# MeryylleA/Lunaris-Orion

Measured on AMD Instinct MI355X. Metric: 128x128 sprites/sec, VAE training step (train_hybrid.py _process_batch), latent_dim=512, higher is better.
Workload: dtype f16; 1 GPU; VAE-only training step (fwd+MSE/KL+bwd+clip+AdamW), per-GPU batch 64, latent_dim 512, teacher scalar 0 (--reward_scale 0 --quality_weight 0; the full hybrid step of BASELINE config 3 is the config3_full_hybrid object of a --full run at N=1), gradient_accumulation_steps 1, fp16 MFMA operands / fp32 accumulate, fp32 master weights; global_batch=64, latent_dim=512, parallelism=single, linear_weight_gradients=factored (never materialised)

## Files before the change

include/lunaris_hip.h:

```cpp
#ifndef LUNARIS_HIP_H
#define LUNARIS_HIP_H
#include <stddef.h>
#include <stdint.h>
#ifdef __cplusplus
extern "C" {
#endif

const char* lo_last_error(void);
int lo_version(void);

void lo_prof_enable(int on);
int lo_prof_count(void);
int lo_prof_get(int i, char* name, int name_cap, double* ms, double* flops, double* bytes);

enum {
  LO_KIND_CONV3_S1 = 0,
  LO_KIND_CONV3_S2 = 1,
  LO_KIND_CONVT4_S2 = 2,
  LO_KIND_CONV3_S1_DGRAD = 3,
  LO_KIND_CONV3_S2_DGRAD = 4,
  LO_KIND_CONVT4_S2_DGRAD = 5,
  LO_KIND_LINEAR = 6
};


size_t lo_packed_weight_elems_for(int kind, int B, int H, int W, int Cin, int Cout);
int lo_pack_weight_for(int kind, int B, int H, int W, int Cin, int Cout, const float* w, void* wp, void* stream);
int lo_conv_forward(int kind, int B, int H, int W, int Cin, int Cout, const void* in, const void* wp, const float* bias,
                    const void* add_src, void* out, float* gn_partial, int* mt_out, void* stream);
int lo_quantize_act_f8(const void* x16, void* x8, size_t n, void* stream);
int lo_pack_weight_f8_for(int kind, int B, int H, int W, int Cin, int Cout, const void* wp16, void* wp8, float* wscale, void* stream);
int lo_conv_forward_f8(int kind, int B, int H, int W, int Cin, int Cout, const void* in8, const void* wp8, const float* wscale,
                       const float* bias, const void* add_src, void* out, float* gn_partial, int* mt_out, void* stream);
int lo_conv3x3_fused_tap_forward(int B, int H, int W, int Cin, int Cout, int fp8, const void* in, const void* wp, const float* wscale,
                                 const float* bias, int leaky_relu, void* out, float* bn_partial, void* stream);
int lo_teacher_conv3x3_forward_f8(int B, int H, int W, int Cin, int Cout, const void* in8, const void* wp8, const float* wscale,
                                  const float* bias, int leaky_relu, void* out, float* bn_partial, int* rows_out, void* stream);
int lo_linear_splitk(int M, int K, int N, const void* x, const void* wp, const float* bias, float* slab, int nsplit,
                     float* out32, void* out16, void* stream);
size_t lo_wgrad_slab_bytes_for(int kind, int B, int H, int W, int Cin, int Cout);
int lo_conv_wgrad(int kind, int B, int H, int W, int Cin, int Cout, const void* x, const void* dy, float* slab,
                  float* grad, float scale, void* stream);

int lo_gn_mish_forward(const void* v, const float* gn_partial, int MT, const float* gamma, const float* beta,
                       const void* other, void* y, float* stats, int B, int HW, int C, int mode, void* stream);
int lo_gn_nchunk_for(int HW, int C);
int lo_gn_mish_backward(const void* dy, const void* v, const void* other, const float* stats, const float* gamma,
                        const float* beta, void* ds, void* dv, float* P1, float* P2, float* dgamma, float* dbeta,
                        float* dbias, int B, int HW, int C, int mode, float scale, void* stream);

int lo_first_conv_forward(const float* x, const float* w, const float* bias, void* v, float* gn_partial, int B, void* stream);
int lo_first_conv_wgrad_op(const float* x, const void* dv, float* partial , float* dw, int B, float scale, void* stream);
int lo_image_dgrad_op(const void* dy, int cout, int stride, const float* w, int B, float scale, float* dx, void* stream);
int lo_final_conv_forward(const void* a4, const float* w, const float* bias, const float* target, float* recon,
                          float* mse_partial, int B, void* stream);
int lo_final_conv_backward(const void* a4, const float* w, const float* recon, const float* target, const float* drecon,
                           const float* coef_dev, float gscale, void* da4, float* partial , float* dw,
                           float* db, int B, float scale, void* stream);

int lo_decode_sprites_u8(const void* u8_hwc, float* out_chw, int B, void* stream);

int lo_selfattn2d_forward(const float* x, const float* wq, const float* bq, const float* wk, const float* bk, const float* wv,
                          const float* bv, const float* gamma, float* q, float* k, float* v, float* out, int B, int C,
                          int N, void* stream);
size_t lo_selfattn2d_backward_scratch_elems(int B, int C, int N);
int lo_selfattn2d_backward(const float* x, const float* wq, const float* wk, const float* wv, const float* gamma,
                           const float* q, const float* k, const float* v, const float* dy, float* scratch, float* dx,
                           float* dwq, float* dbq, float* dwk, float* dbk, float* dwv, float* dbv, float* dgamma, int B,
                           int C, int N, void* stream);

int lo_clip_adamw_step(float* p, const float* g, float* m, float* v, size_t n, float max_norm, float lr, float beta1,
                       float beta2, float eps, float weight_decay, int step, float* scratch, void* stream);

int lo_clip_adamw_step_presummed(float* p, const float* g, float* m, float* v, size_t n, size_t presummed_begin, float max_norm,
                                 float lr, float beta1, float beta2, float eps, float weight_decay, int step, float* scratch,
                                 void* stream);

typedef struct LoVae LoVae;
int lo_vae_create(int batch, int latent_dim, LoVae** out);
#define LO_VAE_FP8_FWD 1u
int lo_vae_create_ex(int batch, int latent_dim, unsigned flags, LoVae** out);
void lo_vae_destroy(LoVae* h);
int lo_vae_set_gradnorm_scratch(LoVae* h, float* scratch);
int lo_gradnorm_early_range(const float* flat_grads, size_t begin, size_t end, float* scratch, void* stream);
int lo_vae_set_async_handover(LoVae* h, int on);
int lo_vae_wait_handover(LoVae* h, void* stream);
int lo_vae_gradnorm_presummed(const LoVae* h);
int lo_vae_num_params(const LoVae* h);
size_t lo_vae_param_offset(const LoVae* h, int index);
size_t lo_vae_param_numel(const LoVae* h, int index);
size_t lo_vae_flat_elems(const LoVae* h);
size_t lo_vae_workspace_bytes(const LoVae* h);
int lo_vae_pack(LoVae* h, const float* flat_params, void* ws, void* stream);
#define LO_OPT_PRESUMMED 1
#define LO_OPT_SERIAL 2
int lo_vae_optimizer_step(LoVae* h, float* p, const float* g, float* m, float* v, void* ws, float max_norm, float lr, float beta1,
                          float beta2, float eps, float weight_decay, int step, float* scratch, int flags, void* stream);
int lo_vae_join(LoVae* h, void* stream);
int lo_vae_set_linear_factored(LoVae* h, int mode);
int lo_vae_factor_block(const LoVae* h, size_t* byte_offset, size_t* bytes);
int lo_vae_materialize_gathered_linear_grads(LoVae* h, const void* gathered, int world, float* flat_grads, void* stream);
int lo_vae_linear_factored(const LoVae* h);
int lo_vae_materialize_linear_grads(LoVae* h, void* ws, float* flat_grads, void* stream);
int lo_vae_forward(LoVae* h, const float* x, const float* eps, uint64_t seed, const float* flat_params, void* ws,
                   float* recon, float* mu, float* logvar, const float* target, void* stream);
int lo_vae_decode(LoVae* h, const float* z, const float* flat_params, void* ws, float* recon, void* stream);
int lo_vae_encode(LoVae* h, const float* x, const float* flat_params, void* ws, float* mu, float* logvar, float* skip0, float* skip1,
                  float* skip2, void* stream);
int lo_vae_decode_skips(LoVae* h, const float* z, int n_skips, const float* skip0, const float* skip1, const float* skip2,
                        const float* flat_params, void* ws, float* recon, void* stream);
int lo_vae_decoder_backward(LoVae* h, const float* flat_params, void* ws, const float* recon, const float* drecon, float loss_scale,
                            float* dz, float* dskip0, float* dskip1, float* dskip2, float* flat_grads, void* stream);
int lo_vae_encoder_backward(LoVae* h, const float* x, const float* flat_params, void* ws, const float* gmu, const float* glv,
                            const float* gskip0, const float* gskip1, const float* gskip2, float loss_scale, float* flat_grads,
                            void* stream);
int lo_vae_encoder_backward_dx(LoVae* h, const float* x, const float* flat_params, void* ws, const float* gmu, const float* glv,
                               const float* gskip0, const float* gskip1, const float* gskip2, float loss_scale, float* flat_grads,
                               float* dx, void* stream);
int lo_vae_loss(LoVae* h, void* ws, float recon_weight, float kl_weight, float mean_advantage, const float* adv_dev,
                float accum, float loss_scale, float* losses_dev, void* stream);
int lo_vae_backward(LoVae* h, const float* x, const float* flat_params, void* ws, const float* recon, const float* target,
                    int fused, const float* drecon, const float* gmu, const float* glv, float loss_scale,
                    float* flat_grads, void* stream);
int lo_vae_backward_dx(LoVae* h, const float* x, const float* flat_params, void* ws, const float* recon, const float* target,
                       int fused, const float* drecon, const float* gmu, const float* glv, float loss_scale,
                       float* flat_grads, float* dx, void* stream);

int lo_vae_sync_fail_word(const LoVae* h, size_t* byte_offset, int* fused_layers);

int lo_grad_scale_pick(const float* g0, size_t n0, const float* g1, size_t n1, const float* g2, size_t n2, const float* g3, size_t n3,
                       const float* g4, size_t n4, float* scratch, void* stream);
int lo_scale_copy_dev(const float* src, float* dst, size_t n, const float* scale_dev, void* stream);
int lo_grad_unscale_dev(float* x, size_t n, const float* scale_dev, const void* fail_word, void* stream);
int lo_vae_fp8_layers(const LoVae* h, int* layers);
int lo_vae_debug_tensor(const LoVae* h, int which, int s, int k, size_t* byte_offset, int* dims4);

typedef struct LoTeacher LoTeacher;
int lo_teacher_create(int batch, int num_experts, int feature_dim, int embedding_dim, LoTeacher** out);
#define LO_TEACHER_FP8_CONV 1u
int lo_teacher_create_ex(int batch, int num_experts, int feature_dim, int embedding_dim, unsigned flags, LoTeacher** out);
void lo_teacher_destroy(LoTeacher* h);
int lo_teacher_num_tensors(const LoTeacher* h);
const char* lo_teacher_tensor_name(const LoTeacher* h, int index);
size_t lo_teacher_tensor_numel(const LoTeacher* h, int index);
long long lo_teacher_tensor_offset(const LoTeacher* h, int index);
size_t lo_teacher_flat_elems(const LoTeacher* h);
size_t lo_teacher_workspace_bytes(const LoTeacher* h);
int lo_teacher_pack(LoTeacher* h, const float* flat_state, void* ws, void* stream);
int lo_teacher_forward(LoTeacher* h, const float* x, float* flat_state, void* ws, int training, float dropout_p,
                       uint64_t drop_seed, float* quality_scores, float* expert_weights, float* style_embedding,
                       float* prompt_embedding, float* semantic_score, void* stream);
int lo_teacher_last_path(const LoTeacher* h);
int lo_dropout_mask(uint64_t drop_seed, int site, float dropout_p, size_t n, uint8_t* keep, void* stream);

int lo_teacher_grad_range(const LoTeacher* h, size_t* begin_elem, size_t* end_elem);
int lo_teacher_heads_backward(LoTeacher* h, const float* flat_state, void* ws, const float* expert_weights, float coef,
                              float* rows, float* flat_grads, void* stream);
int lo_teacher_heads_saved(const LoTeacher* h, size_t* byte_offsets3, size_t* elems3);
int lo_teacher_heads_backward_ex(LoTeacher* h, const float* flat_state, const float* pooled_f, const float* pooled_e,
                                 const float* raw_q, const float* expert_weights, const float* d_quality, const float* d_weights,
                                 float dropout_p, uint64_t drop_seed, float* rows, float* flat_grads, void* stream);
size_t lo_teacher_full_backward_bytes(const LoTeacher* h);
int lo_teacher_forward_keep(LoTeacher* h, const float* images_nchw, float* flat_state, void* ws, void* bws, float dropout_p,
                            uint64_t drop_seed, float* quality_scores, float* expert_weights, float* style_embedding,
                            float* prompt_embedding, float* semantic_score, void* stream);
int lo_teacher_full_backward(LoTeacher* h, const float* images_nchw, float* flat_state, void* ws, void* bws, const float* expert_weights,
                             float coef, float gscale, float* rows, float* flat_grads, void* stream);
int lo_teacher_full_backward_ex(LoTeacher* h, const float* images_nchw, float* flat_state, void* ws, void* bws, const float* pooled_f,
                                const float* pooled_e, const float* raw_q, const float* expert_weights, const float* d_quality,
                                const float* d_weights, float dropout_p, uint64_t drop_seed, float gscale, float* rows, float* flat_grads,
                                void* stream);
int lo_teacher_full_backward_dx(LoTeacher* h, const float* images_nchw, float* flat_state, void* ws, void* bws, const float* pooled_f,
                                const float* pooled_e, const float* raw_q, const float* expert_weights, const float* d_quality,
                                const float* d_weights, float dropout_p, uint64_t drop_seed, float gscale, float* rows, float* flat_grads,
                                float* dx, void* stream);
int lo_teacher_clip_adamw_full(LoTeacher* h, float* flat_state, const float* flat_grads, float* m, float* v, float max_norm, float lr,
                               float beta1, float beta2, float eps, float weight_decay, int step, float* scratch, void* stream);
int lo_teacher_full_param_count(const LoTeacher* h, size_t* tensors, size_t* elems);
int lo_hybrid_reward(const float* quality_scores, const float* semantic_score, int B, float semantic_weight,
                     float reward_scale, float momentum, float quality_weight, float accum, float* state2, float* out7,
                     float* adv_dev, void* stream);

int lo_vae_backward_phase(LoVae* h, int phase, const float* x, const float* flat_params, void* ws, const float* recon,
                          const float* target, int fused, const float* drecon, const float* gmu, const float* glv,
                          float loss_scale, float* flat_grads, void* stream);
int lo_vae_linear_grad_range(const LoVae* h, size_t* begin_elem, size_t* end_elem);
int lo_vae_phase1_grad_range(const LoVae* h, size_t* begin_elem, size_t* end_elem);
int lo_vae_stage4_grad_range(const LoVae* h, size_t* begin_elem, size_t* end_elem);

int lo_dp_pack_f16(const float* g, void* wire, size_t n, float scale, void* stream);
int lo_dp_unpack_f16(const void* wire, float* g, size_t n, float inv_scale, void* stream);
int lo_dp_unpack_f16_sumsq(const void* wire, float* g, size_t n, float inv_scale, float* scratch, void* stream);
int lo_dp_sum_shares(const void* recv, void* share, int world, size_t chunk, int is_f16, void* stream);

#ifdef __cplusplus
}
#endif
#endif
```

lunaris_orion_amd/_lib.py:

```python
from __future__ import annotations

import ctypes as C
import os

import torch

HERE = os.path.dirname(os.path.abspath(__file__))
LIB_PATH = os.path.join(HERE, "liblunaris_hip.so")

if not os.path.exists(LIB_PATH):
    raise ImportError(
        f"{LIB_PATH} not found: build it with `python -m lunaris_orion_amd.build` (hipcc, gfx950). "
        "There is no CPU or PyTorch fallback for the lunaris_orion_amd hot path."
    )

lib = C.CDLL(LIB_PATH, mode=C.RTLD_GLOBAL)

vp, f32p, i32, sz, u64, flt = C.c_void_p, C.c_void_p, C.c_int, C.c_size_t, C.c_uint64, C.c_float

SIGNATURES = {
    "lo_last_error": (C.c_char_p, []),
    "lo_version": (i32, []),
    "lo_prof_enable": (None, [i32]),
    "lo_prof_count": (i32, []),
    "lo_prof_get": (i32, [i32, C.c_char_p, i32, C.POINTER(C.c_double), C.POINTER(C.c_double), C.POINTER(C.c_double)]),
    "lo_packed_weight_elems_for": (sz, [i32] * 6),
    "lo_pack_weight_for": (i32, [i32] * 6 + [f32p, vp, vp]),
    "lo_conv_forward": (i32, [i32] * 6 + [vp, vp, f32p, vp, vp, f32p, C.POINTER(C.c_int), vp]),
    "lo_quantize_act_f8": (i32, [vp, vp, sz, vp]),
    "lo_pack_weight_f8_for": (i32, [i32] * 6 + [vp, vp, f32p, vp]),
    "lo_conv_forward_f8": (i32, [i32] * 6 + [vp, vp, f32p, f32p, vp, vp, f32p, C.POINTER(C.c_int), vp]),
    "lo_conv3x3_fused_tap_forward": (i32, [i32] * 6 + [vp, vp, f32p, f32p, i32, vp, f32p, vp]),
    "lo_teacher_conv3x3_forward_f8": (i32, [i32] * 5 + [vp, vp, f32p, f32p, i32, vp, f32p, C.POINTER(C.c_int), vp]),
    "lo_linear_splitk": (i32, [i32, i32, i32, vp, vp, f32p, f32p, i32, f32p, vp, vp]),
    "lo_wgrad_slab_bytes_for": (sz, [i32] * 6),
    "lo_conv_wgrad": (i32, [i32] * 6 + [vp, vp, f32p, f32p, flt, vp]),
    "lo_gn_mish_forward": (i32, [vp, f32p, i32, f32p, f32p, vp, vp, f32p, i32, i32, i32, i32, vp]),
    "lo_gn_nchunk_for": (i32, [i32, i32]),
    "lo_gn_mish_backward": (i32, [vp, vp, vp, f32p, f32p, f32p, vp, vp, f32p, f32p, f32p, f32p, f32p, i32, i32, i32, i32, flt, vp]),
    "lo_first_conv_forward": (i32, [f32p, f32p, f32p, vp, f32p, i32, vp]),
    "lo_first_conv_wgrad_op": (i32, [f32p, vp, f32p, f32p, i32, flt, vp]),
    "lo_image_dgrad_op": (i32, [vp, i32, i32, f32p, i32, flt, f32p, vp]),
    "lo_final_conv_forward": (i32, [vp, f32p, f32p, f32p, f32p, f32p, i32, vp]),
    "lo_final_conv_backward": (i32, [vp, f32p, f32p, f32p, f32p, f32p, flt, vp, f32p, f32p, f32p, i32, flt, vp]),
    "lo_decode_sprites_u8": (i32, [vp, f32p, i32, vp]),
    "lo_selfattn2d_forward": (i32, [f32p] * 12 + [i32, i32, i32, vp]),
    "lo_selfattn2d_backward_scratch_elems": (C.c_size_t, [i32, i32, i32]),
    "lo_selfattn2d_backward": (i32, [f32p] * 18 + [i32, i32, i32, vp]),
    "lo_clip_adamw_step": (i32, [f32p, f32p, f32p, f32p, sz, flt, flt, flt, flt, flt, flt, i32, f32p, vp]),
    "lo_teacher_create": (i32, [i32, i32, i32, i32, C.POINTER(C.c_void_p)]),
    "lo_teacher_create_ex": (i32, [i32, i32, i32, i32, C.c_uint, C.POINTER(C.c_void_p)]),
    "lo_teacher_destroy": (None, [vp]),
    "lo_teacher_num_tensors": (i32, [vp]),
    "lo_teacher_tensor_name": (C.c_char_p, [vp, i32]),
    "lo_teacher_tensor_numel": (sz, [vp, i32]),
    "lo_teacher_tensor_offset": (C.c_longlong, [vp, i32]),
    "lo_teacher_flat_elems": (sz, [vp]),
    "lo_teacher_workspace_bytes": (sz, [vp]),
    "lo_teacher_pack": (i32, [vp, f32p, vp, vp]),
    "lo_teacher_forward": (i32, [vp, f32p, f32p, vp, i32, flt, u64, f32p, f32p, f32p, f32p, f32p, vp]),
    "lo_teacher_last_path": (i32, [vp]),
    "lo_dropout_mask": (i32, [u64, i32, flt, sz, vp, vp]),
    "lo_teacher_grad_range": (i32, [vp, C.POINTER(C.c_size_t), C.POINTER(C.c_size_t)]),
    "lo_teacher_heads_backward": (i32, [vp, f32p, vp, f32p, flt, f32p, f32p, vp]),
    "lo_teacher_heads_saved": (i32, [vp, C.POINTER(C.c_size_t), C.POINTER(C.c_size_t)]),
    "lo_teacher_full_backward_bytes": (C.c_size_t, [vp]),
    "lo_teacher_full_backward_ex": (i32, [vp, f32p, f32p, vp, vp, f32p, f32p, f32p, f32p, f32p, f32p, flt, u64, flt, f32p, f32p, vp]),
    "lo_teacher_full_backward_dx": (i32, [vp, f32p, f32p, vp, vp, f32p, f32p, f32p, f32p, f32p, f32p, flt, u64, flt, f32p, f32p, f32p, vp]),
    "lo_teacher_forward_keep": (i32, [vp, f32p, f32p, vp, vp, flt, u64, f32p, f32p, f32p, f32p, f32p, vp]),
    "lo_teacher_full_backward": (i32, [vp, f32p, f32p, vp, vp, f32p, flt, flt, f32p, f32p, vp]),
    "lo_teacher_clip_adamw_full": (i32, [vp, f32p, f32p, f32p, f32p, flt, flt, flt, flt, flt, flt, i32, f32p, vp]),
    "lo_teacher_full_param_count": (i32, [vp, C.POINTER(C.c_size_t), C.POINTER(C.c_size_t)]),
    "lo_teacher_heads_backward_ex": (i32, [vp, f32p, f32p, f32p, f32p, f32p, f32p, f32p, flt, u64, f32p, f32p, vp]),
    "lo_hybrid_reward": (i32, [f32p, f32p, i32, flt, flt, flt, flt, flt, f32p, f32p, f32p, vp]),
    "lo_vae_create": (i32, [i32, i32, C.POINTER(C.c_void_p)]),
    "lo_vae_create_ex": (i32, [i32, i32, C.c_uint, C.POINTER(C.c_void_p)]),
    "lo_vae_set_gradnorm_scratch": (i32, [vp, f32p]),
    "lo_gradnorm_early_range": (i32, [f32p, sz, sz, f32p, vp]),
    "lo_vae_set_async_handover": (i32, [vp, i32]),
    "lo_vae_wait_handover": (i32, [vp, vp]),
    "lo_vae_optimizer_step": (i32, [vp, f32p, f32p, f32p, f32p, vp, flt, flt, flt, flt, flt, flt, i32, f32p, i32, vp]),
    "lo_vae_join": (i32, [vp, vp]),
    "lo_vae_set_linear_factored": (i32, [vp, i32]),
    "lo_vae_linear_factored": (i32, [vp]),
    "lo_vae_factor_block": (i32, [vp, C.POINTER(C.c_size_t), C.POINTER(C.c_size_t)]),
    "lo_vae_materialize_gathered_linear_grads": (i32, [vp, vp, i32, f32p, vp]),
    "lo_vae_materialize_linear_grads": (i32, [vp, vp, f32p, vp]),
    "lo_vae_gradnorm_presummed": (i32, [vp]),
    "lo_clip_adamw_step_presummed": (i32, [f32p, f32p, f32p, f32p, sz, sz, flt, flt, flt, flt, flt, flt, i32, f32p, vp]),
    "lo_vae_destroy": (None, [vp]),
    "lo_vae_num_params": (i32, [vp]),
    "lo_vae_param_offset": (sz, [vp, i32]),
    "lo_vae_param_numel": (sz, [vp, i32]),
    "lo_vae_flat_elems": (sz, [vp]),
    "lo_vae_workspace_bytes": (sz, [vp]),
    "lo_vae_pack": (i32, [vp, f32p, vp, vp]),
    "lo_vae_forward": (i32, [vp, f32p, f32p, u64, f32p, vp, f32p, f32p, f32p, f32p, vp]),
    "lo_vae_decode": (i32, [vp, f32p, f32p, vp, f32p, vp]),
    "lo_vae_encode": (i32, [vp, f32p, f32p, vp, f32p, f32p, f32p, f32p, f32p, vp]),
    "lo_vae_decode_skips": (i32, [vp, f32p, i32, f32p, f32p, f32p, f32p, vp, f32p, vp]),
    "lo_vae_decoder_backward": (i32, [vp, f32p, vp, f32p, f32p, flt, f32p, f32p, f32p, f32p, f32p, vp]),
    "lo_vae_encoder_backward": (i32, [vp, f32p, f32p, vp, f32p, f32p, f32p, f32p, f32p, flt, f32p, vp]),
    "lo_vae_encoder_backward_dx": (i32, [vp, f32p, f32p, vp, f32p, f32p, f32p, f32p, f32p, flt, f32p, f32p, vp]),
    "lo_vae_loss": (i32, [vp, vp, flt, flt, flt, f32p, flt, flt, f32p, vp]),
    "lo_vae_backward": (i32, [vp, f32p, f32p, vp, f32p, f32p, i32, f32p, f32p, f32p, flt, f32p, vp]),
    "lo_vae_backward_dx": (i32, [vp, f32p, f32p, vp, f32p, f32p, i32, f32p, f32p, f32p, flt, f32p, f32p, vp]),
    "lo_vae_backward_phase": (i32, [vp, i32, f32p, f32p, vp, f32p, f32p, i32, f32p, f32p, f32p, flt, f32p, vp]),
    "lo_vae_linear_grad_range": (i32, [vp, C.POINTER(C.c_size_t), C.POINTER(C.c_size_t)]),
    "lo_vae_phase1_grad_range": (i32, [vp, C.POINTER(C.c_size_t), C.POINTER(C.c_size_t)]),
    "lo_vae_debug_tensor": (i32, [vp, i32, i32, i32, C.POINTER(C.c_size_t), C.POINTER(C.c_int)]),
    "lo_dp_pack_f16": (i32, [f32p, vp, sz, flt, vp]),
    "lo_dp_unpack_f16": (i32, [vp, f32p, sz, flt, vp]),
    "lo_dp_unpack_f16_sumsq": (i32, [vp, f32p, sz, flt, f32p, vp]),
    "lo_dp_sum_shares": (i32, [vp, vp, i32, sz, i32, vp]),
    "lo_vae_sync_fail_word": (i32, [vp, C.POINTER(C.c_size_t), C.POINTER(C.c_int)]),
    "lo_grad_scale_pick": (i32, [f32p, sz, f32p, sz, f32p, sz, f32p, sz, f32p, sz, f32p, vp]),
    "lo_scale_copy_dev": (i32, [f32p, f32p, sz, f32p, vp]),
    "lo_grad_unscale_dev": (i32, [f32p, sz, f32p, vp, vp]),
    "lo_vae_fp8_layers": (i32, [vp, C.POINTER(C.c_int)]),
    "lo_vae_stage4_grad_range": (i32, [vp, C.POINTER(C.c_size_t), C.POINTER(C.c_size_t)]),
}

for _name, (_res, _args) in SIGNATURES.items():
    _fn = getattr(lib, _name)
    _fn.restype = _res
    _fn.argtypes = _args


class LunarisHipError(RuntimeError):
    pass


def check(rc: int, what: str = "") -> None:
    if rc != 0:
        msg = lib.lo_last_error()
        raise LunarisHipError(f"{what or 'liblunaris_hip'} failed (rc={rc}): {msg.decode() if msg else ''}")


def ptr(t) -> int | None:
    if t is None:
        return None
    return t.data_ptr()


def stream_ptr() -> int:
    return torch.cuda.current_stream().cuda_stream


def require_gpu() -> None:
    if not torch.cuda.is_available():
        raise LunarisHipError(
            "lunaris_orion_amd needs an AMD GPU (gfx950) visible to PyTorch-ROCm; there is no CPU fallback. "
            "The CPU oracle lives in oracle/ and is test infrastructure only."
        )
```

lunaris_orion_amd/build.py:

```python
from __future__ import annotations

import os
import subprocess
import sys

HERE = os.path.dirname(os.path.abspath(__file__))
CSRC = os.path.join(HERE, "csrc")
LIB = os.path.join(HERE, "liblunaris_hip.so")
SOURCES = ["lo_util.cpp", "lo_conv_geom.hip", "lo_igemm.hip", "lo_conv_f8.hip", "lo_conv_select.hip", "lo_conv3.hip", "lo_wgrad.hip", "lo_wgrad3.hip", "lo_wgrad2.hip", "lo_norm.hip", "lo_edge.hip", "lo_imgdgrad.hip", "lo_train.hip", "lo_lowrank.hip", "lo_attn.hip", "lo_teacher_plan.hip", "lo_teacher_kernels.hip", "lo_teacher_f128.hip", "lo_teacher_heads.hip", "lo_teacher_forward.hip", "lo_teacher_bwd_block.hip", "lo_teacher_bwd.hip", "lo_api.hip", "lo_vae_plan.hip", "lo_vae_opt.hip", "lo_vae_step.hip"]
HEADERS = ["lo_common.h", "lo_internal.h", "lo_conv.h", "lo_conv_dev.h", "lo_norm.h", "lo_vae.h", "lo_teacher.h", os.path.join("..", "..", "include", "lunaris_hip.h")]


def _hipcc() -> str:
    for c in (os.environ.get("HIPCC"), "/opt/rocm/bin/hipcc", "hipcc"):
        if c and (os.path.isabs(c) and os.path.exists(c) or not os.path.isabs(c)):
            return c
    return "hipcc"


def needs_build() -> bool:
    if not os.path.exists(LIB):
        return True
    t = os.path.getmtime(LIB)
    for f in SOURCES + HEADERS:
        p = os.path.join(CSRC, f)
        if os.path.exists(p) and os.path.getmtime(p) > t:
            return True
    return False


def build(force: bool = False, verbose: bool = True) -> str:
    if not force and not needs_build():
        return LIB
    objs = []
    procs = []
    os.makedirs(os.path.join(HERE, "build"), exist_ok=True)
    for f in SOURCES:
        src = os.path.join(CSRC, f)
        obj = os.path.join(HERE, "build", f + ".o")
        cmd = [_hipcc(), "--offload-arch=gfx950", "-O3", "-fPIC", "-std=c++17", "-x", "hip", "-c", src, "-o", obj]
        if verbose:
            print(" ".join(cmd), flush=True)
        procs.append((f, subprocess.Popen(cmd, stdout=subprocess.PIPE, stderr=subprocess.STDOUT, text=True)))
        objs.append(obj)
    fail = False
    for f, p in procs:
        out, _ = p.communicate()
        if p.returncode != 0:
            fail = True
            sys.stderr.write(f"[build] {f} failed:\n{out}\n")
        elif verbose and out.strip():
            print(out)
    if fail:
        raise RuntimeError("hipcc failed")
    cmd = [_hipcc(), "--offload-arch=gfx950", "-shared", "-fPIC", "-o", LIB] + objs
    if verbose:
        print(" ".join(cmd), flush=True)
    subprocess.check_call(cmd)
    return LIB


if __name__ == "__main__":
    build(force="--force" in sys.argv)
    print("built", LIB)
```

lunaris_orion_amd/csrc/lo_api.hip:

```cpp
#include "lo_internal.h"
#include "lo_conv.h"
#include "lo_norm.h"
#include "../../include/lunaris_hip.h"
#include <stdio.h>
#include <string.h>
#include <stdlib.h>
#include <vector>


extern "C" const char* lo_last_error(void) { return lo_get_error(); }
extern "C" int lo_version(void) { return 1; }

extern "C" size_t lo_packed_weight_elems_for(int kind, int B, int H, int W, int Cin, int Cout) {
  LoGeom g;
  if (lo_make_geom(&g, kind, B, H, W, Cin, Cout) != LO_OK) return 0;
  return lo_packed_weight_elems(g);
}
extern "C" int lo_pack_weight_for(int kind, int B, int H, int W, int Cin, int Cout, const float* w, void* wp, void* stream) {
  LoGeom g;
  LO_TRY(lo_make_geom(&g, kind, B, H, W, Cin, Cout));
  return lo_pack_weight(w, (f16*)wp, g, S(stream));
}
extern "C" int lo_conv_forward(int kind, int B, int H, int W, int Cin, int Cout, const void* in, const void* wp,
                               const float* bias, const void* add_src, void* out, float* gn_partial, int* mt_out,
                               void* stream) {
  LoGeom g;
  LO_TRY(lo_make_geom(&g, kind, B, H, W, Cin, Cout));
  const LoConvOp op{.in = (const f16*)in, .w = (const f16*)wp, .bias = bias, .add_src = (const f16*)add_src, .out = (f16*)out, .gn_partial = gn_partial};
  if (mt_out) *mt_out = lo_conv_choose(g, lo_conv_use(op)).mts;
  return lo_conv_run(g, op, S(stream));
}
extern "C" int lo_quantize_act_f8(const void* x16, void* x8, size_t n, void* stream) {
  LO_REQUIRE(x16 && x8, "lo_quantize_act_f8: null argument");
  return lo_quantize_f8((const f16*)x16, (uint8_t*)x8, n, S(stream));
}
extern "C" int lo_pack_weight_f8_for(int kind, int B, int H, int W, int Cin, int Cout, const void* wp16, void* wp8, float* wscale,
                                     void* stream) {
  LO_REQUIRE(wp16 && wp8 && wscale, "lo_pack_weight_f8_for: null argument");
  LoGeom g;
  LO_TRY(lo_make_geom(&g, kind, B, H, W, Cin, Cout));
  return lo_pack_f8_one(g, (const f16*)wp16, (uint8_t*)wp8, wscale, S(stream));
}
extern "C" int lo_conv_forward_f8(int kind, int B, int H, int W, int Cin, int Cout, const void* in8, const void* wp8,
                                  const float* wscale, const float* bias, const void* add_src, void* out, float* gn_partial,
                                  int* mt_out, void* stream) {
  LO_REQUIRE(in8 && wp8 && wscale && out, "lo_conv_forward_f8: null argument");
  LoGeom g;
  LO_TRY(lo_make_geom(&g, kind, B, H, W, Cin, Cout));
  const LoConvOp op{.bias = bias, .add_src = (const f16*)add_src, .out = (f16*)out, .gn_partial = gn_partial};
  LoConvUse use = lo_conv_use(op);
  use.f8 = true;
  if (mt_out) *mt_out = lo_conv_choose(g, use).mts;
  return lo_conv_run_f8(g, (const uint8_t*)in8, (const uint8_t*)wp8, wscale, op, S(stream));
}
extern "C" int lo_conv3x3_fused_tap_forward(int B, int H, int W, int Cin, int Cout, int fp8, const void* in, const void* wp, const float* wscale,
                                            const float* bias, int leaky_relu, void* out, float* bn_partial, void* stream) {
  LO_REQUIRE(in && wp && out && (!fp8 || wscale), "lo_conv3x3_fused_tap_forward: null argument");
  LoGeom g;
  LO_TRY(lo_make_geom(&g, LO_CONV3_S1, B, H, W, Cin, Cout));
  LoConvExtra ex{leaky_relu ? 1 : 0, bn_partial};
  if (fp8) return lo_conv3_run_pp_f8(g, (const uint8_t*)in, (const uint8_t*)wp, wscale, bias, (f16*)out, S(stream), &ex);
  return lo_conv3_run_pp_xf(g, (const f16*)in, nullptr, nullptr, 0, (const f16*)wp, bias, (f16*)out, S(stream), &ex);
}
extern "C" int lo_teacher_conv3x3_forward_f8(int B, int H, int W, int Cin, int Cout, const void* in8, const void* wp8, const float* wscale,
                                             const float* bias, int leaky_relu, void* out, float* bn_partial, int* rows_out, void* stream) {
  LO_REQUIRE(in8 && wp8 && wscale && out, "lo_teacher_conv3x3_forward_f8: null argument");
  LoGeom g;
  LO_TRY(lo_make_geom(&g, LO_CONV3_S1, B, H, W, Cin, Cout));
  const LoConvExtra ex{leaky_relu ? 1 : 0, bn_partial};
  const LoConvOp op{.bias = bias, .out = (f16*)out, .ex = &ex};
  LoConvUse use = lo_conv_use(op);
  use.f8 = true;
  const LoConvChoice c = lo_conv_choose(g, use);
  LO_REQUIRE(c.kernel == LO_CK_IGEMM_F8 && (B * H * W) % c.bm == 0,
             "lo_teacher_conv3x3_forward_f8: %d -> %d channels on %d x %d x %d is not served on e4m3 operands (Cin %% 128, Cout %% 64, whole M tiles)",
             Cin, Cout, B, H, W);
  if (rows_out) *rows_out = c.rows;
  return lo_conv_run_f8(g, (const uint8_t*)in8, (const uint8_t*)wp8, wscale, op, S(stream));
}
extern "C" int lo_linear_splitk(int M, int K, int N, const void* x, const void* wp, const float* bias, float* slab,
                                int nsplit, float* out32, void* out16, void* stream) {
  LoGeom g;
  LO_TRY(lo_make_geom(&g, LO_LINEAR, M, 1, 1, K, N));
  LO_TRY(lo_conv_run(g, {.in = (const f16*)x, .w = (const f16*)wp, .slab = slab, .nsplit = nsplit}, S(stream)));
  return lo_splitk_reduce(slab, bias, out32, (f16*)out16, M, N, nsplit, S(stream));
}
extern "C" size_t lo_wgrad_slab_bytes_for(int kind, int B, int H, int W, int Cin, int Cout) {
  LoGeom g;
  if (lo_make_geom(&g, kind, B, H, W, Cin, Cout) != LO_OK) return 0;
  return lo_wgrad_slab_bytes(g);
}
extern "C" int lo_conv_wgrad(int kind, int B, int H, int W, int Cin, int Cout, const void* x, const void* dy, float* slab,
                             float* grad, float scale, void* stream) {
  LoGeom g;
  LO_REQUIRE(kind == LO_CONV3_S1 || kind == LO_CONV3_S2 || kind == LO_CONVT4_S2 || kind == LO_LINEAR,
             "lo_conv_wgrad: kind %d is not a forward op", kind);
  LO_TRY(lo_make_geom(&g, kind, B, H, W, Cin, Cout));
  return lo_wgrad_run(g, (const f16*)x, (const f16*)dy, slab, grad, scale, S(stream));
}
extern "C" int lo_gn_mish_forward(const void* v, const float* gn_partial, int MT, const float* gamma, const float* beta,
                                  const void* other, void* y, float* stats, int B, int HW, int C, int mode, void* stream) {
  return lo_gn_forward({(const f16*)v, stats, gamma, beta, B, HW, C},
                       {.partial = gn_partial, .MT = MT, .other = (const f16*)other, .mode = mode, .y = (f16*)y}, S(stream));
}
extern "C" int lo_gn_nchunk_for(int HW, int C) { return lo_gn_nchunk(HW, C); }
extern "C" int lo_gn_mish_backward(const void* dy, const void* v, const void* other, const float* stats, const float* gamma,
                                   const float* beta, void* ds, void* dv, float* P1, float* P2, float* dgamma, float* dbeta,
                                   float* dbias, int B, int HW, int C, int mode, float scale, void* stream) {
  return lo_gn_bwd({(const f16*)v, stats, gamma, beta, B, HW, C},
                   {.dy = (const f16*)dy, .other = (const f16*)other, .mode = mode, .ds = (f16*)ds, .dv = (f16*)dv, .P1 = P1, .P2 = P2},
                   dgamma, dbeta, dbias, scale, S(stream));
}
extern "C" int lo_first_conv_forward(const float* x, const float* w, const float* bias, void* v, float* gn_partial, int B,
                                     void* stream) {
  return lo_first_conv_fwd(x, w, bias, (f16*)v, gn_partial, B, S(stream));
}
extern "C" int lo_first_conv_wgrad_op(const float* x, const void* dv, float* partial, float* dw, int B, float scale, void* stream) {
  return lo_first_conv_wgrad(x, (const f16*)dv, partial, dw, B, scale, S(stream));
}
extern "C" int lo_image_dgrad_op(const void* dy, int cout, int stride, const float* w, int B, float scale, float* dx, void* stream) {
  return lo_image_dgrad((const f16*)dy, cout, stride, w, B, scale, dx, S(stream));
}
extern "C" int lo_final_conv_forward(const void* a4, const float* w, const float* bias, const float* target, float* recon,
                                     float* mse_partial, int B, void* stream) {
  return lo_final_conv_fwd((const f16*)a4, w, bias, target, recon, mse_partial, B, S(stream));
}
extern "C" int lo_final_conv_backward(const void* a4, const float* w, const float* recon, const float* target,
                                      const float* drecon, const float* coef_dev, float gscale, void* da4, float* partial,
                                      float* dw, float* db, int B, float scale, void* stream) {
  return lo_final_conv_bwd((const f16*)a4, w, recon, target, drecon, coef_dev, gscale, (f16*)da4, partial, dw, db, B, scale,
                           S(stream));
}
extern "C" int lo_clip_adamw_step(float* p, const float* g, float* m, float* v, size_t n, float max_norm, float lr,
                                  float beta1, float beta2, float eps, float weight_decay, int step, float* scratch,
                                  void* stream) {
  LO_TRY(lo_gradnorm(g, n, max_norm, scratch, scratch + 1024, S(stream)));
  return lo_adamw(p, g, m, v, n, scratch + 1024, lr, beta1, beta2, eps, weight_decay, step, S(stream));
}

extern "C" int lo_clip_adamw_step_presummed(float* p, const float* g, float* m, float* v, size_t n, size_t presummed_begin, float max_norm,
                                            float lr, float beta1, float beta2, float eps, float weight_decay, int step, float* scratch,
                                            void* stream) {
  LO_REQUIRE(p && g && m && v && scratch && presummed_begin <= n && presummed_begin % 4 == 0, "lo_clip_adamw_step_presummed: bad argument");
  LO_TRY(lo_gradnorm_split(g, presummed_begin, max_norm, scratch, scratch + 1024, S(stream)));
  return lo_adamw(p, g, m, v, n, scratch + 1024, lr, beta1, beta2, eps, weight_decay, step, S(stream));
}

extern "C" int lo_decode_sprites_u8(const void* u8_hwc, float* out_chw, int B, void* stream) {
  LO_REQUIRE(u8_hwc && out_chw && B > 0, "lo_decode_sprites_u8: bad argument");
  return lo_decode_sprites((const uint8_t*)u8_hwc, out_chw, B, S(stream));
}

extern "C" int lo_selfattn2d_forward(const float* x, const float* wq, const float* bq, const float* wk, const float* bk,
                                     const float* wv, const float* bv, const float* gamma, float* q, float* k, float* v,
                                     float* out, int B, int C, int N, void* stream) {
  LO_REQUIRE(x && wq && bq && wk && bk && wv && bv && gamma && q && k && v && out, "lo_selfattn2d_forward: null argument");
  return lo_selfattn2d_fwd(x, wq, bq, wk, bk, wv, bv, gamma, q, k, v, out, B, C, N, S(stream));
}

extern "C" size_t lo_selfattn2d_backward_scratch_elems(int B, int C, int N) { return lo_selfattn2d_bwd_scratch(B, C, N); }
extern "C" int lo_selfattn2d_backward(const float* x, const float* wq, const float* wk, const float* wv, const float* gamma,
                                      const float* q, const float* k, const float* v, const float* dy, float* scratch, float* dx,
                                      float* dwq, float* dbq, float* dwk, float* dbk, float* dwv, float* dbv, float* dgamma, int B,
                                      int C, int N, void* stream) {
  LO_REQUIRE(x && wq && wk && wv && gamma && q && k && v && dy && scratch && dx && dwq && dbq && dwk && dbk && dwv && dbv && dgamma,
             "lo_selfattn2d_backward: null argument");
  return lo_selfattn2d_bwd(x, wq, wk, wv, gamma, q, k, v, dy, scratch, dx, dwq, dbq, dwk, dbk, dwv, dbv, dgamma, B, C, N, S(stream));
}

extern "C" int lo_dp_pack_f16(const float* g, void* wire, size_t n, float scale, void* stream) {
  LO_REQUIRE(g && wire, "lo_dp_pack_f16: null argument");
  return lo_dp_pack_f16_run(g, (f16*)wire, n, scale, S(stream));
}
extern "C" int lo_dp_unpack_f16_sumsq(const void* wire, float* g, size_t n, float inv_scale, float* scratch, void* stream) {
  LO_REQUIRE(g && wire && scratch, "lo_dp_unpack_f16_sumsq: null argument");
  return lo_dp_unpack_f16_sumsq_run((const f16*)wire, g, n, inv_scale, scratch, S(stream));
}
extern "C" int lo_dp_unpack_f16(const void* wire, float* g, size_t n, float inv_scale, void* stream) {
  LO_REQUIRE(g && wire, "lo_dp_unpack_f16: null argument");
  return lo_dp_unpack_f16_run((const f16*)wire, g, n, inv_scale, S(stream));
}
extern "C" int lo_dp_sum_shares(const void* recv, void* share, int world, size_t chunk, int is_f16, void* stream) {
  LO_REQUIRE(recv && share && world >= 1, "lo_dp_sum_shares: bad argument");
  return lo_dp_sum_shares_run(recv, share, world, chunk, is_f16, 1.0f / (float)world, S(stream));
}

extern "C" int lo_grad_scale_pick(const float* g0, size_t n0, const float* g1, size_t n1, const float* g2, size_t n2, const float* g3,
                                  size_t n3, const float* g4, size_t n4, float* scratch, void* stream) {
  LO_REQUIRE(scratch, "lo_grad_scale_pick: null scratch");
  const float* g[5] = {g0, g1, g2, g3, g4};
  const size_t n[5] = {n0, n1, n2, n3, n4};
  return lo_grad_scale_pick_run(g, n, scratch, S(stream));
}
extern "C" int lo_scale_copy_dev(const float* src, float* dst, size_t n, const float* scale_dev, void* stream) {
  LO_REQUIRE(src && dst && scale_dev, "lo_scale_copy_dev: null argument");
  return lo_scale_copy_dev_run(src, dst, n, scale_dev, S(stream));
}
extern "C" int lo_grad_unscale_dev(float* x, size_t n, const float* scale_dev, const void* fail_word, void* stream) {
  LO_REQUIRE(x && scale_dev, "lo_grad_unscale_dev: null argument");
  return lo_scale_dev_run(x, n, scale_dev, (const unsigned int*)fail_word, S(stream));
}
```

lunaris_orion_amd/csrc/lo_conv.h:

```cpp
#pragma once
#include "lo_common.h"

int lo_pack_weight(const float* w, f16* wp, const LoGeom& g, hipStream_t st);
int lo_pack_all(const LoPackJob* jobs_dev, int njobs, int nblocks, hipStream_t st, int block_base = 0);
int lo_pack_blocks(const LoGeom& g);
size_t lo_packed_weight_elems(const LoGeom& g);
static inline int lo_geom_packed_elems(const LoGeom& g) {
  int off = 0;
  for (int p = 0; p < g.n_phase; ++p) off += g.Cout * g.T[p] * g.Cin;
  return off;
}
static inline double lo_geom_flops(const LoGeom& g) {
  double f = 0;
  for (int p = 0; p < g.n_phase; ++p) f += 2.0 * g.B * g.GH * g.GW * (double)g.Cout * g.T[p] * g.Cin;
  return f;
}
static inline double lo_geom_bytes(const LoGeom& g) {
  return 2.0 * ((double)g.B * g.Hin * g.Win * g.Cin + (double)g.B * g.Hout * g.Wout * g.Cout + lo_geom_packed_elems(g));
}

struct LoGnBwdFuse {
  const f16* v; const float* stats; const float* gamma; const float* beta; float* P1;
  f16* dv = nullptr; float* P2 = nullptr; unsigned int* counter = nullptr; unsigned int target = 0; unsigned int* fail = nullptr;
  bool keep_out = false;
};
struct LoConvExtra { int act; float* bn_partial; int out_pitch = 0; int out_choff = 0; };
struct LoConvOp {
  const f16* in = nullptr;
  const f16* w = nullptr;
  const float* bias = nullptr;
  const f16* add_src = nullptr;
  f16* out = nullptr;
  float* gn_partial = nullptr;
  float* slab = nullptr;
  int nsplit = 1;
  const LoGnBwdFuse* gb = nullptr;
  const LoConvExtra* ex = nullptr;
  const LoGnFuse* gf = nullptr;
};
struct LoConvUse {
  bool bias = false, gn_partial = false, add = false;
  bool gb = false, gb_apply = false;
  bool ex = false, concat = false;
  bool gf = false;
  int nsplit = 1;
  bool f8 = false;
};
static inline LoConvUse lo_conv_use(const LoConvOp& op) {
  LoConvUse u;
  u.bias = op.bias != nullptr; u.gn_partial = op.gn_partial != nullptr; u.add = op.add_src != nullptr;
  u.gb = op.gb != nullptr; u.gb_apply = op.gb && op.gb->dv;
  u.ex = op.ex != nullptr; u.concat = op.ex && op.ex->out_pitch > 0;
  u.gf = op.gf != nullptr;
  u.nsplit = op.nsplit < 1 ? 1 : op.nsplit;
  return u;
}

enum LoConvKernel { LO_CK_NONE = 0, LO_CK_IGEMM, LO_CK_IGEMM_SPLITK, LO_CK_IGEMM_F8, LO_CK_CONV3_PP, LO_CK_CONVT4_PATCH, LO_CK_CONVS2D_PATCH };
struct LoConvChoice {
  int kernel;
  int bm, bn, bk;
  int th, tw;
  int grid;
  int mts;
  int rows;
  int nt;
  bool gn_fuse;
  bool gnb_apply;
};
LoConvChoice lo_conv_choose(const LoGeom& g, const LoConvUse& use);
int lo_conv_splitk_plan(const LoGeom& g);
int lo_conv_run(const LoGeom& g, const LoConvOp& op, hipStream_t st, LoConvChoice* chosen = nullptr);
int lo_conv_run_f8(const LoGeom& g, const uint8_t* in8, const uint8_t* w8, const float* wscale, const LoConvOp& op, hipStream_t st,
                   LoConvChoice* chosen = nullptr);

int lo_igemm_run(const LoGeom& g, const LoConvOp& op, const LoConvChoice& c, hipStream_t st);
int lo_igemm_run_f8(const LoGeom& g, const uint8_t* in8, const uint8_t* w8, const float* wscale, const LoConvOp& op, const LoConvChoice& c,
                    hipStream_t st);
int lo_splitk_reduce(const float* slab, const float* bias, float* out32, f16* out16, int M, int N, int nsplit, hipStream_t st);

int lo_conv3_run(const LoGeom& g, const LoConvOp& op, const LoConvChoice& c, hipStream_t st);
int lo_convt4_patch_run(const LoGeom& g, const LoConvOp& op, const LoConvChoice& c, hipStream_t st);
int lo_convs2d_patch_run(const LoGeom& g, const LoConvOp& op, const LoConvChoice& c, hipStream_t st);
bool lo_conv3_pp_applies(const LoGeom& g);
bool lo_conv3_pp_f8_applies(const LoGeom& g);
int lo_conv3_pp_rows(const LoGeom& g);
int lo_conv3_run_pp_xf(const LoGeom& g, const f16* in, const f16* xc, const f16* kx, int nlev, const f16* wp, const float* bias,
                       f16* out, hipStream_t st, const LoConvExtra* ex);
int lo_conv3_run_pp_f8(const LoGeom& g, const uint8_t* in8, const uint8_t* w8, const float* wscale, const float* bias, f16* out,
                       hipStream_t st, const LoConvExtra* ex);

struct LoPackF8Job { const f16* src; uint8_t* dst; float* scale; int K[LO_MAX_PHASE]; int wofs[LO_MAX_PHASE]; int Cout, n_phase, block0; };
void lo_pack_f8_job(LoPackF8Job* j, const LoGeom& g, const f16* src, uint8_t* dst, float* scale, int block0);
int lo_pack_f8_all(const LoPackF8Job* jobs_dev, int njobs, int nblocks, hipStream_t st, int block_base = 0);
int lo_pack_f8_one(const LoGeom& g, const f16* wp, uint8_t* w8, float* wscale, hipStream_t st);
int lo_quantize_f8(const f16* x, uint8_t* x8, size_t n, hipStream_t st);

enum LoWgradKernel { LO_WK_WGRAD3 = 0, LO_WK_WGRAD2, LO_WK_TN };
struct LoWgradChoice { int kernel; int nsplit; };
LoWgradChoice lo_wgrad_choose(const LoGeom& g);
int lo_wgrad_run(const LoGeom& g, const f16* x, const f16* dy, float* slab, float* grad, float scale, hipStream_t st);
size_t lo_wgrad_slab_bytes(const LoGeom& g);
int lo_wgrad3_nsplit(const LoGeom& g);
int lo_wgrad3_run(const LoGeom& g, const f16* x, const f16* dy, float* slab, hipStream_t st, int* nsplit_out);
int lo_wgrad2_nsplit(const LoGeom& g);
int lo_wgrad2_run(const LoGeom& g, const f16* x, const f16* dy, float* slab, hipStream_t st, int* nsplit_out);
```

lunaris_orion_amd/csrc/lo_conv_select.hip:

```cpp
#include "lo_conv.h"
#include "lo_norm.h"
#include <stdarg.h>
#include <stdio.h>
#include <string.h>
#include <stdlib.h>

int lo_conv_splitk_plan(const LoGeom& g) {
  if (g.n_phase != 1 || g.T[0] < 9 || g.Cin % 64 != 0 || g.Cout % 128 != 0) return 0;
  const long M = (long)g.B * g.GH * g.GW;
  if (M % 128 != 0 || !lo_gn_bwd_local_applies(g.GH * g.GW, g.Cout)) return 0;
  const long tiles = (M / 128) * (g.Cout / 128);
  if (tiles >= 256) return 0;
  const int ksteps = g.T[0] * (g.Cin / 64);
  int ns = (int)((512 + tiles - 1) / tiles);
  while (ns > 1 && ksteps / ns < 8) --ns;
  return ns >= 2 ? ns : 0;
}

static void pick_tile(const LoGeom& g, int* bm_out, int* bn_out) {
  const int per_sample = g.GH * g.GW;
  const size_t M = (size_t)g.B * per_sample;
  const int BK = (g.Cin % 64 == 0) ? 64 : 32;
  constexpr int min_wgs = 512;
  const int cand[4][2] = {{128, 128}, {128, 64}, {64, 128}, {64, 64}};
  int bm = 64, bn = (g.Cout % 64 == 0) ? 64 : 32;
  if (BK == 32) {
    bn = 64;
    bm = (per_sample % 128 == 0 && (M / 128) * (g.Cout / 64) * g.n_phase >= (size_t)min_wgs) ? 128 : 64;
  } else if (g.Cout % 64 != 0) {
    bm = (per_sample % 128 == 0 && (M / 128) * (g.Cout / 32) * g.n_phase >= (size_t)min_wgs) ? 128 : 64;
  } else {
    for (int i = 0; i < 4; ++i) {
      int cm = cand[i][0], cn = cand[i][1];
      if (per_sample % cm || g.Cout % cn || (g.Cout >> 3) > cn) continue;
      bm = cm; bn = cn;
      if (((M + cm - 1) / cm) * (g.Cout / cn) * g.n_phase >= (size_t)min_wgs) break;
    }
  }
  *bm_out = bm; *bn_out = bn;
}

static inline int conv3_mode() {
  static const int m = getenv("LO_HALO") ? atoi(getenv("LO_HALO")) : 2;
  return m;
}
static inline bool conv3_tile(const LoGeom& g, int* th, int* tw, int* bn) {
  if (g.n_phase != 1 || g.T[0] != 9 || g.in_stride != 1 || g.out_stride != 1) return false;
  if (g.Cin % 64 || g.Cout % 64 || g.Win % 16 || g.Hin % 16) return false;
  const long t16 = (long)g.B * (g.Hin / 16) * (g.Win / 16);
  if (g.Cout % 128 == 0 && t16 * (g.Cout / 128) >= 256) { *th = 16; *tw = 16; *bn = 128; }
  else if (g.Cout % 128 == 0) { *th = 8; *tw = 16; *bn = 128; }
  else if (g.Cout == 64) { *th = 16; *tw = 16; *bn = 64; }
  else return false;
  return (g.Cout >> 3) <= *bn;
}
static bool conv3_selected(const LoGeom& g, bool need_bn, int* th, int* tw, int* bn) {
  const int mode = conv3_mode();
  if (mode == 0 || !conv3_tile(g, th, tw, bn)) return false;
  if (mode == 2) {
    const long tiles = (long)g.B * (g.Hin / *th) * (g.Win / *tw) * (g.Cout / *bn);
    const bool long_grid = *th == 16 && *bn == 128 && tiles >= 1024;
    if (!(long_grid || (!need_bn && tiles >= 256))) return false;
  }
  return true;
}

static bool convt4_patch_geom(const LoGeom& g) {
  if (g.n_phase != 4 || g.in_stride != 1 || g.out_stride != 2) return false;
  if (!((g.Cin == 64 && g.Cout == 32) || (g.Cin == 128 && g.Cout == 64))) return false;
  for (int p = 0; p < 4; ++p) if (g.T[p] != 4) return false;
  return g.Hin % 16 == 0 && g.Win % 16 == 0 && g.Hout == 2 * g.Hin && g.Wout == 2 * g.Win;
}
static bool convs2d_patch_geom(const LoGeom& g) {
  if (g.n_phase != 4 || g.in_stride != 1 || g.out_stride != 2 || g.Cin != 128 || g.Cout != 64) return false;
  if (g.T[0] != 1 || g.T[1] != 2 || g.T[2] != 2 || g.T[3] != 4) return false;
  for (int p = 0; p < 4; ++p)
    for (int t = 0; t < g.T[p]; ++t) if (g.dy[p][t] < 0 || g.dy[p][t] > 1 || g.dx[p][t] < 0 || g.dx[p][t] > 1) return false;
  return g.Hin % 16 == 0 && g.Win % 16 == 0 && g.Hout == 2 * g.Hin && g.Wout == 2 * g.Win;
}

static void set_rows(LoConvChoice& c, const LoGeom& g, int mts, int nt) {
  c.mts = mts; c.nt = nt;
  c.rows = g.B * mts;
}
static void choose_igemm_tile(LoConvChoice& c, const LoGeom& g, int n_z) {
  const long M = (long)g.B * g.GH * g.GW;
  c.mts = (g.GH * g.GW / c.bm) * g.n_phase; c.nt = g.Cout / c.bn;
  c.rows = (int)((M / c.bm) * g.n_phase);
  c.grid = (int)((M + c.bm - 1) / c.bm) * c.nt * n_z;
}

static LoConvChoice choose_f8(const LoGeom& g) {
  static const bool force = !(getenv("LO_F8_FORCE") && atoi(getenv("LO_F8_FORCE")) == 0);
  LoConvChoice c{};
  int th, tw, bn;
  if (!(g.Cin % 128 == 0 && g.Cout % 64 == 0 && (force || !conv3_selected(g, false, &th, &tw, &bn)))) return c;
  c.kernel = LO_CK_IGEMM_F8;
  pick_tile(g, &c.bm, &c.bn);
  c.bk = 128;
  choose_igemm_tile(c, g, g.n_phase);
  return c;
}

LoConvChoice lo_conv_choose(const LoGeom& g, const LoConvUse& u) {
  if (u.f8) return choose_f8(g);
  LoConvChoice c{};
  const int nsplit = u.nsplit < 1 ? 1 : u.nsplit;
  const int per_sample = g.GH * g.GW;
  const bool bare = nsplit == 1 && !u.gb && !u.ex && !u.gf;
  const int tiles16 = (g.Hin / 16) * (g.Win / 16);
  if (bare && !u.add && convt4_patch_geom(g)) {
    c.kernel = LO_CK_CONVT4_PATCH;
    set_rows(c, g, tiles16, 1);
    c.grid = g.B * tiles16;
  } else if (bare && !u.bias && !u.gn_partial && convs2d_patch_geom(g) && g.B * tiles16 >= 128) {
    c.kernel = LO_CK_CONVS2D_PATCH;
    set_rows(c, g, 0, 1);
    c.grid = g.B * tiles16;
  } else if (int th, tw, bn; nsplit == 1 && conv3_selected(g, u.ex, &th, &tw, &bn)) {
    c.kernel = LO_CK_CONV3_PP;
    c.th = th; c.tw = tw; c.bn = bn;
    set_rows(c, g, (g.Hin / c.th) * (g.Win / c.tw), g.Cout / c.bn);
    c.grid = c.rows * c.nt;
    c.gn_fuse = u.gf && c.mts * c.nt <= LO_GNF_MAX_TILES;
    c.gnb_apply = u.gb_apply && (g.Cout >> 3) >= 8 && c.mts * c.nt <= LO_GNF_MAX_TILES;
  } else if (nsplit > 1) {
    c.kernel = LO_CK_IGEMM_SPLITK;
    c.bm = c.bn = (g.T[0] > 1 && ((long)g.B * per_sample) % 128 == 0 && g.Cout % 128 == 0) ? 128 : 64;
    c.bk = (g.Cin % 64 == 0) ? 64 : 32;
    choose_igemm_tile(c, g, nsplit);
    c.mts = c.rows = 0;
  } else {
    c.kernel = LO_CK_IGEMM;
    pick_tile(g, &c.bm, &c.bn);
    c.bk = (g.Cin % 64 == 0) ? 64 : 32;
    choose_igemm_tile(c, g, g.n_phase);
    const bool whole = g.Cin % 64 == 0 && g.Cout % 64 == 0 && per_sample % c.bm == 0 && (g.Cout >> 3) <= c.bn;
    c.gn_fuse = u.gf && whole && !convt4_patch_geom(g) && c.mts * c.nt <= LO_GNF_MAX_TILES;
    c.gnb_apply = u.gb_apply && whole && g.n_phase == 1 && (g.Cout >> 3) >= 8 && c.nt <= 8 && c.mts <= LO_GNF_MAX_TILES;
  }
  return c;
}

int lo_conv_run(const LoGeom& g, const LoConvOp& op, hipStream_t st, LoConvChoice* chosen) {
  const LoGnFuse* gf = op.gf;
  const LoGnBwdFuse* gb = op.gb;
  LO_REQUIRE(g.Cin % 32 == 0, "lo_conv_run: Cin=%d must be a multiple of 32", g.Cin);
  LO_REQUIRE(g.Cout % 32 == 0, "lo_conv_run: Cout=%d must be a multiple of 32", g.Cout);
  const LoConvUse u = lo_conv_use(op);
  const LoConvChoice c = lo_conv_choose(g, u);
  if (chosen) *chosen = c;
  if (gf) {
    LO_REQUIRE(u.nsplit <= 1 && !u.add && !gb && !u.ex && gf->y && gf->xbuf && gf->counter && gf->fail && gf->gamma && gf->beta &&
               (gf->mode == 0 || gf->other), "lo_conv_run: bad fused-GroupNorm arguments");
    LO_REQUIRE(c.gn_fuse && c.mts == gf->MTs && c.nt == gf->NT,
               "lo_conv_run: fused GroupNorm asked for a geometry / tile grid the kernel does not have (check LoConvChoice::gn_fuse)");
  }
  if (u.gb_apply)
    LO_REQUIRE(gb->P2 && gb->counter && gb->fail && c.gnb_apply,
               "lo_conv_run: fused GroupNorm-backward apply asked for a geometry the kernel does not support (check LoConvChoice::gnb_apply)");
  LO_REQUIRE(!u.concat || (!u.add && !gb && op.ex->out_pitch % 8 == 0 && op.ex->out_choff % 8 == 0), "lo_conv_run: bad concatenated-output arguments");
  switch (c.kernel) {
    case LO_CK_CONVT4_PATCH: return lo_convt4_patch_run(g, op, c, st);
    case LO_CK_CONVS2D_PATCH: return lo_convs2d_patch_run(g, op, c, st);
    case LO_CK_CONV3_PP: return lo_conv3_run(g, op, c, st);
    case LO_CK_IGEMM_SPLITK:
    case LO_CK_IGEMM: return lo_igemm_run(g, op, c, st);
    default: break;
  }
  lo_set_error("lo_conv_run: no kernel for this op");
  return LO_ERR_ARG;
}

int lo_conv_run_f8(const LoGeom& g, const uint8_t* in8, const uint8_t* w8, const float* wscale, const LoConvOp& op, hipStream_t st,
                   LoConvChoice* chosen) {
  LO_REQUIRE(!op.gb && !op.gf && !op.slab && op.nsplit <= 1 && !(op.ex && op.ex->out_pitch > 0),
             "lo_conv_run_f8: the e4m3 path has bias, residual add, GroupNorm partials and the teacher epilogue (activation, BatchNorm partials) only");
  LoConvUse u = lo_conv_use(op);
  u.f8 = true;
  const LoConvChoice c = lo_conv_choose(g, u);
  if (chosen) *chosen = c;
  LO_REQUIRE(c.kernel == LO_CK_IGEMM_F8, "lo_conv_run_f8: geometry not supported (Cin %% 128, Cout %% 64)");
  return lo_igemm_run_f8(g, in8, w8, wscale, op, c, st);
}
```

lunaris_orion_amd/csrc/lo_internal.h:

```cpp
#pragma once
#include "lo_common.h"

static inline hipStream_t S(void* s) { return reinterpret_cast<hipStream_t>(s); }
#define LO_TRY(call)            \
  do {                          \
    int _r = (call);            \
    if (_r != LO_OK) return _r; \
  } while (0)

const char* lo_get_error();

int lo_first_conv_fwd(const float* x, const float* w, const float* bias, f16* v, float* gn_partial, int B, hipStream_t st);
int lo_first_conv_wgrad(const float* x, const f16* dv, float* partial, float* dw, int B, float scale, hipStream_t st);
int lo_colsum(const float* partial, float* out, int nrow, int ncol, int stride, float scale, hipStream_t st);

int lo_image_dgrad(const f16* dy, int cout, int stride, const float* w, int B, float scale, float* dx, hipStream_t st);
int lo_final_conv_fwd(const f16* a4, const float* w, const float* bias, const float* target, float* recon,
                      float* mse_partial, int B, hipStream_t st);
int lo_final_conv_bwd(const f16* a4, const float* w, const float* recon, const float* target, const float* drecon,
                      const float* coef, float gscale, f16* da4, float* partial, float* dw, float* db, int B, float scale,
                      hipStream_t st, hipStream_t sum_st = nullptr, hipEvent_t sum_after = nullptr);

int lo_head_reduce(const float* slab, const float* bias, const float* eps_in, uint64_t seed, float* mu, float* logvar,
                   f16* z, float* eps_out, float* kl_partial, int B, int L, int nsplit, hipStream_t st, float* mu_user = nullptr,
                   float* logvar_user = nullptr);
int lo_loss_finalize(const float* mse_partial, int n_mse, const float* kl_partial, int n_kl, float rw, float kw, float adv,
                     const float* adv_dev, float accum, float ls, float* losses, float* coefs, float n_rec, float n_lat,
                     hipStream_t st);
int lo_latent_bwd(const f16* dz, const float* mu, const float* logvar, const float* eps, const float* coefs,
                  const float* gmu, const float* glv, float gscale, f16* dml, int B, int L, hipStream_t st);
int lo_colsum_f16(const f16* x, float* out, int M, int N, float scale, hipStream_t st);
int lo_cast_f32_f16(const float* src, f16* dst, size_t n, hipStream_t st);
int lo_scale_f32(float* x, size_t n, float scale, hipStream_t st);
int lo_dp_pack_f16_run(const float* g, f16* wire, size_t n, float scale, hipStream_t st);
int lo_dp_unpack_f16_run(const f16* wire, float* g, size_t n, float inv_scale, hipStream_t st);
int lo_dp_unpack_f16_sumsq_run(const f16* wire, float* g, size_t n, float inv_scale, float* scratch, hipStream_t st);
int lo_dp_sum_shares_run(const void* recv, void* share, int world, size_t chunk, int is_f16, float inv_world, hipStream_t st);
int lo_transpose_cast(const float* src, f16* dst, int R, int C, hipStream_t st);
int lo_gradnorm(const float* g, size_t n, float max_norm, float* partial, float* norm_out, hipStream_t st,
                const unsigned int* fail = nullptr);
int lo_sumsq_range(const float* g, size_t begin, size_t end, float* partial, hipStream_t st);
int lo_gradnorm_split(const float* g, size_t presummed_begin, float max_norm, float* partial, float* norm_out, hipStream_t st,
                      const unsigned int* fail = nullptr);
int lo_grad_scale_pick_run(const float* const g[5], const size_t n[5], float* scratch, hipStream_t st);
int lo_scale_copy_dev_run(const float* src, float* dst, size_t n, const float* scale_dev, hipStream_t st);
int lo_scale_dev_run(float* x, size_t n, const float* scale_dev, const unsigned int* fail, hipStream_t st);
int lo_adamw(float* p, const float* g, float* m, float* v, size_t n, const float* norm, float lr, float beta1, float beta2,
             float eps, float wd, int step, hipStream_t st, f16* cast = nullptr);

int lo_selfattn2d_fwd(const float* x, const float* wq, const float* bq, const float* wk, const float* bk, const float* wv,
                      const float* bv, const float* gamma, float* q, float* k, float* v, float* out, int B, int C, int N,
                      hipStream_t st);
size_t lo_selfattn2d_bwd_scratch(int B, int C, int N);
int lo_selfattn2d_bwd(const float* x, const float* wq, const float* wk, const float* wv, const float* gamma, const float* q,
                      const float* k, const float* v, const float* dy, float* scratch, float* dx, float* dwq, float* dbq,
                      float* dwk, float* dbk, float* dwv, float* dbv, float* dgamma, int B, int C, int N, hipStream_t st);
int lo_decode_sprites(const uint8_t* u8, float* out, int B, hipStream_t st);

int lo_lowrank_bp(int B);
bool lo_lowrank_applies(int B, int N, int K);
int lo_transpose_pad_f16_multi(const f16* const* src, f16* const* dst, const int* C, int njobs, int R, int Rp, hipStream_t st);
struct LoLowrankNorm { const f16* fshort; int n_short; const f16* flong; int n_long; float* gram; float* partial; int nslots; };
int lo_lowrank_sumsq(const LoLowrankNorm* layers, int nlayers, int B, float scale, hipStream_t st);
struct LoLowrankMat { float* p; float* m; float* v; f16* cast; f16* cast_t; const f16* xt; const f16* yt; int N, K; };
int lo_adamw_lowrank(const LoLowrankMat* mats, int nmat, int B, float gscale, const float* norm, float lr, float beta1, float beta2,
                     float eps, float wd, int step, hipStream_t st);
int lo_lowrank_materialize(float* gout, const f16* xt, const f16* yt, int N, int K, int B, float gscale, hipStream_t st);
int lo_lowrank_materialize_gathered(float* gout, const f16* xt, const f16* yt, size_t rank_stride_elems, int world, int N, int K, int B,
                                    float gscale, hipStream_t st);
int lo_sumsq_blocks(const float* g, size_t n, float* partial, int nblocks, hipStream_t st);
```

lunaris_orion_amd/csrc/lo_train.hip:

```cpp
#include "lo_common.h"
#include <stdlib.h>

__device__ __forceinline__ uint64_t lo_mix64(uint64_t x) {
  x += 0x9E3779B97F4A7C15ull;
  x = (x ^ (x >> 30)) * 0xBF58476D1CE4E5B9ull;
  x = (x ^ (x >> 27)) * 0x94D049BB133111EBull;
  return x ^ (x >> 31);
}
__device__ __forceinline__ float lo_randn(uint64_t seed, uint64_t idx) {
  uint64_t h = lo_mix64(seed ^ lo_mix64(idx));
  float u1 = ((float)(uint32_t)(h >> 40) + 0.5f) * (1.0f / 16777216.0f);
  float u2 = ((float)(uint32_t)((h >> 8) & 0xFFFFFF)) * (1.0f / 16777216.0f);
  return sqrtf(-2.0f * __logf(u1)) * __cosf(6.28318530718f * u2);
}

__global__ __launch_bounds__(256) void lo_head_reduce_kernel(const float* __restrict__ slab, const float* __restrict__ bias,
                                                             const float* __restrict__ eps_in, uint64_t seed,
                                                             float* __restrict__ mu, float* __restrict__ logvar,
                                                             f16* __restrict__ z, float* __restrict__ eps_out,
                                                             float* __restrict__ kl_partial, int B, int L, int nsplit,
                                                             float* __restrict__ mu_user, float* __restrict__ logvar_user) {
  __shared__ float red[4];
  int i = blockIdx.x * 256 + threadIdx.x;
  float term = 0.f;
  if (i < B * L) {
    int b = i / L, l = i - b * L;
    float m = bias[l], lv = bias[L + l];
    int s = 0;
    for (; s + 8 <= nsplit; s += 8) {
      float pm[8], pl[8];
#pragma unroll
      for (int u = 0; u < 8; ++u) {
        const float* p = slab + ((size_t)(s + u) * B + b) * (2 * L);
        pm[u] = p[l];
        pl[u] = p[L + l];
      }
#pragma unroll
      for (int u = 0; u < 8; ++u) { m += pm[u]; lv += pl[u]; }
    }
    for (; s < nsplit; ++s) {
      const float* p = slab + ((size_t)s * B + b) * (2 * L);
      m += p[l];
      lv += p[L + l];
    }
    float e = eps_in ? eps_in[i] : lo_randn(seed, (uint64_t)i);
    float sd = expf(0.5f * lv);
    mu[i] = m;
    logvar[i] = lv;
    if (mu_user) { mu_user[i] = m; logvar_user[i] = lv; }
    eps_out[i] = e;
    z[i] = (f16)(m + e * sd);
    term = 1.f + lv - m * m - expf(lv);
  }
  float w = lo_wave_sum(term);
  if ((threadIdx.x & 63) == 0) red[threadIdx.x >> 6] = w;
  __syncthreads();
  if (threadIdx.x == 0) kl_partial[blockIdx.x] = red[0] + red[1] + red[2] + red[3];
}

__global__ __launch_bounds__(256) void lo_loss_finalize_kernel(const float* __restrict__ mse_partial, int n_mse,
                                                               const float* __restrict__ kl_partial, int n_kl,
                                                               float rw, float kw, float adv_host, float accum, float ls,
                                                               const float* __restrict__ adv_dev, float* __restrict__ losses,
                                                               float* __restrict__ coefs, float n_rec, float n_lat) {
  __shared__ double red[2][4];
  double a = 0.0, b = 0.0;
  for (int i0 = threadIdx.x; i0 < n_mse; i0 += 8 * 256) {
    float v[8];
#pragma unroll
    for (int u = 0; u < 8; ++u) v[u] = i0 + u * 256 < n_mse ? mse_partial[i0 + u * 256] : 0.f;
#pragma unroll
    for (int u = 0; u < 8; ++u) a += (double)v[u];
  }
  for (int i = threadIdx.x; i < n_kl; i += 256) b += (double)kl_partial[i];
#pragma unroll
  for (int o = 32; o > 0; o >>= 1) { a += __shfl_xor(a, o, 64); b += __shfl_xor(b, o, 64); }
  if ((threadIdx.x & 63) == 0) { red[0][threadIdx.x >> 6] = a; red[1][threadIdx.x >> 6] = b; }
  __syncthreads();
  if (threadIdx.x == 0) {
    const double sa = (red[0][0] + red[0][1]) + (red[0][2] + red[0][3]), sb = (red[1][0] + red[1][1]) + (red[1][2] + red[1][3]);
    float recon_loss = (float)(sa / (double)n_rec);
    float kl_loss = (float)(-0.5 * sb / (double)n_lat);
    float adv = adv_dev ? adv_dev[0] : adv_host;
    float pg = -adv * recon_loss;
    losses[0] = recon_loss;
    losses[1] = kl_loss;
    losses[2] = (rw * recon_loss + kw * kl_loss + pg) / accum;
    losses[3] = pg;
    coefs[0] = ls * (rw - adv) / accum * 2.0f / n_rec;
    coefs[1] = ls * kw / accum / n_lat;
  }
}

__global__ void lo_latent_bwd_kernel(const f16* __restrict__ dz, const float* __restrict__ mu, const float* __restrict__ logvar,
                                     const float* __restrict__ eps, const float* __restrict__ coefs,
                                     const float* __restrict__ gmu, const float* __restrict__ glv, float gscale,
                                     f16* __restrict__ dml, int B, int L) {
  int i = blockIdx.x * blockDim.x + threadIdx.x;
  if (i >= B * L) return;
  int b = i / L, l = i - b * L;
  float ckl = coefs ? coefs[1] : 0.f;
  float d = (float)dz[i];
  float lv = logvar[i];
  float dm = ckl * mu[i] + d;
  float dl = ckl * 0.5f * (expf(lv) - 1.f) + d * eps[i] * 0.5f * expf(0.5f * lv);
  if (gmu) dm += gscale * gmu[i];
  if (glv) dl += gscale * glv[i];
  dml[(size_t)b * 2 * L + l] = (f16)dm;
  dml[(size_t)b * 2 * L + L + l] = (f16)dl;
}

__global__ __launch_bounds__(256) void lo_colsum_f16_kernel(const f16* __restrict__ x, float* __restrict__ out, int M, int N, float scale) {
  __shared__ float red[8][32][8];
  const int cc = threadIdx.x & 31, rg = threadIdx.x >> 5;
  const int j0 = (blockIdx.x * 32 + cc) * 8;
  float t[8];
#pragma unroll
  for (int q = 0; q < 8; ++q) t[q] = 0.f;
  if (j0 < N) {
    for (int m = rg; m < M; m += 32) {
      f16x8 v[4];
#pragma unroll
      for (int u = 0; u < 4; ++u)
        if (m + 8 * u < M) v[u] = *reinterpret_cast<const f16x8*>(x + (size_t)(m + 8 * u) * N + j0);
#pragma unroll
      for (int u = 0; u < 4; ++u)
        if (m + 8 * u < M) {
#pragma unroll
          for (int q = 0; q < 8; ++q) t[q] += (float)v[u][q];
        }
    }
  }
#pragma unroll
  for (int q = 0; q < 8; ++q) red[rg][cc][q] = t[q];
  __syncthreads();
  const int c = threadIdx.x;
  const int j = blockIdx.x * 256 + c;
  if (j < N) {
    float tot = 0.f;
#pragma unroll
    for (int r = 0; r < 8; ++r) tot += red[r][c >> 3][c & 7];
    out[j] = tot * scale;
  }
}

__global__ void lo_decode_sprites_kernel(const uint8_t* __restrict__ u8, float* __restrict__ out, int npix_total) {
  int i = blockIdx.x * blockDim.x + threadIdx.x;
  if (i >= npix_total) return;
  int n = i >> 14, p = i & 16383;
  const uint8_t* s = u8 + (size_t)i * 3;
  float* d = out + (size_t)n * 3 * 16384 + p;
  d[0] = (float)s[0] / 127.5f - 1.0f;
  d[16384] = (float)s[1] / 127.5f - 1.0f;
  d[32768] = (float)s[2] / 127.5f - 1.0f;
}

__global__ void lo_cast_f32_f16_kernel(const float* __restrict__ src, f16* __restrict__ dst, size_t n4) {
  size_t i = (size_t)blockIdx.x * blockDim.x + threadIdx.x;
  size_t stride = (size_t)gridDim.x * blockDim.x;
  for (; i < n4; i += stride) {
    f32x4 v = reinterpret_cast<const f32x4*>(src)[i];
    f16x4 h = {(f16)v[0], (f16)v[1], (f16)v[2], (f16)v[3]};
    reinterpret_cast<f16x4*>(dst)[i] = h;
  }
}
__global__ __launch_bounds__(256) void lo_transpose_cast_kernel(const float* __restrict__ src, f16* __restrict__ dst, int R, int C) {
  __shared__ float t[64][65];
  const int r0 = blockIdx.y * 64, c0 = blockIdx.x * 64;
  const int tx = threadIdx.x & 63, ty = threadIdx.x >> 6;
  for (int i = ty; i < 64; i += 4) {
    int r = r0 + i, c = c0 + tx;
    t[i][tx] = (r < R && c < C) ? src[(size_t)r * C + c] : 0.f;
  }
  __syncthreads();
  for (int i = ty; i < 64; i += 4) {
    int c = c0 + i, r = r0 + tx;
    if (r < R && c < C) dst[(size_t)c * R + r] = (f16)t[tx][i];
  }
}

__global__ __launch_bounds__(256) void lo_sumsq_partial_kernel(const float* __restrict__ g, size_t n, float* __restrict__ partial) {
  __shared__ float red[4];
  size_t i = (size_t)blockIdx.x * 256 + threadIdx.x;
  size_t stride = (size_t)gridDim.x * 256;
  float acc = 0.f;
  size_t n4 = n / 4;
  for (size_t k = i; k < n4; k += stride) {
    f32x4 v = reinterpret_cast<const f32x4*>(g)[k];
    acc += v[0] * v[0] + v[1] * v[1] + v[2] * v[2] + v[3] * v[3];
  }
  if (blockIdx.x == 0 && threadIdx.x == 0)
    for (size_t k = n4 * 4; k < n; ++k) acc += g[k] * g[k];
  float w = lo_wave_sum(acc);
  if ((threadIdx.x & 63) == 0) red[threadIdx.x >> 6] = w;
  __syncthreads();
  if (threadIdx.x == 0) partial[blockIdx.x] = red[0] + red[1] + red[2] + red[3];
}
__global__ __launch_bounds__(256) void lo_gradnorm_finalize_kernel(const float* __restrict__ partial, int n, float max_norm,
                                                                   float* __restrict__ norm_out, const unsigned int* __restrict__ fail) {
  __shared__ double red[256];
  double a = 0.0;
  for (int i = threadIdx.x; i < n; i += 256) a += (double)partial[i];
  red[threadIdx.x] = a;
  __syncthreads();
  if (threadIdx.x == 0) {
    double s = 0.0;
    for (int i = 0; i < 256; ++i) s += red[i];
    float norm = (float)sqrt(s);
    float coef = max_norm / (norm + 1e-6f);
    if (coef > 1.0f) coef = 1.0f;
    bool finite = isfinite(norm);
    const bool lost = fail && *fail != 0u;
    norm_out[0] = norm;
    norm_out[1] = (finite && !lost) ? coef : 0.f;
    norm_out[2] = (finite && !lost) ? 1.f : 0.f;
    if (!finite) norm_out[3] += 1.f;
  }
}
__device__ __forceinline__ void lo_adamw_elem(float& p, float g, float& m, float& v, float coef, float decay, float omb1, float beta2,
                                              float omb2, float bc2_sqrt, float eps, float step_size) {
#pragma clang fp contract(off)
  const float gg = g * coef;
  const float pp = p * decay;
  const float mm = __builtin_fmaf(gg - m, omb1, m);
  const float v2 = __builtin_fmaf(omb2 * gg, gg, v * beta2);
  const float denom = sqrtf(v2) / bc2_sqrt + eps;
  p = __builtin_fmaf(-step_size, mm / denom, pp);
  m = mm;
  v = v2;
}
__global__ __launch_bounds__(256) void lo_adamw_kernel(float* __restrict__ p, const float* __restrict__ g, float* __restrict__ m,
                                                       float* __restrict__ v, size_t n, const float* __restrict__ norm,
                                                       float lr, float beta1, float beta2, float eps, float wd, float bc1,
                                                       float bc2_sqrt, f16* __restrict__ cast) {
  const float coef = norm ? norm[1] : 1.0f;
  const bool ok = norm ? (norm[2] != 0.f) : true;
  if (!ok) return;
  size_t i = (size_t)blockIdx.x * 256 + threadIdx.x;
  size_t stride = (size_t)gridDim.x * 256;
  const float step_size = lr / bc1, decay = 1.0f - lr * wd, omb1 = 1.0f - beta1, omb2 = 1.0f - beta2;
  size_t n4 = n / 4;
  constexpr int U = 4;
  for (size_t k0 = i; k0 < n4; k0 += U * stride) {
    f32x4 pv[U], gv[U], mv[U], vv[U];
#pragma unroll
    for (int u = 0; u < U; ++u) {
      const size_t k = k0 + u * stride;
      if (k < n4) {
        pv[u] = reinterpret_cast<f32x4*>(p)[k];
        gv[u] = reinterpret_cast<const f32x4*>(g)[k];
        mv[u] = reinterpret_cast<f32x4*>(m)[k];
        vv[u] = reinterpret_cast<f32x4*>(v)[k];
      }
    }
#pragma unroll
    for (int u = 0; u < U; ++u) {
      const size_t k = k0 + u * stride;
      if (k < n4) {
#pragma unroll
        for (int j = 0; j < 4; ++j) {
          float pe = pv[u][j], me = mv[u][j], ve = vv[u][j];
          lo_adamw_elem(pe, gv[u][j], me, ve, coef, decay, omb1, beta2, omb2, bc2_sqrt, eps, step_size);
          pv[u][j] = pe; mv[u][j] = me; vv[u][j] = ve;
        }
        reinterpret_cast<f32x4*>(p)[k] = pv[u];
        reinterpret_cast<f32x4*>(m)[k] = mv[u];
        reinterpret_cast<f32x4*>(v)[k] = vv[u];
        if (cast) reinterpret_cast<f16x4*>(cast)[k] = (f16x4){(f16)pv[u][0], (f16)pv[u][1], (f16)pv[u][2], (f16)pv[u][3]};
      }
    }
  }
  if (blockIdx.x == 0 && threadIdx.x == 0)
    for (size_t k = n4 * 4; k < n; ++k) {
      float pe = p[k], me = m[k], ve = v[k];
      lo_adamw_elem(pe, g[k], me, ve, coef, decay, omb1, beta2, omb2, bc2_sqrt, eps, step_size);
      p[k] = pe; m[k] = me; v[k] = ve;
      if (cast) cast[k] = (f16)pe;
    }
}

int lo_head_reduce(const float* slab, const float* bias, const float* eps_in, uint64_t seed, float* mu, float* logvar,
                   f16* z, float* eps_out, float* kl_partial, int B, int L, int nsplit, hipStream_t st, float* mu_user,
                   float* logvar_user) {
  int nb = (B * L + 255) / 256;
  LoProfScope _p("lo_head_reduce", 0, 4.0 * B * 2 * L * (nsplit + 2), st);
  hipLaunchKernelGGL(lo_head_reduce_kernel, dim3(nb), dim3(256), 0, st, slab, bias, eps_in, seed, mu, logvar, z, eps_out,
                     kl_partial, B, L, nsplit, mu_user, logvar_user);
  LO_LAUNCH_CHECK("head_reduce");
  return LO_OK;
}
int lo_loss_finalize(const float* mse_partial, int n_mse, const float* kl_partial, int n_kl, float rw, float kw, float adv,
                     const float* adv_dev, float accum, float ls, float* losses, float* coefs, float n_rec, float n_lat,
                     hipStream_t st) {
  LoProfScope _p("lo_loss_finalize", 0, 0, st);
  hipLaunchKernelGGL(lo_loss_finalize_kernel, dim3(1), dim3(256), 0, st, mse_partial, n_mse, kl_partial, n_kl, rw, kw, adv,
                     accum, ls, adv_dev, losses, coefs, n_rec, n_lat);
  LO_LAUNCH_CHECK("loss_finalize");
  return LO_OK;
}
int lo_latent_bwd(const f16* dz, const float* mu, const float* logvar, const float* eps, const float* coefs,
                  const float* gmu, const float* glv, float gscale, f16* dml, int B, int L, hipStream_t st) {
  int n = B * L;
  LoProfScope _p("lo_latent_bwd", 0, 0, st);
  LO_LAUNCH_STOP(lo_latent_bwd_kernel, dim3((n + 255) / 256), dim3(256), 0, st, dz, mu, logvar, eps, coefs, gmu, glv,
                     gscale, dml, B, L);
  LO_LAUNCH_CHECK("latent_bwd");
  return LO_OK;
}
int lo_colsum_f16(const f16* x, float* out, int M, int N, float scale, hipStream_t st) {
  LO_REQUIRE(N % 8 == 0, "lo_colsum_f16: N=%d must be a multiple of 8", N);
  LoProfScope _p("lo_colsum_f16", 0, 2.0 * M * N, st);
  hipLaunchKernelGGL(lo_colsum_f16_kernel, dim3((N + 255) / 256), dim3(256), 0, st, x, out, M, N, scale);
  LO_LAUNCH_CHECK("colsum_f16");
  return LO_OK;
}
__global__ void lo_scale_f32_kernel(float* __restrict__ x, size_t n, float scale) {
  const size_t i = (size_t)blockIdx.x * blockDim.x + threadIdx.x;
  if (i < n) x[i] *= scale;
}
int lo_scale_f32(float* x, size_t n, float scale, hipStream_t st) {
  hipLaunchKernelGGL(lo_scale_f32_kernel, dim3((unsigned)((n + 255) / 256)), dim3(256), 0, st, x, n, scale);
  LO_LAUNCH_CHECK("scale_f32");
  return LO_OK;
}
int lo_cast_f32_f16(const float* src, f16* dst, size_t n, hipStream_t st) {
  LO_REQUIRE(n % 4 == 0, "lo_cast_f32_f16: n must be a multiple of 4");
  size_t n4 = n / 4;
  int nb = (int)((n4 + 255) / 256 < 4096 ? (n4 + 255) / 256 : 4096);
  LoProfScope _p("lo_cast_f32_f16", 0, 6.0 * n, st);
  hipLaunchKernelGGL(lo_cast_f32_f16_kernel, dim3(nb), dim3(256), 0, st, src, dst, n4);
  LO_LAUNCH_CHECK("cast");
  return LO_OK;
}
int lo_transpose_cast(const float* src, f16* dst, int R, int C, hipStream_t st) {
  LoProfScope _p("lo_transpose_cast", 0, 6.0 * R * C, st);
  hipLaunchKernelGGL(lo_transpose_cast_kernel, dim3((C + 63) / 64, (R + 63) / 64), dim3(256), 0, st, src, dst, R, C);
  LO_LAUNCH_CHECK("transpose_cast");
  return LO_OK;
}
#define LO_NORM_BLOCKS 1024
int lo_sumsq_range(const float* g, size_t begin, size_t end, float* partial, hipStream_t st) {
  LoProfScope _p("lo_gradnorm (early range)", 0, 4.0 * (end - begin), st);
  hipLaunchKernelGGL(lo_sumsq_partial_kernel, dim3(LO_NORM_BLOCKS / 2), dim3(256), 0, st, g + begin, end - begin, partial + LO_NORM_BLOCKS / 2);
  LO_LAUNCH_CHECK("sumsq_range");
  return LO_OK;
}
int lo_sumsq_blocks(const float* g, size_t n, float* partial, int nblocks, hipStream_t st) {
  LoProfScope _p("lo_gradnorm (early range)", 0, 4.0 * n, st);
  hipLaunchKernelGGL(lo_sumsq_partial_kernel, dim3(nblocks), dim3(256), 0, st, g, n, partial);
  LO_LAUNCH_CHECK("sumsq_blocks");
  return LO_OK;
}
int lo_gradnorm_split(const float* g, size_t presummed_begin, float max_norm, float* partial, float* norm_out, hipStream_t st,
                      const unsigned int* fail) {
  LoProfScope _p("lo_gradnorm", 0, 4.0 * presummed_begin, st);
  hipLaunchKernelGGL(lo_sumsq_partial_kernel, dim3(LO_NORM_BLOCKS / 2), dim3(256), 0, st, g, presummed_begin, partial);
  LO_LAUNCH_CHECK("sumsq_head");
  hipLaunchKernelGGL(lo_gradnorm_finalize_kernel, dim3(1), dim3(256), 0, st, partial, LO_NORM_BLOCKS, max_norm, norm_out, fail);
  LO_LAUNCH_CHECK("gradnorm_finalize");
  return LO_OK;
}
int lo_gradnorm(const float* g, size_t n, float max_norm, float* partial , float* norm_out, hipStream_t st,
                const unsigned int* fail) {
  LoProfScope _p("lo_gradnorm", 0, 4.0 * n, st);
  hipLaunchKernelGGL(lo_sumsq_partial_kernel, dim3(LO_NORM_BLOCKS), dim3(256), 0, st, g, n, partial);
  LO_LAUNCH_CHECK("sumsq");
  hipLaunchKernelGGL(lo_gradnorm_finalize_kernel, dim3(1), dim3(256), 0, st, partial, LO_NORM_BLOCKS, max_norm, norm_out, fail);
  LO_LAUNCH_CHECK("gradnorm_finalize");
  return LO_OK;
}
int lo_adamw(float* p, const float* g, float* m, float* v, size_t n, const float* norm, float lr, float beta1, float beta2,
             float eps, float wd, int step, hipStream_t st, f16* cast) {
  float bc1 = 1.0f - powf(beta1, (float)step);
  float bc2 = 1.0f - powf(beta2, (float)step);
  double bc1d = 1.0 - pow((double)beta1, (double)step), bc2d = 1.0 - pow((double)beta2, (double)step);
  (void)bc1; (void)bc2;
  LoProfScope _p(cast ? "lo_adamw(+fp16 copy)" : "lo_adamw", 0, (cast ? 30.0 : 28.0) * n, st);
  constexpr int max_blocks = 256;
  const size_t want = (n / 4 + 255) / 256;
  const int nblk = want >= (size_t)max_blocks ? max_blocks : (want < 1 ? 1 : (int)want);
  LO_LAUNCH_STOP(lo_adamw_kernel, dim3(nblk), dim3(256), 0, st, p, g, m, v, n, norm, lr, beta1, beta2, eps, wd,
                     (float)bc1d, (float)sqrt(bc2d), cast);
  LO_LAUNCH_CHECK("adamw");
  return LO_OK;
}

int lo_decode_sprites(const uint8_t* u8, float* out, int B, hipStream_t st) {
  int n = B * 16384;
  LoProfScope _p("lo_decode_sprites", 0, 15.0 * n, st);
  hipLaunchKernelGGL(lo_decode_sprites_kernel, dim3((n + 255) / 256), dim3(256), 0, st, u8, out, n);
  LO_LAUNCH_CHECK("decode_sprites");
  return LO_OK;
}

__device__ __forceinline__ float lo_sat16(float x) { return x != x ? x : fminf(fmaxf(x, -65504.0f), 65504.0f); }
__global__ __launch_bounds__(256) void lo_dp_pack_f16_kernel(const float* __restrict__ g, f16* __restrict__ wire, size_t n, float scale) {
  const size_t stride = (size_t)gridDim.x * blockDim.x * 4;
  for (size_t i = ((size_t)blockIdx.x * blockDim.x + threadIdx.x) * 4; i < n; i += stride) {
    if (i + 4 <= n) {
      const float4 v = *reinterpret_cast<const float4*>(g + i);
      f16x4 o = {(f16)lo_sat16(v.x * scale), (f16)lo_sat16(v.y * scale), (f16)lo_sat16(v.z * scale), (f16)lo_sat16(v.w * scale)};
      *reinterpret_cast<f16x4*>(wire + i) = o;
    } else {
      for (size_t j = i; j < n; ++j) wire[j] = (f16)lo_sat16(g[j] * scale);
    }
  }
}
__global__ __launch_bounds__(256) void lo_dp_unpack_f16_kernel(const f16* __restrict__ wire, float* __restrict__ g, size_t n, float inv_scale) {
  const size_t stride = (size_t)gridDim.x * blockDim.x * 4;
  for (size_t i = ((size_t)blockIdx.x * blockDim.x + threadIdx.x) * 4; i < n; i += stride) {
    if (i + 4 <= n) {
      const f16x4 v = *reinterpret_cast<const f16x4*>(wire + i);
      *reinterpret_cast<float4*>(g + i) = make_float4((float)v[0] * inv_scale, (float)v[1] * inv_scale, (float)v[2] * inv_scale, (float)v[3] * inv_scale);
    } else {
      for (size_t j = i; j < n; ++j) g[j] = (float)wire[j] * inv_scale;
    }
  }
}
__global__ __launch_bounds__(256) void lo_dp_unpack_f16_sumsq_kernel(const f16* __restrict__ wire, float* __restrict__ g, size_t n, float inv_scale,
                                                                     float* __restrict__ partial) {
  __shared__ float red[4];
  const size_t stride = (size_t)gridDim.x * blockDim.x * 4;
  float acc = 0.f;
  for (size_t i = ((size_t)blockIdx.x * blockDim.x + threadIdx.x) * 4; i < n; i += stride) {
    if (i + 4 <= n) {
      const f16x4 v = *reinterpret_cast<const f16x4*>(wire + i);
      const float a = (float)v[0] * inv_scale, b = (float)v[1] * inv_scale, c = (float)v[2] * inv_scale, d = (float)v[3] * inv_scale;
      *reinterpret_cast<float4*>(g + i) = make_float4(a, b, c, d);
      acc += a * a + b * b + c * c + d * d;
    } else {
      for (size_t j = i; j < n; ++j) { const float a = (float)wire[j] * inv_scale; g[j] = a; acc += a * a; }
    }
  }
  const float w = lo_wave_sum(acc);
  if ((threadIdx.x & 63) == 0) red[threadIdx.x >> 6] = w;
  __syncthreads();
  if (threadIdx.x == 0) partial[blockIdx.x] = red[0] + red[1] + red[2] + red[3];
}
template <typename T>
__global__ __launch_bounds__(256) void lo_dp_sum_shares_kernel(const T* __restrict__ recv, T* __restrict__ share, int world, size_t chunk, float inv_world) {
  const size_t stride = (size_t)gridDim.x * blockDim.x;
  for (size_t i = (size_t)blockIdx.x * blockDim.x + threadIdx.x; i < chunk; i += stride) {
    float t = 0.f;
    for (int r = 0; r < world; ++r) t += (float)recv[(size_t)r * chunk + i];
    share[i] = (T)(t * inv_world);
  }
}
static inline int lo_dp_blocks(size_t work_items) {
  size_t b = (work_items + 255) / 256;
  return (int)(b < 1 ? 1 : (b > 2048 ? 2048 : b));
}
int lo_dp_pack_f16_run(const float* g, f16* wire, size_t n, float scale, hipStream_t st) {
  LoProfScope _p("lo_dp_pack_f16", 0, 6.0 * n, st);
  hipLaunchKernelGGL(lo_dp_pack_f16_kernel, dim3(lo_dp_blocks((n + 3) / 4)), dim3(256), 0, st, g, wire, n, scale);
  LO_LAUNCH_CHECK("dp_pack_f16");
  return LO_OK;
}
int lo_dp_unpack_f16_run(const f16* wire, float* g, size_t n, float inv_scale, hipStream_t st) {
  LoProfScope _p("lo_dp_unpack_f16", 0, 6.0 * n, st);
  hipLaunchKernelGGL(lo_dp_unpack_f16_kernel, dim3(lo_dp_blocks((n + 3) / 4)), dim3(256), 0, st, wire, g, n, inv_scale);
  LO_LAUNCH_CHECK("dp_unpack_f16");
  return LO_OK;
}
int lo_dp_unpack_f16_sumsq_run(const f16* wire, float* g, size_t n, float inv_scale, float* scratch, hipStream_t st) {
  LoProfScope _p("lo_dp_unpack_f16(+sumsq)", 0, 6.0 * n, st);
  hipLaunchKernelGGL(lo_dp_unpack_f16_sumsq_kernel, dim3(LO_NORM_BLOCKS / 2), dim3(256), 0, st, wire, g, n, inv_scale, scratch + LO_NORM_BLOCKS / 2);
  LO_LAUNCH_CHECK("dp_unpack_f16_sumsq");
  return LO_OK;
}
int lo_dp_sum_shares_run(const void* recv, void* share, int world, size_t chunk, int is_f16, float inv_world, hipStream_t st) {
  LoProfScope _p("lo_dp_sum_shares", 0, (is_f16 ? 2.0 : 4.0) * (world + 1) * chunk, st);
  if (is_f16) hipLaunchKernelGGL((lo_dp_sum_shares_kernel<f16>), dim3(lo_dp_blocks(chunk)), dim3(256), 0, st, (const f16*)recv, (f16*)share, world, chunk, inv_world);
  else hipLaunchKernelGGL((lo_dp_sum_shares_kernel<float>), dim3(lo_dp_blocks(chunk)), dim3(256), 0, st, (const float*)recv, (float*)share, world, chunk, inv_world);
  LO_LAUNCH_CHECK("dp_sum_shares");
  return LO_OK;
}

struct LoAmaxJobs { const float* p[5]; size_t n[5]; };
__global__ __launch_bounds__(256) void lo_amax_partial_kernel(LoAmaxJobs J, float* __restrict__ partial) {
  __shared__ float red[4];
  float a = 0.f;
#pragma unroll
  for (int j = 0; j < 5; ++j) {
    const float* g = J.p[j];
    if (!g) continue;
    const size_t n = J.n[j], n4 = n / 4;
    for (size_t k = (size_t)blockIdx.x * 256 + threadIdx.x; k < n4; k += (size_t)gridDim.x * 256) {
      const f32x4 v = reinterpret_cast<const f32x4*>(g)[k];
      a = fmaxf(a, fmaxf(fmaxf(fabsf(v[0]), fabsf(v[1])), fmaxf(fabsf(v[2]), fabsf(v[3]))));
    }
    if (blockIdx.x == 0 && threadIdx.x == 0)
      for (size_t k = n4 * 4; k < n; ++k) a = fmaxf(a, fabsf(g[k]));
  }
#pragma unroll
  for (int o = 32; o > 0; o >>= 1) a = fmaxf(a, __shfl_xor(a, o, 64));
  if ((threadIdx.x & 63) == 0) red[threadIdx.x >> 6] = a;
  __syncthreads();
  if (threadIdx.x == 0) partial[blockIdx.x] = fmaxf(fmaxf(red[0], red[1]), fmaxf(red[2], red[3]));
}
__global__ __launch_bounds__(256) void lo_amax_finalize_kernel(const float* __restrict__ partial, int n, float* __restrict__ out2) {
  __shared__ float red[4];
  float a = 0.f;
  for (int i = threadIdx.x; i < n; i += 256) a = fmaxf(a, partial[i]);
#pragma unroll
  for (int o = 32; o > 0; o >>= 1) a = fmaxf(a, __shfl_xor(a, o, 64));
  if ((threadIdx.x & 63) == 0) red[threadIdx.x >> 6] = a;
  __syncthreads();
  if (threadIdx.x == 0) {
    a = fmaxf(fmaxf(red[0], red[1]), fmaxf(red[2], red[3]));
    float r = 1.0f;
    if (a > 0.f && isfinite(a)) {
      int e;
      (void)frexpf(a, &e);
      e = e > 100 ? 100 : (e < -100 ? -100 : e);
      r = ldexpf(1.0f, 2 - e);
    }
    out2[0] = r;
    out2[1] = 1.0f / r;
    out2[2] = a;
  }
}
__global__ __launch_bounds__(256) void lo_scale_copy_dev_kernel(const float* __restrict__ src, float* __restrict__ dst, size_t n,
                                                                const float* __restrict__ scale) {
  const float s = scale[0];
  const size_t n4 = n / 4;
  for (size_t k = (size_t)blockIdx.x * 256 + threadIdx.x; k < n4; k += (size_t)gridDim.x * 256) {
    f32x4 v = reinterpret_cast<const f32x4*>(src)[k];
    v *= s;
    reinterpret_cast<f32x4*>(dst)[k] = v;
  }
  if (blockIdx.x == 0 && threadIdx.x == 0)
    for (size_t k = n4 * 4; k < n; ++k) dst[k] = src[k] * s;
}
__global__ __launch_bounds__(256) void lo_scale_dev_kernel(float* __restrict__ x, size_t n, const float* __restrict__ scale,
                                                           const unsigned int* __restrict__ fail) {
  const float s = (fail && *fail != 0u) ? __builtin_nanf("") : scale[0];
  const size_t n4 = n / 4;
  for (size_t k = (size_t)blockIdx.x * 256 + threadIdx.x; k < n4; k += (size_t)gridDim.x * 256) {
    f32x4 v = reinterpret_cast<f32x4*>(x)[k];
    v *= s;
    reinterpret_cast<f32x4*>(x)[k] = v;
  }
  if (blockIdx.x == 0 && threadIdx.x == 0)
    for (size_t k = n4 * 4; k < n; ++k) x[k] *= s;
}
static inline int lo_stream_blocks(size_t n) {
  size_t b = (n / 4 + 255) / 256;
  return (int)(b < 1 ? 1 : (b > 1024 ? 1024 : b));
}
int lo_grad_scale_pick_run(const float* const g[5], const size_t n[5], float* scratch , hipStream_t st) {
  LoAmaxJobs J;
  size_t total = 0;
  for (int j = 0; j < 5; ++j) { J.p[j] = g[j]; J.n[j] = g[j] ? n[j] : 0; total += J.n[j]; }
  size_t want = (total / 4 + 255) / 256;
  const int nb = (int)(want < 1 ? 1 : (want > 256 ? 256 : want));
  hipLaunchKernelGGL(lo_amax_partial_kernel, dim3(nb), dim3(256), 0, st, J, scratch + 4);
  LO_LAUNCH_CHECK("amax_partial");
  hipLaunchKernelGGL(lo_amax_finalize_kernel, dim3(1), dim3(256), 0, st, scratch + 4, nb, scratch);
  LO_LAUNCH_CHECK("amax_finalize");
  return LO_OK;
}
int lo_scale_copy_dev_run(const float* src, float* dst, size_t n, const float* scale_dev, hipStream_t st) {
  hipLaunchKernelGGL(lo_scale_copy_dev_kernel, dim3(lo_stream_blocks(n)), dim3(256), 0, st, src, dst, n, scale_dev);
  LO_LAUNCH_CHECK("scale_copy_dev");
  return LO_OK;
}
int lo_scale_dev_run(float* x, size_t n, const float* scale_dev, const unsigned int* fail, hipStream_t st) {
  hipLaunchKernelGGL(lo_scale_dev_kernel, dim3(lo_stream_blocks(n)), dim3(256), 0, st, x, n, scale_dev, fail);
  LO_LAUNCH_CHECK("scale_dev");
  return LO_OK;
}
```

lunaris_orion_amd/csrc/lo_vae.h:

```cpp
#pragma once
#include "lo_internal.h"
#include "lo_conv.h"
#include "lo_norm.h"
#include "../../include/lunaris_hip.h"
#include <stdio.h>
#include <string.h>
#include <stdlib.h>
#include <vector>

#define WSP(T, off) reinterpret_cast<T*>(reinterpret_cast<unsigned char*>(ws) + (off))
#define PRM(i) (P + h->p_off[(i)])
#define GRD(i) (G + h->p_off[(i)])

struct ConvLayer {
  int kind = 0;
  int H = 0, W = 0, Cin = 0, Cout = 0;
  int Ho = 0, Wo = 0;
  LoGeom gf{}, gd{};
  int p_w = 0, p_b = 0, p_gw = 0, p_gb = 0;
  size_t o_wp_f = 0, o_wp_d = 0;
  size_t o_v = 0, o_a = 0;
  size_t o_part = 0, o_stats = 0;
  size_t o_P1 = 0, o_P2 = 0;
  int prow_cap = 0, np1 = 0, np2 = 0;
  int MT = 0;
  size_t o_dv = 0;
  bool f8 = false;
  size_t o_wp8 = 0, o_wscale = 0, o_a8 = 0;
  bool gnf = false; int gnf_mts = 0, gnf_nt = 0;
  size_t o_xbuf = 0, o_xcnt = 0;
  unsigned gnf_epoch = 0;
  size_t o_bcnt = 0;
  unsigned gba_epoch = 0;
  bool dv_done = false;
  hipEvent_t ev_ready = nullptr;
  int sk_fwd = 0, sk_dgrad = 0;
};

struct LoVae {
  int B = 0, L = 0;
  int nparam = 0;
  std::vector<size_t> p_off, p_numel;
  size_t flat_elems = 0;
  ConvLayer enc[4][3];
  ConvLayer dec[4];
  size_t o_eout[4] = {};
  size_t o_skipin[3] = {};
  LoGeom g_head{}, g_head_d{}, g_dfc{}, g_dfc_d{};
  int head_split = 32, dfcd_split = 32;
  size_t o_wp_head = 0, o_wp_head_t = 0, o_wp_dfc = 0, o_wp_dfc_t = 0;
  size_t o_xflat = 0, o_slab_head = 0, o_eps = 0, o_z = 0, o_klp = 0, o_mu = 0, o_lv = 0, o_yfc = 0, o_h0 = 0;
  size_t o_msep = 0, o_losses = 0, o_coefs = 0;
  size_t o_G[6] = {}, o_skipg[3] = {}, o_P1 = 0, o_P2 = 0, o_wslab = 0, o_wslab_lin = 0, o_fcw_part = 0, o_lc_part = 0, o_dz = 0, o_dml = 0,
         o_slab_dz = 0, o_gfc = 0;
  size_t o_packjobs = 0;
  std::vector<LoPackJob> packjobs_host;
  int n_packjobs = 0, pack_blocks = 0;
  int n_packjobs_enc = 0, pack_blocks_enc = 0;
  const void* packjobs_for_ws = nullptr;
  const void* packjobs_for_params = nullptr;
  size_t ws_bytes = 0;
  int idx_fc_mu_w = 0, idx_fc_mu_b = 0, idx_fc_lv_w = 0, idx_fc_lv_b = 0, idx_dfc_w = 0, idx_dfc_b = 0, idx_final_w = 0, idx_final_b = 0;
  bool forward_done = false, loss_done = false;
  bool enc_done = false, dec_done = false;
  int dec_skips = 0;
  hipStream_t side = nullptr;
  hipEvent_t ev_dv[4] = {}, ev_join = nullptr, ev_pre = nullptr, ev_range = nullptr;
  bool async_handover = false, range_pending = false;
  hipEvent_t ev_lvl[6] = {};
  bool lvl_pending[6] = {};
  struct { bool pending = false; float* P; const float* G; float* M; float* V; void* ws; const float* norm; float lr, beta1, beta2, eps, wd; int step; } defer;
  int n_packjobs_s4 = 0, pack_blocks_s4 = 0, n_packjobs8_s4 = 0, pack_blocks8_s4 = 0;
  int bwd_layer = 0;
  size_t o_skslab = 0;
  bool gn_local = true;
  int nevent = 0;
  bool overlap = false;
  float* norm_scratch = nullptr;
  bool fuse_gnb = true;
  bool fuse_gnf = false;
  bool fuse_gna = true;
  size_t o_sync_fail = 0;
  bool lin_factored = false, fac_ready = false;
  bool lin_factored_dp = false;
  int Bp = 0;
  size_t o_fac_dmlT = 0, o_fac_xT = 0, o_fac_gfcT = 0, o_fac_zT = 0, o_gram = 0;
  float fac_scale = 1.f;
  int n_cu = 0;
  const void* sync_for_ws = nullptr;
  bool fp8_fwd = false;
  size_t o_eout8[4] = {}, o_h08 = 0, o_packjobs8 = 0;
  std::vector<LoPackF8Job> packjobs8_host;
  int n_packjobs8 = 0, pack_blocks8 = 0;
  int n_packjobs8_enc = 0, pack_blocks8_enc = 0;
};

template <typename H, typename F>
static inline void for_each_layer(H* h, F&& fn) {
  for (int s = 0; s < 4; ++s)
    for (int k = 0; k < 3; ++k) fn(h->enc[s][k]);
  for (int s = 0; s < 4; ++s) fn(h->dec[s]);
}

static inline LoGnLayer vae_gn_layer(const LoVae* h, const ConvLayer& c, const float* P, void* ws) {
  return {WSP(f16, c.o_v), WSP(float, c.o_stats), PRM(c.p_gw), PRM(c.p_gb), h->B, c.Ho * c.Wo, c.Cout};
}
static inline int vae_record_rows(ConvLayer& c, LoGnRows r) {
  LO_REQUIRE(r.p1 <= c.prow_cap && r.p2 <= c.prow_cap, "GroupNorm backward %dx%dx%d: %d / %d rows of P1 / P2 per sample, room for %d",
             c.Ho, c.Wo, c.Cout, r.p1, r.p2, c.prow_cap);
  if (r.p1 > 0) c.np1 = r.p1;
  if (r.p2 > 0) c.np2 = r.p2;
  return LO_OK;
}

static inline bool vae_side_on(const LoVae* h) { return h->overlap && !g_lo_prof_on; }
static inline int vae_order(hipStream_t behind, hipStream_t ahead, hipEvent_t e) {
  LO_HIP(hipEventRecord(e, ahead));
  LO_HIP(hipStreamWaitEvent(behind, e, 0));
  return LO_OK;
}
static inline bool lo_event_marker() {
  static const bool on = getenv("LO_EVENT_MARKER") != nullptr;
  return on;
}
struct LoHandover {
  hipEvent_t ev = nullptr;
  LoHandover(hipEvent_t e, bool on) { if (on) { ev = e; if (!lo_event_marker()) g_lo_stop_event = e; } }
  LoHandover(LoVae* h, bool on) : LoHandover(on ? h->ev_dv[h->nevent & 3] : nullptr, on) { if (on) ++h->nevent; }
  ~LoHandover() { g_lo_stop_event = nullptr; }
  int finish(hipStream_t st) {
    if (ev && (g_lo_stop_event || lo_event_marker())) {
      g_lo_stop_event = nullptr;
      LO_HIP(hipEventRecord(ev, st));
    }
    return LO_OK;
  }
};

struct LoProfTag {
  template <typename... A>
  explicit LoProfTag(const char* fmt, A... a) {
    if (!(g_lo_prof_on && g_lo_prof_layers)) return;
    char text[64];
    snprintf(text, sizeof(text), fmt, a...);
    g_lo_prof_tag = lo_prof_intern(text);
  }
  void end() { g_lo_prof_tag = nullptr; }
  ~LoProfTag() { end(); }
};

int vae_flush_deferred(LoVae* h, hipStream_t after_main);
int vae_wait_level(LoVae* h, hipStream_t st, int lvl);
```

lunaris_orion_amd/csrc/lo_vae_plan.hip:

```cpp
#include "lo_vae.h"
#include <memory>

namespace {
struct Arena {
  size_t off = 0;
  size_t take(size_t bytes) {
    size_t o = off;
    off += (bytes + 255) & ~(size_t)255;
    return o;
  }
};
bool env_is_zero(const char* v) { return v && atoi(v) == 0; }
const int kEncCh[5] = {3, 64, 128, 256, 512};
const int kDecCh[5] = {512, 256, 128, 64, 32};
}

static int setup_conv_layer(ConvLayer& c, int kind, int B, int H, int W, int Cin, int Cout, int p_w, Arena& ar, bool first) {
  c.kind = kind; c.H = H; c.W = W; c.Cin = Cin; c.Cout = Cout;
  c.p_w = p_w; c.p_b = p_w + 1; c.p_gw = p_w + 2; c.p_gb = p_w + 3;
  if (!first) {
    LO_TRY(lo_make_geom(&c.gf, kind, B, H, W, Cin, Cout));
    int dk = kind == LO_CONV3_S1 ? LO_CONV3_S1_DGRAD : (kind == LO_CONV3_S2 ? LO_CONV3_S2_DGRAD : LO_CONVT4_S2_DGRAD);
    c.Ho = c.gf.Hout; c.Wo = c.gf.Wout;
    LO_TRY(lo_make_geom(&c.gd, dk, B, c.Ho, c.Wo, Cout, Cin));
    c.o_wp_f = ar.take(lo_packed_weight_elems(c.gf) * 2);
    c.o_wp_d = ar.take(lo_packed_weight_elems(c.gd) * 2);
    c.MT = lo_conv_choose(c.gf, {.bias = true, .gn_partial = true}).mts;
  } else {
    c.Ho = H / 2; c.Wo = W / 2;
    c.MT = 64;
  }
  size_t act = (size_t)B * c.Ho * c.Wo * Cout * 2;
  c.o_v = ar.take(act);
  c.o_a = ar.take(act);
  c.o_part = ar.take((size_t)B * c.MT * 16 * 4);
  c.o_stats = ar.take((size_t)B * 16 * 4);
  int nchunk = lo_gn_nchunk(c.Ho * c.Wo, Cout);
  c.prow_cap = nchunk > (c.Ho * c.Wo) / 64 ? nchunk : (c.Ho * c.Wo) / 64;
  c.o_P1 = ar.take((size_t)B * c.prow_cap * Cout * 2 * 4);
  c.o_P2 = ar.take((size_t)B * c.prow_cap * Cout * 4);
  c.o_dv = ar.take(act);
  c.o_xbuf = ar.take((size_t)B * LO_GNF_MAX_TILES * 128);
  c.o_xcnt = ar.take((size_t)B * 4);
  c.o_bcnt = ar.take((size_t)B * 8 * 4);
  return LO_OK;
}

static int plan_parameters(LoVae* h) {
  const int L = h->L;
  std::vector<size_t>& numel = h->p_numel;
  for (int s = 0; s < 4; ++s) {
    size_t ci = kEncCh[s], co = kEncCh[s + 1];
    numel.push_back(co * ci * 9); numel.push_back(co); numel.push_back(co); numel.push_back(co);
    for (int k = 0; k < 2; ++k) { numel.push_back(co * co * 9); numel.push_back(co); numel.push_back(co); numel.push_back(co); }
  }
  h->idx_fc_mu_w = (int)numel.size(); numel.push_back((size_t)L * 32768);
  h->idx_fc_mu_b = (int)numel.size(); numel.push_back(L);
  h->idx_fc_lv_w = (int)numel.size(); numel.push_back((size_t)L * 32768);
  h->idx_fc_lv_b = (int)numel.size(); numel.push_back(L);
  h->idx_dfc_w = (int)numel.size(); numel.push_back((size_t)32768 * L);
  h->idx_dfc_b = (int)numel.size(); numel.push_back(32768);
  const int dec_first = (int)numel.size();
  for (int s = 0; s < 4; ++s) {
    size_t ci = kDecCh[s], co = kDecCh[s + 1];
    numel.push_back(ci * co * 16); numel.push_back(co); numel.push_back(co); numel.push_back(co);
  }
  h->idx_final_w = (int)numel.size(); numel.push_back(3 * 32 * 9);
  h->idx_final_b = (int)numel.size(); numel.push_back(3);
  h->nparam = (int)numel.size();
  h->p_off.assign(h->nparam, 0);
  size_t off = 0;
  auto place = [&](int i) { h->p_off[i] = off; off += (numel[i] + 63) & ~(size_t)63; };
  for (int i = 0; i < h->nparam; ++i) {
    if (i == h->idx_fc_mu_b || i == h->idx_fc_lv_w || i == h->idx_fc_lv_b) continue;
    place(i);
    if (i == h->idx_fc_mu_w) { place(h->idx_fc_lv_w); place(h->idx_fc_mu_b); place(h->idx_fc_lv_b); }
  }
  h->flat_elems = off;
  return dec_first;
}

static int plan_forward_buffers(LoVae* h, Arena& ar, int dec_first) {
  const int B = h->B, L = h->L;
  int Hs = 128;
  int pidx = 0;
  for (int s = 0; s < 4; ++s) {
    int ci = kEncCh[s], co = kEncCh[s + 1];
    LO_TRY(setup_conv_layer(h->enc[s][0], LO_CONV3_S2, B, Hs, Hs, ci, co, pidx, ar, s == 0));
    pidx += 4;
    Hs /= 2;
    LO_TRY(setup_conv_layer(h->enc[s][1], LO_CONV3_S1, B, Hs, Hs, co, co, pidx, ar, false));
    pidx += 4;
    LO_TRY(setup_conv_layer(h->enc[s][2], LO_CONV3_S1, B, Hs, Hs, co, co, pidx, ar, false));
    pidx += 4;
    h->o_eout[s] = ar.take((size_t)B * Hs * Hs * co * 2);
  }
  Hs = 8;
  for (int s = 0; s < 4; ++s) {
    LO_TRY(setup_conv_layer(h->dec[s], LO_CONVT4_S2, B, Hs, Hs, kDecCh[s], kDecCh[s + 1], dec_first + 4 * s, ar, false));
    Hs *= 2;
  }
  for (int k = 0; k < 3; ++k) h->o_skipin[k] = ar.take((size_t)B * (64 >> k) * (64 >> k) * (64 << k) * 2);
  LO_TRY(lo_make_geom(&h->g_head, LO_LINEAR, B, 1, 1, 32768, 2 * L));
  LO_TRY(lo_make_geom(&h->g_head_d, LO_LINEAR, B, 1, 1, 2 * L, 32768));
  LO_TRY(lo_make_geom(&h->g_dfc, LO_LINEAR, B, 1, 1, L, 32768));
  LO_TRY(lo_make_geom(&h->g_dfc_d, LO_LINEAR, B, 1, 1, 32768, L));
  h->o_wp_head = ar.take((size_t)2 * L * 32768 * 2);
  h->o_wp_head_t = ar.take((size_t)2 * L * 32768 * 2);
  h->o_wp_dfc = ar.take((size_t)L * 32768 * 2);
  h->o_wp_dfc_t = ar.take((size_t)L * 32768 * 2);
  h->o_xflat = ar.take((size_t)B * 32768 * 2);
  h->o_slab_head = ar.take((size_t)h->head_split * B * 2 * L * 4);
  h->o_eps = ar.take((size_t)B * L * 4);
  h->o_mu = ar.take((size_t)B * L * 4);
  h->o_lv = ar.take((size_t)B * L * 4);
  h->o_z = ar.take((size_t)B * L * 2);
  h->o_klp = ar.take((size_t)((B * L + 255) / 256) * 4);
  h->o_yfc = ar.take((size_t)B * 32768 * 2);
  h->o_h0 = ar.take((size_t)B * 32768 * 2);
  h->o_msep = ar.take((size_t)B * 64 * 4);
  h->o_losses = ar.take(16 * 4);
  h->o_coefs = ar.take(16 * 4);
  return LO_OK;
}

static void plan_backward_buffers(LoVae* h, Arena& ar) {
  const int B = h->B, L = h->L;
  size_t max_act = (size_t)B * 128 * 128 * 32 * 2;
  for (int i = 0; i < 4; ++i) h->o_G[i] = ar.take(max_act);
  h->o_skipg[0] = ar.take((size_t)B * 64 * 64 * 64 * 2);
  h->o_skipg[1] = ar.take((size_t)B * 32 * 32 * 128 * 2);
  h->o_skipg[2] = ar.take((size_t)B * 16 * 16 * 256 * 2);
  h->o_P1 = ar.take((size_t)B * 64 * 512 * 2 * 4);
  h->o_P2 = ar.take((size_t)B * 64 * 512 * 4);
  size_t wslab = 0;
  for_each_layer(h, [&](ConvLayer& c) {
    if (&c == &h->enc[0][0]) return;
    size_t b = lo_wgrad_slab_bytes(c.gf);
    wslab = b > wslab ? b : wslab;
  });
  h->o_wslab = ar.take(wslab);
  size_t b = lo_wgrad_slab_bytes(h->g_head), b2 = lo_wgrad_slab_bytes(h->g_dfc);
  h->o_wslab_lin = ar.take(b > b2 ? b : b2);
  h->o_fcw_part = ar.take((size_t)B * 16 * 1728 * 4);
  h->o_lc_part = ar.take((size_t)B * 64 * 867 * 4);
  h->o_dz = ar.take((size_t)B * L * 2);
  h->o_dml = ar.take((size_t)B * 2 * L * 2);
  h->o_gfc = ar.take((size_t)B * 32768 * 2);
  h->o_slab_dz = ar.take((size_t)h->dfcd_split * B * L * 4);
  h->o_packjobs = ar.take(sizeof(LoPackJob) * 64);
  h->o_sync_fail = ar.take(256);
  h->Bp = lo_lowrank_bp(B);
  h->o_fac_dmlT = ar.take((size_t)2 * L * h->Bp * 2);
  h->o_fac_xT = ar.take((size_t)32768 * h->Bp * 2);
  h->o_fac_gfcT = ar.take((size_t)32768 * h->Bp * 2);
  h->o_fac_zT = ar.take((size_t)L * h->Bp * 2);
  h->o_gram = ar.take((size_t)2 * 128 * 128 * 4);
}

static void plan_splitk_and_fp8(LoVae* h, Arena& ar) {
  const int B = h->B;
  size_t slab = 0;
  if (!env_is_zero(getenv("LO_SPLITK_CONV")) && !h->fp8_fwd)
    for_each_layer(h, [&](ConvLayer& c) {
      if (&c == &h->enc[0][0]) return;
      c.sk_fwd = lo_conv_splitk_plan(c.gf);
      c.sk_dgrad = lo_conv_splitk_plan(c.gd);
      const size_t bf = (size_t)c.sk_fwd * B * c.gf.GH * c.gf.GW * c.gf.Cout * 4, bd = (size_t)c.sk_dgrad * B * c.gd.GH * c.gd.GW * c.gd.Cout * 4;
      slab = bf > slab ? bf : slab;
      slab = bd > slab ? bd : slab;
    });
  h->o_skslab = ar.take(slab > 0 ? slab : 256);
  if (!h->fp8_fwd) return;
  auto enable = [&](ConvLayer& c, size_t* producer_copy) {
    if (lo_conv_choose(c.gf, {.bias = true, .gn_partial = true, .f8 = true}).kernel == LO_CK_NONE) return;
    if (lo_conv_choose(c.gf, {.bias = true, .gn_partial = true}).kernel == LO_CK_CONVT4_PATCH) return;
    c.f8 = true;
    c.o_wp8 = ar.take(lo_packed_weight_elems(c.gf));
    c.o_wscale = ar.take((size_t)c.gf.n_phase * c.Cout * 4);
    if (!*producer_copy) *producer_copy = ar.take((size_t)B * c.H * c.W * c.Cin);
  };
  for (int s = 0; s < 4; ++s) {
    if (s > 0) enable(h->enc[s][0], &h->o_eout8[s - 1]);
    enable(h->enc[s][1], &h->enc[s][0].o_a8);
    enable(h->enc[s][2], &h->enc[s][1].o_a8);
  }
  enable(h->dec[0], &h->o_h08);
  for (int s = 1; s < 4; ++s) enable(h->dec[s], &h->dec[s - 1].o_a8);
  h->o_packjobs8 = ar.take(sizeof(LoPackF8Job) * 32);
}

static void plan_gn_fusions(LoVae* h) {
  h->fuse_gnb = !env_is_zero(getenv("LO_GNB_FUSE"));
  h->gn_local = !env_is_zero(getenv("LO_GN_LOCAL"));
  h->fuse_gnf = getenv("LO_GN_FUSE") && atoi(getenv("LO_GN_FUSE")) != 0 && !h->fp8_fwd;
  h->fuse_gna = h->fuse_gnb && !env_is_zero(getenv("LO_GNB_APPLY_FUSE"));
  int dev = 0, ncu = 0;
  if (hipGetDevice(&dev) == hipSuccess && hipDeviceGetAttribute(&ncu, hipDeviceAttributeMultiprocessorCount, dev) == hipSuccess) h->n_cu = ncu;
  else (void)hipGetLastError();
  if (h->n_cu < 256) h->fuse_gnf = false;
  for_each_layer(h, [&](ConvLayer& c) {
    if (!h->fuse_gnf || &c == &h->enc[0][0] || c.sk_fwd) return;
    const LoConvChoice ch = lo_conv_choose(c.gf, {.bias = true, .gf = true});
    c.gnf = ch.gn_fuse; c.gnf_mts = ch.mts; c.gnf_nt = ch.nt;
  });
}

static void create_side_stream(LoVae* h) {
  h->overlap = getenv("LO_NO_OVERLAP") == nullptr;
  if (!h->overlap) return;
  int prio_least = 0, prio_greatest = 0;
  bool ok;
  if (hipDeviceGetStreamPriorityRange(&prio_least, &prio_greatest) == hipSuccess && prio_least != prio_greatest)
    ok = hipStreamCreateWithPriority(&h->side, hipStreamNonBlocking, prio_least) == hipSuccess;
  else
    ok = hipStreamCreateWithFlags(&h->side, hipStreamNonBlocking) == hipSuccess;
  constexpr unsigned evf = hipEventDisableTiming | hipEventDisableSystemFence;
  for (int i = 0; i < 4 && ok; ++i)
    ok = hipEventCreateWithFlags(&h->ev_dv[i], evf) == hipSuccess;
  ok = ok && hipEventCreateWithFlags(&h->ev_range, hipEventDisableTiming) == hipSuccess;
  ok = ok && hipEventCreateWithFlags(&h->ev_join, evf) == hipSuccess &&
       hipEventCreateWithFlags(&h->ev_pre, evf) == hipSuccess;
  for (int l = 1; l < 6 && ok; ++l) ok = hipEventCreateWithFlags(&h->ev_lvl[l], evf) == hipSuccess;
  if (!ok) { (void)hipGetLastError(); h->overlap = false; }
}

extern "C" int lo_vae_create(int B, int L, LoVae** out) { return lo_vae_create_ex(B, L, 0u, out); }

extern "C" int lo_vae_create_ex(int B, int L, unsigned flags, LoVae** out) {
  LO_REQUIRE(out, "lo_vae_create: null out");
  LO_REQUIRE((flags & ~(unsigned)LO_VAE_FP8_FWD) == 0, "lo_vae_create_ex: unknown flag bits 0x%x", flags);
  LO_REQUIRE(B >= 1 && B <= 4096, "lo_vae_create: batch %d out of range", B);
  LO_REQUIRE(L >= 64 && L % 64 == 0 && L <= 4096, "lo_vae_create: latent_dim %d must be a multiple of 64", L);
  std::unique_ptr<LoVae> h(new LoVae());
  h->B = B; h->L = L;
  h->fp8_fwd = (flags & LO_VAE_FP8_FWD) != 0;
  Arena ar;
  LO_TRY(plan_forward_buffers(h.get(), ar, plan_parameters(h.get())));
  plan_backward_buffers(h.get(), ar);
  plan_splitk_and_fp8(h.get(), ar);
  h->ws_bytes = ar.off;
  plan_gn_fusions(h.get());
  create_side_stream(h.get());
  *out = h.release();
  return LO_OK;
}

extern "C" void lo_vae_destroy(LoVae* h) {
  if (!h) return;
  if (h->overlap) {
    (void)vae_flush_deferred(h, nullptr);
    (void)hipStreamDestroy(h->side);
    for (int i = 0; i < 4; ++i) (void)hipEventDestroy(h->ev_dv[i]);
    (void)hipEventDestroy(h->ev_join); (void)hipEventDestroy(h->ev_pre); (void)hipEventDestroy(h->ev_range);
    for (int l = 1; l < 6; ++l) (void)hipEventDestroy(h->ev_lvl[l]);
  }
  delete h;
}
extern "C" int lo_vae_set_gradnorm_scratch(LoVae* h, float* scratch) {
  LO_REQUIRE(h, "lo_vae_set_gradnorm_scratch: null handle");
  h->norm_scratch = scratch;
  return LO_OK;
}
extern "C" int lo_vae_gradnorm_presummed(const LoVae* h) { return h && h->norm_scratch && (vae_side_on(h) || h->lin_factored); }
extern "C" int lo_vae_set_linear_factored(LoVae* h, int on) {
  LO_REQUIRE(h, "lo_vae_set_linear_factored: null handle");
  LO_REQUIRE(on >= 0 && on <= 2, "lo_vae_set_linear_factored: mode must be 0 (off), 1 (single process) or 2 (data parallel: factors only)");
  if (on) LO_REQUIRE(lo_lowrank_applies(h->B, 2 * h->L, 32768) && lo_lowrank_applies(h->B, 32768, h->L),
                     "lo_vae_set_linear_factored: batch %d is above the rank the factored update is built for (128)", h->B);
  h->lin_factored = on == 1;
  h->lin_factored_dp = on == 2;
  h->fac_ready = false;
  return LO_OK;
}
extern "C" int lo_vae_factor_block(const LoVae* h, size_t* byte_offset, size_t* bytes) {
  LO_REQUIRE(h && byte_offset && bytes, "lo_vae_factor_block: null argument");
  *byte_offset = h->o_fac_dmlT;
  *bytes = h->o_gram - h->o_fac_dmlT;
  return LO_OK;
}
extern "C" int lo_vae_materialize_gathered_linear_grads(LoVae* h, const void* gathered, int world, float* G, void* stream) {
  LO_REQUIRE(h && gathered && G && world >= 1, "lo_vae_materialize_gathered_linear_grads: bad argument");
  hipStream_t st = S(stream);
  const int L = h->L;
  const size_t blk = (h->o_gram - h->o_fac_dmlT) / 2;
  const f16* base = reinterpret_cast<const f16*>(gathered);
  const float sc = h->fac_scale / (float)world;
  LO_TRY(lo_lowrank_materialize_gathered(G + h->p_off[h->idx_fc_mu_w], base + (h->o_fac_xT - h->o_fac_dmlT) / 2, base, blk, world, 2 * L, 32768, h->B, sc, st));
  return lo_lowrank_materialize_gathered(G + h->p_off[h->idx_dfc_w], base + (h->o_fac_zT - h->o_fac_dmlT) / 2, base + (h->o_fac_gfcT - h->o_fac_dmlT) / 2,
                                         blk, world, 32768, L, h->B, sc, st);
}
extern "C" int lo_vae_linear_factored(const LoVae* h) { return h && h->lin_factored ? 1 : 0; }
extern "C" int lo_vae_num_params(const LoVae* h) { return h->nparam; }
extern "C" size_t lo_vae_param_offset(const LoVae* h, int i) { return (i >= 0 && i < h->nparam) ? h->p_off[i] : (size_t)-1; }
extern "C" size_t lo_vae_param_numel(const LoVae* h, int i) { return (i >= 0 && i < h->nparam) ? h->p_numel[i] : 0; }
extern "C" size_t lo_vae_flat_elems(const LoVae* h) { return h->flat_elems; }
extern "C" size_t lo_vae_workspace_bytes(const LoVae* h) { return h->ws_bytes; }

extern "C" int lo_vae_debug_tensor(const LoVae* h, int which, int s, int k, size_t* byte_offset, int* dims4) {
  LO_REQUIRE(h && byte_offset && dims4 && s >= 0 && s < 4 && k >= 0 && k < 3, "lo_vae_debug_tensor: bad argument");
  const ConvLayer* c = which == 0 ? &h->enc[s][k] : ((which == 1 || which == 3) ? &h->dec[s] : (which == 2 ? &h->enc[s][2] : nullptr));
  LO_REQUIRE(c, "lo_vae_debug_tensor: unknown tensor kind %d", which);
  *byte_offset = which == 2 ? h->o_eout[s] : (which == 3 ? c->o_a : c->o_v);
  dims4[0] = h->B; dims4[1] = c->Ho; dims4[2] = c->Wo; dims4[3] = c->Cout;
  return LO_OK;
}

extern "C" int lo_vae_sync_fail_word(const LoVae* h, size_t* byte_offset, int* fused_layers) {
  LO_REQUIRE(h && byte_offset, "lo_vae_sync_fail_word: null argument");
  *byte_offset = h->o_sync_fail;
  if (fused_layers) {
    int n = 0;
    for_each_layer(h, [&](const ConvLayer& c) { n += c.gnf ? 1 : 0; });
    *fused_layers = n;
  }
  return LO_OK;
}

extern "C" int lo_vae_set_async_handover(LoVae* h, int on) {
  LO_REQUIRE(h, "lo_vae_set_async_handover: null handle");
  h->async_handover = on != 0;
  return LO_OK;
}
extern "C" int lo_vae_wait_handover(LoVae* h, void* stream) {
  LO_REQUIRE(h, "lo_vae_wait_handover: null handle");
  if (h->range_pending) {
    LO_HIP(hipStreamWaitEvent(S(stream), h->ev_range, 0));
    h->range_pending = false;
  }
  return LO_OK;
}
extern "C" int lo_gradnorm_early_range(const float* flat_grads, size_t begin, size_t end, float* scratch, void* stream) {
  LO_REQUIRE(flat_grads && scratch && end > begin, "lo_gradnorm_early_range: bad argument");
  return lo_sumsq_range(flat_grads, begin, end, scratch, S(stream));
}

extern "C" int lo_vae_fp8_layers(const LoVae* h, int* layers) {
  LO_REQUIRE(h && layers, "lo_vae_fp8_layers: null argument");
  int n = 0;
  for_each_layer(h, [&](const ConvLayer& c) { n += c.f8 ? 1 : 0; });
  *layers = n;
  return LO_OK;
}
extern "C" int lo_vae_linear_grad_range(const LoVae* h, size_t* begin, size_t* end) {
  LO_REQUIRE(h && begin && end, "lo_vae_linear_grad_range: null argument");
  *begin = h->p_off[h->idx_fc_mu_w];
  *end = h->p_off[h->idx_dfc_b] + ((h->p_numel[h->idx_dfc_b] + 63) & ~(size_t)63);
  return LO_OK;
}

extern "C" int lo_vae_phase1_grad_range(const LoVae* h, size_t* begin, size_t* end) {
  LO_REQUIRE(h && begin && end, "lo_vae_phase1_grad_range: null argument");
  *begin = h->p_off[h->idx_fc_mu_w];
  *end = h->flat_elems;
  return LO_OK;
}

extern "C" int lo_vae_stage4_grad_range(const LoVae* h, size_t* begin, size_t* end) {
  LO_REQUIRE(h && begin && end, "lo_vae_stage4_grad_range: null argument");
  *begin = h->p_off[h->enc[3][0].p_w];
  *end = h->p_off[h->idx_fc_mu_w];
  return LO_OK;
}
```

lunaris_orion_amd/csrc/lo_vae_step.hip:

```cpp
#include "lo_vae.h"

static int vae_ensure_sync_init(LoVae* h, void* ws, hipStream_t st) {
  if (h->sync_for_ws == ws) return LO_OK;
  hipError_t e = hipSuccess;
  for_each_layer(h, [&](ConvLayer& c) {
    if (e == hipSuccess) e = hipMemsetAsync(WSP(void, c.o_xcnt), 0, (size_t)h->B * 4, st);
    if (e == hipSuccess) e = hipMemsetAsync(WSP(void, c.o_bcnt), 0, (size_t)h->B * 8 * 4, st);
    c.gnf_epoch = 0; c.gba_epoch = 0;
  });
  LO_HIP(e);
  LO_HIP(hipMemsetAsync(WSP(void, h->o_sync_fail), 0, 256, st));
  h->sync_for_ws = ws;
  return LO_OK;
}

static int conv_gn(LoVae* h, ConvLayer& c, const f16* in, const f16* other, f16* y, int mode, const float* P, void* ws,
                   hipStream_t st, size_t o_in8 = 0, size_t o_y8 = 0) {
  LoProfTag tag("fwd kind%d %dx%d %d->%d", c.kind, c.Ho, c.Wo, c.gf.Cin, c.gf.Cout);
  if (c.sk_fwd && !c.f8 && !o_y8) {
    LO_TRY(lo_conv_run(c.gf, {.in = in, .w = WSP(f16, c.o_wp_f), .slab = WSP(float, h->o_skslab), .nsplit = c.sk_fwd}, st));
    tag.end();
    return lo_gn_forward(vae_gn_layer(h, c, P, ws),
                         {.slab = WSP(float, h->o_skslab), .nsplit = c.sk_fwd, .bias = PRM(c.p_b), .other = other, .mode = mode, .y = y}, st);
  }
  const bool fuse = c.gnf && !c.f8 && !o_y8;
  LoGnFuse gf;
  if (fuse) {
    memset(&gf, 0, sizeof(gf));
    gf.xbuf = WSP(float, c.o_xbuf); gf.counter = WSP(unsigned int, c.o_xcnt);
    gf.MTs = c.gnf_mts; gf.NT = c.gnf_nt;
    gf.target = (++c.gnf_epoch) * (unsigned)(c.gnf_mts * c.gnf_nt);
    gf.gamma = PRM(c.p_gw); gf.beta = PRM(c.p_gb); gf.other = other; gf.y = y; gf.stats = WSP(float, c.o_stats); gf.mode = mode;
    gf.fail = WSP(unsigned int, h->o_sync_fail);
  }
  int r_;
  if (c.f8) {
    LO_REQUIRE(o_in8, "fp8 mode: no e4m3 copy of the input of a conv %d->%d", c.Cin, c.Cout);
    r_ = lo_conv_run_f8(c.gf, WSP(uint8_t, o_in8), WSP(uint8_t, c.o_wp8), WSP(float, c.o_wscale),
                        {.bias = PRM(c.p_b), .out = WSP(f16, c.o_v), .gn_partial = WSP(float, c.o_part)}, st);
  } else {
    r_ = lo_conv_run(c.gf, {.in = in, .w = WSP(f16, c.o_wp_f), .bias = PRM(c.p_b), .out = WSP(f16, c.o_v),
                            .gn_partial = fuse ? nullptr : WSP(float, c.o_part), .gf = fuse ? &gf : nullptr}, st);
  }
  tag.end();
  if (r_ != LO_OK) { if (fuse) --c.gnf_epoch; return r_; }
  if (fuse) return LO_OK;
  return lo_gn_forward(vae_gn_layer(h, c, P, ws), {.partial = WSP(float, c.o_part), .MT = c.MT, .other = other, .mode = mode, .y = y,
                                                   .y8 = o_y8 ? WSP(uint8_t, o_y8) : nullptr}, st);
}

static int vae_decoder_forward(LoVae* h, const f16* const skips[3], const float* P, void* ws, float* recon, const float* target,
                               hipStream_t st) {
  const int B = h->B;
  LO_TRY(vae_ensure_sync_init(h, ws, st));
  LO_TRY(vae_wait_level(h, st, 4));
  LO_TRY(lo_conv_run(h->g_dfc, {.in = WSP(f16, h->o_z), .w = WSP(f16, h->o_wp_dfc), .bias = PRM(h->idx_dfc_b), .out = WSP(f16, h->o_yfc)}, st));
  LO_TRY(lo_nchw_to_nhwc_f16(WSP(f16, h->o_yfc), WSP(f16, h->o_h0), B, 64, 512, st, h->o_h08 ? WSP(uint8_t, h->o_h08) : nullptr));
  const f16* cur = WSP(f16, h->o_h0);
  size_t cur8 = h->o_h08;
  for (int s = 0; s < 4; ++s) {
    ConvLayer& c = h->dec[s];
    const f16* skip = s < 3 ? skips[2 - s] : nullptr;
    LO_TRY(conv_gn(h, c, cur, skip, WSP(f16, c.o_a), skip ? 1 : 0, P, ws, st, cur8, c.o_a8));
    cur = WSP(f16, c.o_a);
    cur8 = c.o_a8;
  }
  h->dec_done = true;
  h->dec_skips = (skips[0] ? 1 : 0) + (skips[1] ? 1 : 0) + (skips[2] ? 1 : 0);
  return lo_final_conv_fwd(cur, PRM(h->idx_final_w), PRM(h->idx_final_b), target, recon, target ? WSP(float, h->o_msep) : nullptr,
                           B, st);
}

static int vae_encoder_forward(LoVae* h, const float* x, const float* eps, uint64_t seed, const float* P, void* ws, float* mu,
                               float* logvar, hipStream_t st);

extern "C" int lo_vae_forward(LoVae* h, const float* x, const float* eps, uint64_t seed, const float* P, void* ws,
                              float* recon, float* mu, float* logvar, const float* target, void* stream) {
  LO_REQUIRE(h && x && P && ws && recon && mu && logvar, "lo_vae_forward: null argument");
  hipStream_t st = S(stream);
  LO_TRY(vae_encoder_forward(h, x, eps, seed, P, ws, mu, logvar, st));
  const f16* skips[3] = {WSP(f16, h->o_eout[0]), WSP(f16, h->o_eout[1]), WSP(f16, h->o_eout[2])};
  LO_TRY(vae_decoder_forward(h, skips, P, ws, recon, target, st));
  h->forward_done = true;
  h->loss_done = false;
  return LO_OK;
}

static int vae_encoder_forward(LoVae* h, const float* x, const float* eps, uint64_t seed, const float* P, void* ws, float* mu,
                               float* logvar, hipStream_t st) {
  const int B = h->B, L = h->L;
  LO_TRY(vae_ensure_sync_init(h, ws, st));
  const f16* cur = nullptr;
  size_t cur8 = 0;
  for (int s = 0; s < 4; ++s) {
    ConvLayer& c0 = h->enc[s][0];
    ConvLayer& c1 = h->enc[s][1];
    ConvLayer& c2 = h->enc[s][2];
    if (s == 0) {
      LO_TRY(lo_first_conv_fwd(x, PRM(c0.p_w), PRM(c0.p_b), WSP(f16, c0.o_v), WSP(float, c0.o_part), B, st));
      LO_TRY(lo_gn_forward(vae_gn_layer(h, c0, P, ws), {.partial = WSP(float, c0.o_part), .MT = c0.MT, .y = WSP(f16, c0.o_a),
                                                        .y8 = c0.o_a8 ? WSP(uint8_t, c0.o_a8) : nullptr}, st));
      LO_TRY(vae_wait_level(h, st, 1));
    } else {
      if (s == 3) LO_TRY(vae_wait_level(h, st, 2));
      LO_TRY(conv_gn(h, c0, cur, nullptr, WSP(f16, c0.o_a), 0, P, ws, st, cur8, c0.o_a8));
    }
    LO_TRY(conv_gn(h, c1, WSP(f16, c0.o_a), nullptr, WSP(f16, c1.o_a), 0, P, ws, st, c0.o_a8, c1.o_a8));
    LO_TRY(conv_gn(h, c2, WSP(f16, c1.o_a), WSP(f16, c0.o_a), WSP(f16, h->o_eout[s]), 2, P, ws, st, c1.o_a8, h->o_eout8[s]));
    cur = WSP(f16, h->o_eout[s]);
    cur8 = h->o_eout8[s];
  }
  LO_TRY(lo_nhwc_to_nchw_f16(cur, WSP(f16, h->o_xflat), B, 64, 512, st));
  LO_TRY(vae_wait_level(h, st, 3));
  LO_TRY(lo_conv_run(h->g_head, {.in = WSP(f16, h->o_xflat), .w = WSP(f16, h->o_wp_head), .slab = WSP(float, h->o_slab_head), .nsplit = h->head_split}, st));
  LO_REQUIRE(h->p_off[h->idx_fc_lv_b] == h->p_off[h->idx_fc_mu_b] + (size_t)L, "flat layout: head biases not adjacent");
  LO_TRY(lo_head_reduce(WSP(float, h->o_slab_head), PRM(h->idx_fc_mu_b), eps, seed, WSP(float, h->o_mu), WSP(float, h->o_lv),
                        WSP(f16, h->o_z), WSP(float, h->o_eps), WSP(float, h->o_klp), B, L, h->head_split, st, mu, logvar));
  h->enc_done = true;
  return LO_OK;
}

extern "C" int lo_vae_encode(LoVae* h, const float* x, const float* P, void* ws, float* mu, float* logvar, float* skip0, float* skip1,
                             float* skip2, void* stream) {
  LO_REQUIRE(h && x && P && ws && mu && logvar, "lo_vae_encode: null argument");
  hipStream_t st = S(stream);
  LO_TRY(vae_encoder_forward(h, x, nullptr, 0, P, ws, mu, logvar, st));
  float* sk[3] = {skip0, skip1, skip2};
  for (int k = 0; k < 3; ++k)
    if (sk[k]) LO_TRY(lo_nhwc_f16_to_nchw_f32(WSP(f16, h->o_eout[k]), sk[k], h->B, (64 >> k) * (64 >> k), 64 << k, 1.0f, st));
  h->forward_done = false;
  return LO_OK;
}

extern "C" int lo_vae_decode_skips(LoVae* h, const float* z, int n_skips, const float* skip0, const float* skip1, const float* skip2,
                                   const float* P, void* ws, float* recon, void* stream) {
  LO_REQUIRE(h && z && P && ws && recon && n_skips >= 0 && n_skips <= 3, "lo_vae_decode_skips: bad argument");
  const float* sk[3] = {skip0, skip1, skip2};
  for (int k = 0; k < n_skips; ++k) LO_REQUIRE(sk[k], "lo_vae_decode_skips: skip %d is NULL but n_skips = %d", k, n_skips);
  hipStream_t st = S(stream);
  LO_TRY(lo_cast_f32_f16(z, WSP(f16, h->o_z), (size_t)h->B * h->L, st));
  const f16* skips[3] = {nullptr, nullptr, nullptr};
  for (int k = 0; k < n_skips; ++k) {
    LO_TRY(lo_nchw_f32_to_nhwc_f16(sk[k], WSP(f16, h->o_skipin[k]), h->B, (64 >> k) * (64 >> k), 64 << k, 1.0f, st));
    skips[k] = WSP(f16, h->o_skipin[k]);
  }
  LO_TRY(vae_decoder_forward(h, skips, P, ws, recon, nullptr, st));
  h->forward_done = false;
  return LO_OK;
}

extern "C" int lo_vae_decode(LoVae* h, const float* z, const float* P, void* ws, float* recon, void* stream) {
  LO_REQUIRE(h && z && P && ws && recon, "lo_vae_decode: null argument");
  hipStream_t st = S(stream);
  LO_TRY(lo_cast_f32_f16(z, WSP(f16, h->o_z), (size_t)h->B * h->L, st));
  const f16* skips[3] = {nullptr, nullptr, nullptr};
  LO_TRY(vae_decoder_forward(h, skips, P, ws, recon, nullptr, st));
  h->forward_done = false;
  return LO_OK;
}

extern "C" int lo_vae_loss(LoVae* h, void* ws, float recon_weight, float kl_weight, float mean_advantage, const float* adv_dev,
                           float accum, float loss_scale, float* losses_dev, void* stream) {
  LO_REQUIRE(h && ws && losses_dev, "lo_vae_loss: null argument");
  if (!h->forward_done) { lo_set_error("lo_vae_loss: no forward with a target has run"); return LO_ERR_STATE; }
  hipStream_t st = S(stream);
  const int B = h->B, L = h->L;
  LO_TRY(lo_loss_finalize(WSP(float, h->o_msep), B * 64, WSP(float, h->o_klp), (B * L + 255) / 256, recon_weight, kl_weight,
                          mean_advantage, adv_dev, accum, loss_scale, losses_dev, WSP(float, h->o_coefs),
                          (float)B * 3.f * 128.f * 128.f, (float)B * (float)L, st));
  h->loss_done = true;
  return LO_OK;
}

static int vae_gn_finalize(LoVae* h, unsigned enc_mask, bool dec, float* G, void* ws, float inv, hipStream_t st) {
  const int B = h->B;
  LoGnFinJobs jobs;
  jobs.n = 0;
  int blocks = 0;
  bool rows_ok = true;
  auto add = [&](ConvLayer& c) {
    LoGnFinJob& j = jobs.j[jobs.n++];
    j.P1 = WSP(float, c.o_P1); j.P2 = WSP(float, c.o_P2);
    j.dgamma = GRD(c.p_gw); j.dbeta = GRD(c.p_gb); j.dbias = GRD(c.p_b);
    rows_ok = rows_ok && c.np1 > 0 && c.np2 > 0;
    j.nblk1 = B * c.np1; j.nblk2 = B * c.np2;
    j.C = c.Cout; j.block0 = blocks;
    blocks += (c.Cout + 3) / 4;
  };
  for (int s = 0; s < 4; ++s)
    if (enc_mask & (1u << s)) for (int k = 0; k < 3; ++k) add(h->enc[s][k]);
  if (dec) for (int s = 0; s < 4; ++s) add(h->dec[s]);
  LO_REQUIRE(rows_ok, "GroupNorm finalize: a layer's backward has not run (no P1 / P2 rows recorded)");
  return lo_gn_finalize_all(jobs, inv, st);
}

struct LoGapTable { unsigned long long off[80]; int len[80]; int n; };
__global__ void lo_zero_gaps_kernel(float* G, LoGapTable t) {
  const int i = blockIdx.x;
  if (i < t.n && (int)threadIdx.x < t.len[i]) G[t.off[i] + threadIdx.x] = 0.f;
}
static int vae_zero_gaps(LoVae* h, float* G, hipStream_t st) {
  LoGapTable t;
  t.n = 0;
  LO_REQUIRE(h->nparam <= 80, "gap table too small");
  for (int i = 0; i < h->nparam; ++i) {
    const size_t n = h->p_numel[i], padded = (n + 63) & ~(size_t)63;
    if (padded > n) { t.off[t.n] = h->p_off[i] + n; t.len[t.n] = (int)(padded - n); ++t.n; }
  }
  if (t.n == 0) return LO_OK;
  hipLaunchKernelGGL(lo_zero_gaps_kernel, dim3(t.n), dim3(64), 0, st, G, t);
  LO_LAUNCH_CHECK("zero_gaps");
  return LO_OK;
}

namespace {
struct VaeBackward {
  LoVae* h; const float* P; float* G; void* ws; float loss_scale; hipStream_t st;
  float inv;
  bool side;
  f16 *Ga, *Gb, *Gc, *Gd;
  VaeBackward(LoVae* h_, const float* P_, float* G_, void* ws_, float loss_scale_, void* stream)
      : h(h_), P(P_), G(G_), ws(ws_), loss_scale(loss_scale_), st(S(stream)), inv(1.0f / loss_scale_), side(vae_side_on(h_)),
        Ga(WSP(f16, h_->o_G[0])), Gb(WSP(f16, h_->o_G[1])), Gc(WSP(f16, h_->o_G[2])), Gd(WSP(f16, h_->o_G[3])) {}

  int begin(bool first_call);
  int gn_backward(ConvLayer& c, const LoGnBwd& op);
  int layer(ConvLayer& c, const f16* dy, const f16* other, int mode, const f16* layer_in, f16* ds, f16* din, const f16* add_src,
            ConvLayer* prod = nullptr, bool din_has_other_readers = false);
  int dgrad_splitk(ConvLayer& c, int k, const f16* dv, f16* din, const f16* add_src, ConvLayer& prod, bool din_has_other_readers);
  int dgrad(ConvLayer& c, int k, const f16* dv, f16* din, const f16* add_src, ConvLayer* prod, bool din_has_other_readers);
  int decoder_chain(int fused, const float* recon, const float* target, const float* drecon, bool fac, float* dz32);
  int latent_and_heads(int fused, const float* gmu, const float* glv, bool fac, bool beside, bool hand_to_side);
  int early_norm(bool fac1);
  int encoder_stages(int s_hi, int s_lo, const float* x, float* dx);
  int finalize(unsigned enc_mask, bool dec, hipStream_t on) { return vae_gn_finalize(h, enc_mask, dec, G, ws, inv, on); }
  int publish_range(unsigned enc_mask, bool dec);
  int join() { return side ? vae_order(st, h->side, h->ev_join) : LO_OK; }
};

int VaeBackward::begin(bool first_call) {
  LO_TRY(vae_wait_level(h, st, 5));
  if (!first_call) return LO_OK;
  h->bwd_layer = 0;
  for_each_layer(h, [](ConvLayer& c) { c.np1 = 0; c.dv_done = false; c.np2 = 0; c.ev_ready = nullptr; });
  return LO_OK;
}

int VaeBackward::gn_backward(ConvLayer& c, const LoGnBwd& op_in) {
  LoGnBwd op = op_in;
  op.P1 = WSP(float, c.o_P1); op.P2 = WSP(float, c.o_P2);
  op.rows_in_P1 = c.np1; op.allow_local = h->gn_local;
  LO_TRY(vae_record_rows(c, lo_gn_bwd_choose(c.Ho * c.Wo, c.Cout, lo_gn_use(op)).rows));
  return lo_gn_backward(vae_gn_layer(h, c, P, ws), op, st);
}

int VaeBackward::layer(ConvLayer& c, const f16* dy, const f16* other, int mode, const f16* layer_in, f16* ds, f16* din,
                       const f16* add_src, ConvLayer* prod, bool din_has_other_readers) {
  const int k = h->bwd_layer++;
  f16* dv = WSP(f16, c.o_dv);
  hipEvent_t ready = nullptr;
  if (c.dv_done) { ready = c.ev_ready; c.ev_ready = nullptr; }
  else {
    LoHandover ho(h, side);
    LO_TRY(gn_backward(c, {.dy = dy, .other = other, .mode = mode, .ds = ds, .dv = dv}));
    LO_TRY(ho.finish(st));
    ready = ho.ev;
  }
  {
    if (side && ready) LO_HIP(hipStreamWaitEvent(h->side, ready, 0));
    else if (side) LO_TRY(vae_order(h->side, st, h->ev_dv[(h->nevent++) & 3]));
    LoProfTag tag("wgrad L%02d kind%d %dx%d %d->%d", k, c.kind, c.Ho, c.Wo, c.gf.Cin, c.gf.Cout);
    LO_TRY(lo_wgrad_run(c.gf, layer_in, dv, WSP(float, h->o_wslab), GRD(c.p_w), inv, side ? h->side : st));
  }
  if (!din) return LO_OK;
  if (prod && c.sk_dgrad && lo_gn_bwd_choose(prod->Ho * prod->Wo, prod->Cout, {.slab = true}).form == LO_GNB_SLAB_LOCAL)
    return dgrad_splitk(c, k, dv, din, add_src, *prod, din_has_other_readers);
  return dgrad(c, k, dv, din, add_src, prod, din_has_other_readers);
}

int VaeBackward::dgrad_splitk(ConvLayer& c, int k, const f16* dv, f16* din, const f16* add_src, ConvLayer& prod, bool din_has_other_readers) {
  {
    LoProfTag tag("dgrad L%02d kind%d %dx%d %d->%d", k, c.kind, c.Ho, c.Wo, c.gd.Cin, c.gd.Cout);
    LO_TRY(lo_conv_run(c.gd, {.in = dv, .w = WSP(f16, c.o_wp_d), .slab = WSP(float, h->o_skslab), .nsplit = c.sk_dgrad}, st));
  }
  LoHandover ho(h, side);
  LO_TRY(gn_backward(prod, {.slab = WSP(float, h->o_skslab), .nsplit = c.sk_dgrad, .add_src = add_src,
                            .dy_out = din_has_other_readers ? din : nullptr, .dv = WSP(f16, prod.o_dv)}));
  LO_TRY(ho.finish(st));
  prod.ev_ready = ho.ev;
  prod.dv_done = true;
  return LO_OK;
}

int VaeBackward::dgrad(ConvLayer& c, int k, const f16* dv, f16* din, const f16* add_src, ConvLayer* prod, bool din_has_other_readers) {
  LoGnBwdFuse gb, *gbp = nullptr;
  if (prod && h->fuse_gnb) {
    gb.v = WSP(f16, prod->o_v); gb.stats = WSP(float, prod->o_stats); gb.gamma = PRM(prod->p_gw); gb.beta = PRM(prod->p_gb);
    gb.P1 = WSP(float, prod->o_P1);
    const LoConvChoice ch = lo_conv_choose(c.gd, {.add = add_src != nullptr, .gb = true, .gb_apply = true});
    const int mts = ch.mts, nt = ch.nt;
    const bool apply = h->fuse_gna && ch.gnb_apply && h->B * mts * nt <= h->n_cu;
    LO_TRY(vae_record_rows(*prod, {mts, apply ? mts : 0}));
    if (apply) {
      gb.dv = WSP(f16, prod->o_dv); gb.P2 = WSP(float, prod->o_P2);
      gb.counter = WSP(unsigned int, prod->o_bcnt);
      gb.target = (++prod->gba_epoch) * (unsigned)mts;
      gb.fail = WSP(unsigned int, h->o_sync_fail);
      gb.keep_out = din_has_other_readers;
      prod->dv_done = true;
    }
    gbp = &gb;
  }
  const bool writes_dv = gbp && gbp->dv;
  LoProfTag tag("dgrad L%02d kind%d %dx%d %d->%d", k, c.kind, c.Ho, c.Wo, c.gd.Cin, c.gd.Cout);
  LoHandover ho(h, side && writes_dv);
  int r_ = lo_conv_run(c.gd, {.in = dv, .w = WSP(f16, c.o_wp_d), .add_src = add_src, .out = din, .gb = gbp}, st);
  if (r_ != LO_OK) { if (writes_dv) { --prod->gba_epoch; prod->dv_done = false; } return r_; }
  if (writes_dv) { LO_TRY(ho.finish(st)); prod->ev_ready = ho.ev; }
  return LO_OK;
}

int VaeBackward::decoder_chain(int fused, const float* recon, const float* target, const float* drecon, bool fac, float* dz32) {
  const int B = h->B, L = h->L;
  if (fused || drecon) {
    LoHandover ho(h, side && !lo_event_marker());
    LO_TRY(lo_final_conv_bwd(WSP(f16, h->dec[3].o_a), PRM(h->idx_final_w), recon, fused ? target : nullptr, fused ? nullptr : drecon,
                             fused ? WSP(float, h->o_coefs) : nullptr, loss_scale, Ga, WSP(float, h->o_lc_part),
                             GRD(h->idx_final_w), GRD(h->idx_final_b), B, inv, st, ho.ev ? h->side : nullptr, ho.ev));
  } else {
    LO_HIP(hipMemsetAsync(Ga, 0, (size_t)B * 128 * 128 * 32 * 2, st));
  }
  const f16* gout = Ga;
  for (int s = 3; s >= 0; --s) {
    const f16* layer_in = s > 0 ? WSP(f16, h->dec[s - 1].o_a) : WSP(f16, h->o_h0);
    f16* din = s > 0 ? WSP(f16, h->o_skipg[3 - s]) : Ga;
    LO_TRY(layer(h->dec[s], gout, nullptr, 0, layer_in, nullptr, din, nullptr, s > 0 ? &h->dec[s - 1] : nullptr, true));
    gout = din;
  }
  hipStream_t gs = side ? h->side : st;
  f16* Gfc = WSP(f16, h->o_gfc);
  {
    LoHandover ho(h, side);
    LO_TRY(lo_nhwc_to_nchw_f16(Ga, Gfc, B, 64, 512, st));
    LO_TRY(ho.finish(st));
    if (side) LO_HIP(hipStreamWaitEvent(h->side, ho.ev, 0));
  }
  LO_TRY(lo_colsum_f16(Gfc, GRD(h->idx_dfc_b), B, 32768, inv, gs));
  if (!fac)
    LO_TRY(lo_wgrad_run(h->g_dfc, WSP(f16, h->o_z), Gfc, WSP(float, h->o_wslab_lin), GRD(h->idx_dfc_w), inv, gs));
  LO_TRY(lo_conv_run(h->g_dfc_d, {.in = Gfc, .w = WSP(f16, h->o_wp_dfc_t), .slab = WSP(float, h->o_slab_dz), .nsplit = h->dfcd_split}, st));
  return lo_splitk_reduce(WSP(float, h->o_slab_dz), nullptr, dz32, WSP(f16, h->o_dz), B, L, h->dfcd_split, st);
}

int VaeBackward::latent_and_heads(int fused, const float* gmu, const float* glv, bool fac, bool beside, bool hand_to_side) {
  const int B = h->B, L = h->L;
  beside = beside && side;
  hipStream_t gs = beside ? h->side : st;
  {
    LoHandover ho(h, beside);
    LO_TRY(lo_latent_bwd(WSP(f16, h->o_dz), WSP(float, h->o_mu), WSP(float, h->o_lv), WSP(float, h->o_eps),
                         fused ? WSP(float, h->o_coefs) : nullptr, fused ? nullptr : gmu, fused ? nullptr : glv, loss_scale,
                         WSP(f16, h->o_dml), B, L, st));
    LO_TRY(ho.finish(st));
    if (beside) LO_HIP(hipStreamWaitEvent(h->side, ho.ev, 0));
  }
  LO_TRY(lo_colsum_f16(WSP(f16, h->o_dml), GRD(h->idx_fc_mu_b), B, 2 * L, inv, gs));
  if (fac) {
    const f16* src[4] = {WSP(f16, h->o_dml), WSP(f16, h->o_xflat), WSP(f16, h->o_gfc), WSP(f16, h->o_z)};
    f16* dst[4] = {WSP(f16, h->o_fac_dmlT), WSP(f16, h->o_fac_xT), WSP(f16, h->o_fac_gfcT), WSP(f16, h->o_fac_zT)};
    const int Cs[4] = {2 * L, 32768, 32768, L};
    LO_TRY(lo_transpose_pad_f16_multi(src, dst, Cs, 4, B, h->Bp, gs));
  } else {
    LO_TRY(lo_wgrad_run(h->g_head, WSP(f16, h->o_xflat), WSP(f16, h->o_dml), WSP(float, h->o_wslab_lin), GRD(h->idx_fc_mu_w), inv, gs));
  }
  LO_TRY(lo_conv_run(h->g_head_d, {.in = WSP(f16, h->o_dml), .w = WSP(f16, h->o_wp_head_t), .out = Gb}, st));
  LoHandover ho(h->ev_pre, beside && hand_to_side);
  LO_TRY(lo_nchw_to_nhwc_f16(Gb, Ga, B, 64, 512, st));
  LO_TRY(ho.finish(st));
  if (ho.ev) LO_HIP(hipStreamWaitEvent(h->side, ho.ev, 0));
  return LO_OK;
}

int VaeBackward::early_norm(bool fac1) {
  const int L = h->L;
  hipStream_t ns = side ? h->side : st;
  LO_TRY(finalize(0u, true, ns));
  if (!fac1) return lo_sumsq_range(G, h->p_off[h->idx_fc_mu_w], h->flat_elems, h->norm_scratch, ns);
  const size_t bh = h->p_off[h->idx_fc_mu_w], nh = (size_t)2 * L * 32768, bd = h->p_off[h->idx_dfc_w], nd = (size_t)32768 * L;
  float* sc = h->norm_scratch;
  LO_TRY(lo_sumsq_blocks(G + bd + nd, h->flat_elems - (bd + nd), sc + 512, 255, ns));
  LO_TRY(lo_sumsq_blocks(G + bh + nh, bd - (bh + nh), sc + 767, 1, ns));
  const LoLowrankNorm nl[2] = {{WSP(f16, h->o_dml), 2 * L, WSP(f16, h->o_xflat), 32768, WSP(float, h->o_gram), sc + 768, 128},
                               {WSP(f16, h->o_z), L, WSP(f16, h->o_gfc), 32768, WSP(float, h->o_gram) + 128 * 128, sc + 896, 128}};
  LO_TRY(lo_lowrank_sumsq(nl, 2, h->B, inv, ns));
  h->fac_scale = inv;
  h->fac_ready = true;
  return LO_OK;
}

int VaeBackward::encoder_stages(int s_hi, int s_lo, const float* x, float* dx) {
  const int B = h->B;
  for (int s = s_hi; s >= s_lo; --s) {
    ConvLayer& c0 = h->enc[s][0];
    ConvLayer& c1 = h->enc[s][1];
    ConvLayer& c2 = h->enc[s][2];
    LO_TRY(layer(c2, Ga, WSP(f16, c0.o_a), 2, WSP(f16, c1.o_a), Gb, Gd, nullptr, &c1));
    LO_TRY(layer(c1, Gd, nullptr, 0, WSP(f16, c0.o_a), nullptr, Gc, Gb, &c0));
    if (s > 0) {
      LO_TRY(layer(c0, Gc, nullptr, 0, WSP(f16, h->o_eout[s - 1]), nullptr, Ga, WSP(f16, h->o_skipg[s - 1])));
      continue;
    }
    const f16* dv0 = Gd;
    if (c0.dv_done) dv0 = WSP(f16, c0.o_dv);
    else
      LO_TRY(gn_backward(c0, {.dy = Gc, .dv = Gd}));
    LO_TRY(lo_first_conv_wgrad(x, dv0, WSP(float, h->o_fcw_part), GRD(c0.p_w), B, inv, st));
    if (dx) LO_TRY(lo_image_dgrad(dv0, 64, 2, PRM(c0.p_w), B, inv, dx, st));
  }
  return LO_OK;
}

int VaeBackward::publish_range(unsigned enc_mask, bool dec) {
  LO_TRY(finalize(enc_mask, dec, h->side));
  LO_HIP(hipEventRecord(h->ev_range, h->side));
  h->range_pending = true;
  return LO_OK;
}

int vae_backward_checks(const LoVae* h, bool args_ok, bool fwd_ran, int fused, const float* target, float loss_scale) {
  LO_REQUIRE(args_ok, "lo_vae_backward: null argument");
  if (!fwd_ran) { lo_set_error("lo_vae_backward: the forward this backward belongs to has not run"); return LO_ERR_STATE; }
  if (fused && (!h->loss_done || !target)) { lo_set_error("lo_vae_backward: fused mode needs lo_vae_loss and a target"); return LO_ERR_STATE; }
  LO_REQUIRE(loss_scale > 0.f, "lo_vae_backward: loss_scale must be positive");
  return LO_OK;
}
}

extern "C" int lo_vae_backward_dx(LoVae* h, const float* x, const float* P, void* ws, const float* recon, const float* target,
                                  int fused, const float* drecon, const float* gmu, const float* glv, float loss_scale,
                                  float* G, float* dx, void* stream) {
  const bool args_ok = h && P && ws && G && x && recon;
  LO_TRY(vae_backward_checks(h, args_ok, args_ok && h->forward_done, fused, target, loss_scale));
  VaeBackward b(h, P, G, ws, loss_scale, stream);
  LO_TRY(b.begin(true));
  const bool fac1 = h->lin_factored && fused;
  if (fac1 && !h->norm_scratch) { lo_set_error("lo_vae_backward: the factored Linear-gradient mode needs lo_vae_set_gradnorm_scratch"); return LO_ERR_STATE; }
  h->fac_ready = false;
  const bool early = h->norm_scratch && (b.side || fac1);
  LO_TRY(vae_zero_gaps(h, G, (b.side && fused) ? h->side : b.st));
  LO_TRY(b.decoder_chain(fused, recon, target, drecon, fac1, nullptr));
  LO_TRY(b.latent_and_heads(fused, gmu, glv, fac1, true, h->norm_scratch != nullptr));
  if (early) LO_TRY(b.early_norm(fac1));
  LO_TRY(b.encoder_stages(3, 0, x, dx));
  LO_TRY(b.finalize(0xFu, !early, b.st));
  return b.join();
}
extern "C" int lo_vae_backward(LoVae* h, const float* x, const float* P, void* ws, const float* recon, const float* target,
                               int fused, const float* drecon, const float* gmu, const float* glv, float loss_scale,
                               float* G, void* stream) {
  return lo_vae_backward_dx(h, x, P, ws, recon, target, fused, drecon, gmu, glv, loss_scale, G, nullptr, stream);
}

extern "C" int lo_vae_backward_phase(LoVae* h, int phase, const float* x, const float* P, void* ws, const float* recon,
                                     const float* target, int fused, const float* drecon, const float* gmu, const float* glv,
                                     float loss_scale, float* G, void* stream) {
  LO_REQUIRE(phase >= 1 && phase <= 4, "lo_vae_backward_phase: phase must be 1 (final conv, decoder, Linear layers), 2 (whole encoder), "
             "3 (encoder stage 4) or 4 (encoder stages 3..1, after 3)");
  const bool args_ok = h && P && ws && G && x && recon;
  LO_TRY(vae_backward_checks(h, args_ok, args_ok && h->forward_done, fused, target, loss_scale));
  VaeBackward b(h, P, G, ws, loss_scale, stream);
  LO_TRY(b.begin(phase == 1));
  const bool async = b.side && h->async_handover;
  if (phase == 1) {
    const bool facdp = h->lin_factored_dp && fused;
    h->fac_ready = false;
    LO_TRY(vae_zero_gaps(h, G, (b.side && fused) ? h->side : b.st));
    LO_TRY(b.decoder_chain(fused, recon, target, drecon, facdp, nullptr));
    LO_TRY(b.latent_and_heads(fused, gmu, glv, facdp, true, async));
    if (facdp) h->fac_scale = b.inv;
    if (async) return b.publish_range(0u, true);
    LO_TRY(b.join());
    return b.finalize(0u, true, b.st);
  }
  LO_TRY(b.encoder_stages(phase == 4 ? 2 : 3, phase == 3 ? 3 : 0, x, nullptr));
  if (phase == 3 && async) {
    LO_TRY(vae_order(h->side, b.st, h->ev_pre));
    return b.publish_range(0x8u, false);
  }
  LO_TRY(b.finalize(phase == 3 ? 0x8u : (phase == 4 ? 0x7u : 0xFu), false, b.st));
  return b.join();
}

extern "C" int lo_vae_decoder_backward(LoVae* h, const float* P, void* ws, const float* recon, const float* drecon, float loss_scale,
                                       float* dz, float* dskip0, float* dskip1, float* dskip2, float* G, void* stream) {
  LO_REQUIRE(h && drecon && dz, "lo_vae_decoder_backward: null argument");
  LO_TRY(vae_backward_checks(h, P && ws && G && recon, h->dec_done, 0, nullptr, loss_scale));
  VaeBackward b(h, P, G, ws, loss_scale, stream);
  const int B = h->B;
  float* dskip[3] = {dskip0, dskip1, dskip2};
  LO_TRY(b.begin(true));
  LO_TRY(vae_zero_gaps(h, G, b.st));
  LO_TRY(b.decoder_chain(0, recon, nullptr, drecon, false, dz));
  LO_TRY(lo_scale_f32(dz, (size_t)B * h->L, b.inv, b.st));
  for (int k = 0; k < 3; ++k)
    if (dskip[k]) LO_TRY(lo_nhwc_f16_to_nchw_f32(WSP(f16, h->o_skipg[k]), dskip[k], B, (64 >> k) * (64 >> k), 64 << k, b.inv, b.st));
  LO_TRY(b.join());
  return b.finalize(0u, true, b.st);
}
extern "C" int lo_vae_encoder_backward_dx(LoVae* h, const float* x, const float* P, void* ws, const float* gmu, const float* glv,
                                          const float* gskip0, const float* gskip1, const float* gskip2, float loss_scale, float* G,
                                          float* dx, void* stream) {
  const bool args_ok = h && P && ws && G && x;
  LO_TRY(vae_backward_checks(h, args_ok, args_ok && h->enc_done, 0, nullptr, loss_scale));
  VaeBackward b(h, P, G, ws, loss_scale, stream);
  const int B = h->B;
  const float* gskip[3] = {gskip0, gskip1, gskip2};
  LO_TRY(b.begin(true));
  LO_TRY(vae_zero_gaps(h, G, b.st));
  for (int k = 0; k < 3; ++k) {
    const size_t n = (size_t)B * (64 >> k) * (64 >> k) * (64 << k);
    if (gskip[k]) LO_TRY(lo_nchw_f32_to_nhwc_f16(gskip[k], WSP(f16, h->o_skipg[k]), B, (64 >> k) * (64 >> k), 64 << k, loss_scale, b.st));
    else LO_HIP(hipMemsetAsync(WSP(f16, h->o_skipg[k]), 0, n * 2, b.st));
  }
  LO_HIP(hipMemsetAsync(WSP(f16, h->o_dz), 0, (size_t)B * h->L * 2, b.st));
  LO_TRY(b.latent_and_heads(0, gmu, glv, false, false, false));
  LO_TRY(b.encoder_stages(3, 0, x, dx));
  LO_TRY(b.finalize(0xFu, false, b.st));
  return b.join();
}
extern "C" int lo_vae_encoder_backward(LoVae* h, const float* x, const float* P, void* ws, const float* gmu, const float* glv,
                                       const float* gskip0, const float* gskip1, const float* gskip2, float loss_scale, float* G,
                                       void* stream) {
  return lo_vae_encoder_backward_dx(h, x, P, ws, gmu, glv, gskip0, gskip1, gskip2, loss_scale, G, nullptr, stream);
}
```

Before: 24790 sprites/s.

## Add streaming linear kernel with NHWC epilogue and fold dz split-K reduce into latent backward

Adds a new weight-streaming linear GEMV-style kernel for small-batch fully connected layers. It can write its output directly in NHWC layout, which would remove the separate NCHW-to-NHWC transpose after the decoder FC and the head dgrad. It also lets the latent backward kernel sum the dz split-K slab itself, so the separate split-K reduce launch is dropped. The streaming kernel is only selected when LO_LINEAR_STREAM>=2, so by default only the slab-reduce fusion runs. That fusion adds a strided multi-split read inside the elementwise kernel.

```diff
diff --git a/include/lunaris_hip.h b/include/lunaris_hip.h
--- a/include/lunaris_hip.h
+++ b/include/lunaris_hip.h
@@ -38,6 +38,12 @@
                                   const float* bias, int leaky_relu, void* out, float* bn_partial, int* rows_out, void* stream);
 int lo_linear_splitk(int M, int K, int N, const void* x, const void* wp, const float* bias, float* slab, int nsplit,
                      float* out32, void* out16, void* stream);
+int lo_linear_forward(int M, int K, int N, const void* x, const void* wp, const float* bias, void* out, int nhwc_hw, void* stream);
+int lo_linear_uses_stream(int M, int K, int N, int nsplit, int nhwc);
+int lo_linear_stream_enable(int mode);
+int lo_nchw_to_nhwc_half(const void* src, void* dst, int B, int HW, int C, void* stream);
+int lo_latent_backward_slab(const float* slab, int nsplit, int fused, void* dz16, const float* mu, const float* logvar, const float* eps,
+                            const float* coefs, const float* gmu, const float* glv, float gscale, void* dml, int B, int L, void* stream);
 size_t lo_wgrad_slab_bytes_for(int kind, int B, int H, int W, int Cin, int Cout);
 int lo_conv_wgrad(int kind, int B, int H, int W, int Cin, int Cout, const void* x, const void* dy, float* slab,
                   float* grad, float scale, void* stream);
diff --git a/lunaris_orion_amd/_lib.py b/lunaris_orion_amd/_lib.py
--- a/lunaris_orion_amd/_lib.py
+++ b/lunaris_orion_amd/_lib.py
@@ -33,6 +33,11 @@
     "lo_conv3x3_fused_tap_forward": (i32, [i32] * 6 + [vp, vp, f32p, f32p, i32, vp, f32p, vp]),
     "lo_teacher_conv3x3_forward_f8": (i32, [i32] * 5 + [vp, vp, f32p, f32p, i32, vp, f32p, C.POINTER(C.c_int), vp]),
     "lo_linear_splitk": (i32, [i32, i32, i32, vp, vp, f32p, f32p, i32, f32p, vp, vp]),
+    "lo_linear_forward": (i32, [i32, i32, i32, vp, vp, f32p, vp, i32, vp]),
+    "lo_linear_uses_stream": (i32, [i32] * 5),
+    "lo_linear_stream_enable": (i32, [i32]),
+    "lo_nchw_to_nhwc_half": (i32, [vp, vp, i32, i32, i32, vp]),
+    "lo_latent_backward_slab": (i32, [f32p, i32, i32, vp, f32p, f32p, f32p, f32p, f32p, f32p, flt, vp, i32, i32, vp]),
     "lo_wgrad_slab_bytes_for": (sz, [i32] * 6),
     "lo_conv_wgrad": (i32, [i32] * 6 + [vp, vp, f32p, f32p, flt, vp]),
     "lo_gn_mish_forward": (i32, [vp, f32p, i32, f32p, f32p, vp, vp, f32p, i32, i32, i32, i32, vp]),
diff --git a/lunaris_orion_amd/build.py b/lunaris_orion_amd/build.py
--- a/lunaris_orion_amd/build.py
+++ b/lunaris_orion_amd/build.py
@@ -7,7 +7,7 @@
 HERE = os.path.dirname(os.path.abspath(__file__))
 CSRC = os.path.join(HERE, "csrc")
 LIB = os.path.join(HERE, "liblunaris_hip.so")
-SOURCES = ["lo_util.cpp", "lo_conv_geom.hip", "lo_igemm.hip", "lo_conv_f8.hip", "lo_conv_select.hip", "lo_conv3.hip", "lo_wgrad.hip", "lo_wgrad3.hip", "lo_wgrad2.hip", "lo_norm.hip", "lo_edge.hip", "lo_imgdgrad.hip", "lo_train.hip", "lo_lowrank.hip", "lo_attn.hip", "lo_teacher_plan.hip", "lo_teacher_kernels.hip", "lo_teacher_f128.hip", "lo_teacher_heads.hip", "lo_teacher_forward.hip", "lo_teacher_bwd_block.hip", "lo_teacher_bwd.hip", "lo_api.hip", "lo_vae_plan.hip", "lo_vae_opt.hip", "lo_vae_step.hip"]
+SOURCES = ["lo_util.cpp", "lo_conv_geom.hip", "lo_igemm.hip", "lo_linear_stream.hip", "lo_conv_f8.hip", "lo_conv_select.hip", "lo_conv3.hip", "lo_wgrad.hip", "lo_wgrad3.hip", "lo_wgrad2.hip", "lo_norm.hip", "lo_edge.hip", "lo_imgdgrad.hip", "lo_train.hip", "lo_lowrank.hip", "lo_attn.hip", "lo_teacher_plan.hip", "lo_teacher_kernels.hip", "lo_teacher_f128.hip", "lo_teacher_heads.hip", "lo_teacher_forward.hip", "lo_teacher_bwd_block.hip", "lo_teacher_bwd.hip", "lo_api.hip", "lo_vae_plan.hip", "lo_vae_opt.hip", "lo_vae_step.hip"]
 HEADERS = ["lo_common.h", "lo_internal.h", "lo_conv.h", "lo_conv_dev.h", "lo_norm.h", "lo_vae.h", "lo_teacher.h", os.path.join("..", "..", "include", "lunaris_hip.h")]
 
 
diff --git a/lunaris_orion_amd/csrc/lo_api.hip b/lunaris_orion_amd/csrc/lo_api.hip
--- a/lunaris_orion_amd/csrc/lo_api.hip
+++ b/lunaris_orion_amd/csrc/lo_api.hip
@@ -82,8 +82,37 @@
                                 int nsplit, float* out32, void* out16, void* stream) {
   LoGeom g;
   LO_TRY(lo_make_geom(&g, LO_LINEAR, M, 1, 1, K, N));
-  LO_TRY(lo_conv_run(g, {.in = (const f16*)x, .w = (const f16*)wp, .slab = slab, .nsplit = nsplit}, S(stream)));
+  LO_TRY(lo_conv_run(g, {.in = (const f16*)x, .w = (const f16*)wp, .slab = slab, .nsplit = nsplit, .lin_stream = g_lo_linear_stream_mode}, S(stream)));
   return lo_splitk_reduce(slab, bias, out32, (f16*)out16, M, N, nsplit, S(stream));
+}
+extern "C" int lo_linear_forward(int M, int K, int N, const void* x, const void* wp, const float* bias, void* out, int nhwc_hw, void* stream) {
+  LoGeom g;
+  LO_TRY(lo_make_geom(&g, LO_LINEAR, M, 1, 1, K, N));
+  return lo_conv_run(g, {.in = (const f16*)x, .w = (const f16*)wp, .bias = bias, .out = (f16*)out, .nhwc_hw = nhwc_hw,
+                         .lin_stream = g_lo_linear_stream_mode}, S(stream));
+}
+extern "C" int lo_linear_uses_stream(int M, int K, int N, int nsplit, int nhwc) {
+  LoGeom g;
+  if (lo_make_geom(&g, LO_LINEAR, M, 1, 1, K, N) != LO_OK) return 0;
+  return lo_conv_choose(g, {.bias = nsplit <= 1, .nsplit = nsplit, .nhwc = nhwc != 0, .lin_stream = g_lo_linear_stream_mode}).kernel == LO_CK_LINEAR_STREAM;
+}
+extern "C" int lo_linear_stream_enable(int mode) {
+  const int was = g_lo_linear_stream_mode;
+  g_lo_linear_stream_mode = mode < 0 ? 0 : (mode > 2 ? 2 : mode);
+  return was;
+}
+extern "C" int lo_nchw_to_nhwc_half(const void* src, void* dst, int B, int HW, int C, void* stream) {
+  return lo_nchw_to_nhwc_f16((const f16*)src, (f16*)dst, B, HW, C, S(stream));
+}
+extern "C" int lo_latent_backward_slab(const float* slab, int nsplit, int fused, void* dz16, const float* mu, const float* logvar, const float* eps,
+                                       const float* coefs, const float* gmu, const float* glv, float gscale, void* dml, int B, int L, void* stream) {
+  LO_REQUIRE(slab && dz16 && mu && logvar && eps && dml && nsplit >= 1, "lo_latent_backward_slab: bad argument");
+  if (!fused) {
+    LO_TRY(lo_splitk_reduce(slab, nullptr, nullptr, (f16*)dz16, B, L, nsplit, S(stream)));
+    return lo_latent_bwd((const f16*)dz16, mu, logvar, eps, coefs, gmu, glv, gscale, (f16*)dml, B, L, S(stream));
+  }
+  const LoLatentSlabSrc src{slab, nsplit, (f16*)dz16};
+  return lo_latent_bwd(nullptr, mu, logvar, eps, coefs, gmu, glv, gscale, (f16*)dml, B, L, S(stream), &src);
 }
 extern "C" size_t lo_wgrad_slab_bytes_for(int kind, int B, int H, int W, int Cin, int Cout) {
   LoGeom g;
diff --git a/lunaris_orion_amd/csrc/lo_conv.h b/lunaris_orion_amd/csrc/lo_conv.h
--- a/lunaris_orion_amd/csrc/lo_conv.h
+++ b/lunaris_orion_amd/csrc/lo_conv.h
@@ -37,6 +37,8 @@
   const LoGnBwdFuse* gb = nullptr;
   const LoConvExtra* ex = nullptr;
   const LoGnFuse* gf = nullptr;
+  int nhwc_hw = 0;
+  int lin_stream = 1;
 };
 struct LoConvUse {
   bool bias = false, gn_partial = false, add = false;
@@ -45,6 +47,8 @@
   bool gf = false;
   int nsplit = 1;
   bool f8 = false;
+  bool nhwc = false;
+  int lin_stream = 1;
 };
 static inline LoConvUse lo_conv_use(const LoConvOp& op) {
   LoConvUse u;
@@ -53,10 +57,12 @@
   u.ex = op.ex != nullptr; u.concat = op.ex && op.ex->out_pitch > 0;
   u.gf = op.gf != nullptr;
   u.nsplit = op.nsplit < 1 ? 1 : op.nsplit;
+  u.nhwc = op.nhwc_hw > 0; u.lin_stream = op.lin_stream;
   return u;
 }
 
-enum LoConvKernel { LO_CK_NONE = 0, LO_CK_IGEMM, LO_CK_IGEMM_SPLITK, LO_CK_IGEMM_F8, LO_CK_CONV3_PP, LO_CK_CONVT4_PATCH, LO_CK_CONVS2D_PATCH };
+enum LoConvKernel { LO_CK_NONE = 0, LO_CK_IGEMM, LO_CK_IGEMM_SPLITK, LO_CK_IGEMM_F8, LO_CK_CONV3_PP, LO_CK_CONVT4_PATCH, LO_CK_CONVS2D_PATCH,
+                    LO_CK_LINEAR_STREAM };
 struct LoConvChoice {
   int kernel;
   int bm, bn, bk;
@@ -69,6 +75,7 @@
   bool gnb_apply;
 };
 LoConvChoice lo_conv_choose(const LoGeom& g, const LoConvUse& use);
+extern int g_lo_linear_stream_mode;
 int lo_conv_splitk_plan(const LoGeom& g);
 int lo_conv_run(const LoGeom& g, const LoConvOp& op, hipStream_t st, LoConvChoice* chosen = nullptr);
 int lo_conv_run_f8(const LoGeom& g, const uint8_t* in8, const uint8_t* w8, const float* wscale, const LoConvOp& op, hipStream_t st,
@@ -78,6 +85,8 @@
 int lo_igemm_run_f8(const LoGeom& g, const uint8_t* in8, const uint8_t* w8, const float* wscale, const LoConvOp& op, const LoConvChoice& c,
                     hipStream_t st);
 int lo_splitk_reduce(const float* slab, const float* bias, float* out32, f16* out16, int M, int N, int nsplit, hipStream_t st);
+
+int lo_linear_stream_run(const LoGeom& g, const LoConvOp& op, const LoConvChoice& c, hipStream_t st);
 
 int lo_conv3_run(const LoGeom& g, const LoConvOp& op, const LoConvChoice& c, hipStream_t st);
 int lo_convt4_patch_run(const LoGeom& g, const LoConvOp& op, const LoConvChoice& c, hipStream_t st);
diff --git a/lunaris_orion_amd/csrc/lo_conv_select.hip b/lunaris_orion_amd/csrc/lo_conv_select.hip
--- a/lunaris_orion_amd/csrc/lo_conv_select.hip
+++ b/lunaris_orion_amd/csrc/lo_conv_select.hip
@@ -102,6 +102,22 @@
   return c;
 }
 
+int g_lo_linear_stream_mode = 1;
+static bool linear_stream_selected(const LoGeom& g, const LoConvUse& u, int* kslice, int* grid) {
+  if (u.lin_stream < 2 || u.f8 || u.add || u.gn_partial || u.gb || u.ex || u.gf) return false;
+  if (g.n_phase != 1 || g.T[0] != 1 || g.Hin != 1 || g.Win != 1 || g.GH != 1 || g.GW != 1 || g.B > 64) return false;
+  const int ns = u.nsplit < 1 ? 1 : u.nsplit;
+  if (g.Cout % 64 || g.Cin % ns) return false;
+  const int ks = g.Cin / ns;
+  if (ks % 256 || ks > 1024 || (long)g.Cin * g.Cout < 64 * 512) return false;
+  if (u.nhwc && ns != 1) return false;
+  const int nsets = g.Cout / 64;
+  int wgs = nsets;
+  if (ns == 1 && wgs > 512) wgs = 512;
+  *kslice = ks; *grid = ns * wgs;
+  return true;
+}
+
 LoConvChoice lo_conv_choose(const LoGeom& g, const LoConvUse& u) {
   if (u.f8) return choose_f8(g);
   LoConvChoice c{};
@@ -109,7 +125,12 @@
   const int per_sample = g.GH * g.GW;
   const bool bare = nsplit == 1 && !u.gb && !u.ex && !u.gf;
   const int tiles16 = (g.Hin / 16) * (g.Win / 16);
-  if (bare && !u.add && convt4_patch_geom(g)) {
+  if (int ks, grid; linear_stream_selected(g, u, &ks, &grid)) {
+    c.kernel = LO_CK_LINEAR_STREAM;
+    c.bm = c.bn = 64; c.bk = ks;
+    c.grid = grid;
+    c.nt = g.Cout / 64;
+  } else if (bare && !u.add && convt4_patch_geom(g)) {
     c.kernel = LO_CK_CONVT4_PATCH;
     set_rows(c, g, tiles16, 1);
     c.grid = g.B * tiles16;
@@ -160,7 +181,9 @@
     LO_REQUIRE(gb->P2 && gb->counter && gb->fail && c.gnb_apply,
                "lo_conv_run: fused GroupNorm-backward apply asked for a geometry the kernel does not support (check LoConvChoice::gnb_apply)");
   LO_REQUIRE(!u.concat || (!u.add && !gb && op.ex->out_pitch % 8 == 0 && op.ex->out_choff % 8 == 0), "lo_conv_run: bad concatenated-output arguments");
+  LO_REQUIRE(!u.nhwc || c.kernel == LO_CK_LINEAR_STREAM, "lo_conv_run: the NHWC epilogue is lo_linear_stream's (check lo_conv_choose first)");
   switch (c.kernel) {
+    case LO_CK_LINEAR_STREAM: return lo_linear_stream_run(g, op, c, st);
     case LO_CK_CONVT4_PATCH: return lo_convt4_patch_run(g, op, c, st);
     case LO_CK_CONVS2D_PATCH: return lo_convs2d_patch_run(g, op, c, st);
     case LO_CK_CONV3_PP: return lo_conv3_run(g, op, c, st);
diff --git a/lunaris_orion_amd/csrc/lo_internal.h b/lunaris_orion_amd/csrc/lo_internal.h
--- a/lunaris_orion_amd/csrc/lo_internal.h
+++ b/lunaris_orion_amd/csrc/lo_internal.h
@@ -27,8 +27,10 @@
 int lo_loss_finalize(const float* mse_partial, int n_mse, const float* kl_partial, int n_kl, float rw, float kw, float adv,
                      const float* adv_dev, float accum, float ls, float* losses, float* coefs, float n_rec, float n_lat,
                      hipStream_t st);
+struct LoLatentSlabSrc { const float* slab; int nsplit; f16* dz_out; };
 int lo_latent_bwd(const f16* dz, const float* mu, const float* logvar, const float* eps, const float* coefs,
-                  const float* gmu, const float* glv, float gscale, f16* dml, int B, int L, hipStream_t st);
+                  const float* gmu, const float* glv, float gscale, f16* dml, int B, int L, hipStream_t st,
+                  const LoLatentSlabSrc* src = nullptr);
 int lo_colsum_f16(const f16* x, float* out, int M, int N, float scale, hipStream_t st);
 int lo_cast_f32_f16(const float* src, f16* dst, size_t n, hipStream_t st);
 int lo_scale_f32(float* x, size_t n, float scale, hipStream_t st);
diff --git a/lunaris_orion_amd/csrc/lo_linear_stream.hip b/lunaris_orion_amd/csrc/lo_linear_stream.hip
--- /dev/null
+++ b/lunaris_orion_amd/csrc/lo_linear_stream.hip
@@ -0,0 +1,204 @@
+#include "lo_conv.h"
+
+struct LinStreamArgs {
+  const f16* x;
+  const f16* w;
+  const float* bias;
+  f16* out;
+  float* slab;
+  int M, K, N;
+  int kslice;
+  int nsets;
+  int wgs;
+  int hw;
+};
+
+#define LS_U 8
+#define LS_BATCH (LS_U * 32)
+#define LS_NB 1
+
+template <int NB>
+struct LsSlot { f16x8 w[NB * LS_U]; f32x4 b; };
+
+template <bool NHWC>
+__global__ __launch_bounds__(256, 2) void lo_linear_stream_kernel(LinStreamArgs a) {
+  constexpr int NB = LS_NB;
+  constexpr int PH = NB * LS_BATCH;
+  constexpr int PITCH = PH * 2 + 16;
+  constexpr int CPR = PH / 8;
+  constexpr int RPP = 256 / CPR;
+  constexpr int XL = 64 / RPP;
+  constexpr int NW = NB * LS_U;
+  extern __shared__ __attribute__((aligned(16))) unsigned char smem[];
+  const int tid = threadIdx.x, lane = tid & 63;
+  const int wave = __builtin_amdgcn_readfirstlane(tid >> 6);
+  const int fr = lane & 15, fq = lane >> 4;
+  const int split = blockIdx.x / a.wgs, g0 = blockIdx.x - split * a.wgs;
+  const int kbase = split * a.kslice;
+  const int MB = (a.M + 15) >> 4;
+  const int nps = a.kslice / PH;
+  const int my_sets = (a.nsets - g0 + a.wgs - 1) / a.wgs;
+  const int total = my_sets * nps;
+  const int cgroups = NHWC ? (a.N / a.hw) >> 4 : 1;
+
+  auto w_row = [&](int s) __attribute__((always_inline)) -> const f16* {
+    int n;
+    if (NHWC) {
+      const int pg = s / cgroups, cg = s - pg * cgroups;
+      n = (cg * 16 + fr) * a.hw + pg * 4 + wave;
+    } else {
+      n = s * 64 + wave * 16 + fr;
+    }
+    return a.w + (size_t)n * a.K + kbase + fq * 8;
+  };
+  const float* const bias0 = a.bias ? a.bias : reinterpret_cast<const float*>(a.w);
+  const int bstride = NHWC ? a.hw : 1;
+  auto b_ptr = [&](int s) __attribute__((always_inline)) -> const float* {
+    if (!a.bias) return bias0;
+    if (NHWC) {
+      const int pg = s / cgroups, cg = s - pg * cgroups;
+      return bias0 + (cg * 16 + fq * 4) * a.hw + pg * 4 + wave;
+    }
+    return bias0 + s * 64 + wave * 16 + fq * 4;
+  };
+  int l_set = g0, l_p = 0, l_left = total;
+  const f16* l_row = w_row(l_set);
+  const float* l_bias = b_ptr(l_set);
+  auto load = [&](LsSlot<NB>& sl) __attribute__((always_inline)) {
+    const bool live = l_left > 0;
+    const f16* p = live ? l_row + l_p * PH : a.w;
+    const int us = live ? 32 : 0;
+#pragma unroll
+    for (int u = 0; u < NW; ++u) sl.w[u] = *reinterpret_cast<const f16x8*>(p + u * us);
+#pragma unroll
+    for (int j = 0; j < 4; ++j) sl.b[j] = l_bias[j * bstride];
+    --l_left;
+    if (++l_p == nps) {
+      l_p = 0;
+      l_set = min(l_set + a.wgs, a.nsets - 1);
+      l_row = w_row(l_set);
+      l_bias = b_ptr(l_set);
+    }
+  };
+  f16x8 xr[XL];
+  int x_p = 0;
+  const int xr0 = tid / CPR, xc = tid - xr0 * CPR;
+  auto xload = [&]() __attribute__((always_inline)) {
+    const f16* base = a.x + kbase + x_p * PH + xc * 8;
+#pragma unroll
+    for (int u = 0; u < XL; ++u) {
+      const int r = xr0 + u * RPP;
+      xr[u] = *reinterpret_cast<const f16x8*>(base + (size_t)min(r, a.M - 1) * a.K);
+      if (r >= a.M) xr[u] = (f16x8){0, 0, 0, 0, 0, 0, 0, 0};
+    }
+    if (++x_p == nps) x_p = 0;
+  };
+  auto xwrite = [&]() __attribute__((always_inline)) {
+#pragma unroll
+    for (int u = 0; u < XL; ++u) {
+      const int r = xr0 + u * RPP;
+      if (r < MB * 16) *reinterpret_cast<f16x8*>(smem + r * PITCH + xc * 16) = xr[u];
+    }
+  };
+
+  LsSlot<NB> s0, s1;
+  load(s0);
+  xload();
+  load(s1);
+
+  f32x4 acc[4];
+#pragma unroll
+  for (int mi = 0; mi < 4; ++mi) acc[mi] = (f32x4){0.f, 0.f, 0.f, 0.f};
+
+  auto epilogue = [&](int s, const f32x4& bv) __attribute__((always_inline)) {
+    int pg = 0, cg = 0;
+    if (NHWC) { pg = s / cgroups; cg = s - pg * cgroups; }
+#pragma unroll
+    for (int mi = 0; mi < 4; ++mi) {
+      const int m = mi * 16 + fr;
+      if (mi < MB && m < a.M) {
+        if (NHWC) {
+          const int c = cg * 16 + fq * 4, p = pg * 4 + wave, C = a.N / a.hw;
+          f16x4 o;
+#pragma unroll
+          for (int j = 0; j < 4; ++j) o[j] = (f16)(acc[mi][j] + (a.bias ? bv[j] : 0.f));
+          *reinterpret_cast<f16x4*>(a.out + ((size_t)m * a.hw + p) * C + c) = o;
+        } else {
+          const int n = s * 64 + wave * 16 + fq * 4;
+          if (a.slab) {
+            *reinterpret_cast<f32x4*>(a.slab + ((size_t)split * a.M + m) * a.N + n) = acc[mi];
+          } else {
+            f16x4 o;
+#pragma unroll
+            for (int j = 0; j < 4; ++j) o[j] = (f16)(acc[mi][j] + (a.bias ? bv[j] : 0.f));
+            *reinterpret_cast<f16x4*>(a.out + (size_t)m * a.N + n) = o;
+          }
+        }
+      }
+      acc[mi] = (f32x4){0.f, 0.f, 0.f, 0.f};
+    }
+  };
+
+  int c_set = g0, c_p = 0;
+  const unsigned char* xrow = smem + fr * PITCH + fq * 16;
+  auto phase = [&](const LsSlot<NB>& sl) __attribute__((always_inline)) {
+#pragma unroll
+    for (int u = 0; u < NW; ++u) {
+#pragma unroll
+      for (int mi = 0; mi < 4; ++mi)
+        if (mi < MB) {
+          const f16x8 xf = *reinterpret_cast<const f16x8*>(xrow + mi * 16 * PITCH + u * 64);
+          acc[mi] = __builtin_amdgcn_mfma_f32_16x16x32_f16(sl.w[u], xf, acc[mi], 0, 0, 0);
+        }
+    }
+    if (++c_p == nps) {
+      epilogue(c_set, sl.b);
+      c_p = 0;
+      c_set += a.wgs;
+    }
+  };
+
+  for (int q = 0; q < total; q += 2) {
+    __syncthreads();
+    xwrite();
+    xload();
+    __syncthreads();
+    phase(s0);
+    load(s0);
+    __syncthreads();
+    if (q + 1 < total) xwrite();
+    xload();
+    __syncthreads();
+    if (q + 1 < total) phase(s1);
+    load(s1);
+  }
+}
+
+template <bool NHWC>
+static int ls_launch(const LinStreamArgs& a, int grid, int lds, hipStream_t st) {
+  LO_LAUNCH_STOP((lo_linear_stream_kernel<NHWC>), dim3(grid), dim3(256), lds, st, a);
+  LO_LAUNCH_CHECK("linear_stream");
+  return LO_OK;
+}
+
+int lo_linear_stream_run(const LoGeom& g, const LoConvOp& op, const LoConvChoice& c, hipStream_t st) {
+  LinStreamArgs a;
+  a.x = op.in; a.w = op.w; a.bias = op.bias; a.out = op.out; a.slab = op.slab;
+  a.M = g.B * g.GH * g.GW; a.K = g.Cin; a.N = g.Cout;
+  const int nsplit = op.nsplit < 1 ? 1 : op.nsplit;
+  a.kslice = c.bk; a.nsets = a.N / 64; a.hw = op.nhwc_hw;
+  LO_REQUIRE(a.M >= 1 && a.M <= 64 && a.N % 64 == 0 && a.kslice * nsplit == a.K && a.kslice % LS_BATCH == 0 && a.kslice <= 1024 &&
+             c.grid % nsplit == 0 && c.grid / nsplit >= 1 && c.grid / nsplit <= a.nsets,
+             "lo_linear_stream: M=%d K=%d N=%d nsplit=%d is not a shape the kernel serves", a.M, a.K, a.N, nsplit);
+  a.wgs = c.grid / nsplit;
+  LO_REQUIRE(op.in && op.w && ((op.slab != nullptr) != (op.out != nullptr)), "lo_linear_stream: one of slab / out");
+  LO_REQUIRE(nsplit == 1 || op.slab, "lo_linear_stream: a K split writes slabs");
+  LO_REQUIRE(!op.slab || (!op.bias && !op.nhwc_hw), "lo_linear_stream: the slab form has no bias and no NHWC epilogue");
+  LO_REQUIRE(!op.nhwc_hw || (op.nhwc_hw % 4 == 0 && a.N % op.nhwc_hw == 0 && (a.N / op.nhwc_hw) % 16 == 0),
+             "lo_linear_stream: NHWC epilogue needs whole sets of 16 channels x 4 pixels");
+  const int lds = ((a.M + 15) / 16) * 16 * (LS_NB * LS_BATCH * 2 + 16);
+  const double out_bytes = op.slab ? 4.0 * nsplit * a.M * a.N : 2.0 * a.M * a.N;
+  LoProfScope _p(lo_prof_geom_name(op.nhwc_hw ? "lo_linear_stream/nhwc" : (op.slab ? "lo_linear_stream/splitK" : "lo_linear_stream"), g),
+                 lo_geom_flops(g), 2.0 * ((double)a.N * a.K + (double)a.M * a.K) + out_bytes, st);
+  return op.nhwc_hw ? ls_launch<true>(a, c.grid, lds, st) : ls_launch<false>(a, c.grid, lds, st);
+}
diff --git a/lunaris_orion_amd/csrc/lo_train.hip b/lunaris_orion_amd/csrc/lo_train.hip
--- a/lunaris_orion_amd/csrc/lo_train.hip
+++ b/lunaris_orion_amd/csrc/lo_train.hip
@@ -1,4 +1,4 @@
-#include "lo_common.h"
+#include "lo_internal.h"
 #include <stdlib.h>
 
 __device__ __forceinline__ uint64_t lo_mix64(uint64_t x) {
@@ -95,12 +95,30 @@
 __global__ void lo_latent_bwd_kernel(const f16* __restrict__ dz, const float* __restrict__ mu, const float* __restrict__ logvar,
                                      const float* __restrict__ eps, const float* __restrict__ coefs,
                                      const float* __restrict__ gmu, const float* __restrict__ glv, float gscale,
-                                     f16* __restrict__ dml, int B, int L) {
+                                     f16* __restrict__ dml, int B, int L, LoLatentSlabSrc ss) {
   int i = blockIdx.x * blockDim.x + threadIdx.x;
   if (i >= B * L) return;
   int b = i / L, l = i - b * L;
   float ckl = coefs ? coefs[1] : 0.f;
-  float d = (float)dz[i];
+  float d;
+  if (ss.slab) {
+    const size_t MN = (size_t)B * L;
+    float v = 0.f;
+    int s = 0;
+    for (; s + 8 <= ss.nsplit; s += 8) {
+      float t[8];
+#pragma unroll
+      for (int u = 0; u < 8; ++u) t[u] = ss.slab[(size_t)(s + u) * MN + i];
+#pragma unroll
+      for (int u = 0; u < 8; ++u) v += t[u];
+    }
+    for (; s < ss.nsplit; ++s) v += ss.slab[(size_t)s * MN + i];
+    const f16 dh = (f16)v;
+    if (ss.dz_out) ss.dz_out[i] = dh;
+    d = (float)dh;
+  } else {
+    d = (float)dz[i];
+  }
   float lv = logvar[i];
   float dm = ckl * mu[i] + d;
   float dl = ckl * 0.5f * (expf(lv) - 1.f) + d * eps[i] * 0.5f * expf(0.5f * lv);
@@ -299,11 +317,12 @@
   return LO_OK;
 }
 int lo_latent_bwd(const f16* dz, const float* mu, const float* logvar, const float* eps, const float* coefs,
-                  const float* gmu, const float* glv, float gscale, f16* dml, int B, int L, hipStream_t st) {
+                  const float* gmu, const float* glv, float gscale, f16* dml, int B, int L, hipStream_t st, const LoLatentSlabSrc* src) {
   int n = B * L;
-  LoProfScope _p("lo_latent_bwd", 0, 0, st);
+  const LoLatentSlabSrc ss = src ? *src : LoLatentSlabSrc{nullptr, 0, nullptr};
+  LoProfScope _p(ss.slab ? "lo_latent_bwd/slab" : "lo_latent_bwd", 0, ss.slab ? 4.0 * n * ss.nsplit : 0, st);
   LO_LAUNCH_STOP(lo_latent_bwd_kernel, dim3((n + 255) / 256), dim3(256), 0, st, dz, mu, logvar, eps, coefs, gmu, glv,
-                     gscale, dml, B, L);
+                     gscale, dml, B, L, ss);
   LO_LAUNCH_CHECK("latent_bwd");
   return LO_OK;
 }
diff --git a/lunaris_orion_amd/csrc/lo_vae.h b/lunaris_orion_amd/csrc/lo_vae.h
--- a/lunaris_orion_amd/csrc/lo_vae.h
+++ b/lunaris_orion_amd/csrc/lo_vae.h
@@ -79,6 +79,7 @@
   float* norm_scratch = nullptr;
   bool fuse_gnb = true;
   bool fuse_gnf = false;
+  int lin_stream = 1;
   bool fuse_gna = true;
   size_t o_sync_fail = 0;
   bool lin_factored = false, fac_ready = false;
diff --git a/lunaris_orion_amd/csrc/lo_vae_plan.hip b/lunaris_orion_amd/csrc/lo_vae_plan.hip
--- a/lunaris_orion_amd/csrc/lo_vae_plan.hip
+++ b/lunaris_orion_amd/csrc/lo_vae_plan.hip
@@ -195,6 +195,7 @@
   h->gn_local = !env_is_zero(getenv("LO_GN_LOCAL"));
   h->fuse_gnf = getenv("LO_GN_FUSE") && atoi(getenv("LO_GN_FUSE")) != 0 && !h->fp8_fwd;
   h->fuse_gna = h->fuse_gnb && !env_is_zero(getenv("LO_GNB_APPLY_FUSE"));
+  h->lin_stream = getenv("LO_LINEAR_STREAM") ? atoi(getenv("LO_LINEAR_STREAM")) : 1;
   int dev = 0, ncu = 0;
   if (hipGetDevice(&dev) == hipSuccess && hipDeviceGetAttribute(&ncu, hipDeviceAttributeMultiprocessorCount, dev) == hipSuccess) h->n_cu = ncu;
   else (void)hipGetLastError();
diff --git a/lunaris_orion_amd/csrc/lo_vae_step.hip b/lunaris_orion_amd/csrc/lo_vae_step.hip
--- a/lunaris_orion_amd/csrc/lo_vae_step.hip
+++ b/lunaris_orion_amd/csrc/lo_vae_step.hip
@@ -54,8 +54,15 @@
   const int B = h->B;
   LO_TRY(vae_ensure_sync_init(h, ws, st));
   LO_TRY(vae_wait_level(h, st, 4));
-  LO_TRY(lo_conv_run(h->g_dfc, {.in = WSP(f16, h->o_z), .w = WSP(f16, h->o_wp_dfc), .bias = PRM(h->idx_dfc_b), .out = WSP(f16, h->o_yfc)}, st));
-  LO_TRY(lo_nchw_to_nhwc_f16(WSP(f16, h->o_yfc), WSP(f16, h->o_h0), B, 64, 512, st, h->o_h08 ? WSP(uint8_t, h->o_h08) : nullptr));
+  const int ls = h->lin_stream;
+  if (!h->o_h08 && lo_conv_choose(h->g_dfc, {.bias = true, .nhwc = true, .lin_stream = ls}).kernel == LO_CK_LINEAR_STREAM) {
+    LO_TRY(lo_conv_run(h->g_dfc, {.in = WSP(f16, h->o_z), .w = WSP(f16, h->o_wp_dfc), .bias = PRM(h->idx_dfc_b), .out = WSP(f16, h->o_h0),
+                                  .nhwc_hw = 64, .lin_stream = ls}, st));
+  } else {
+    LO_TRY(lo_conv_run(h->g_dfc, {.in = WSP(f16, h->o_z), .w = WSP(f16, h->o_wp_dfc), .bias = PRM(h->idx_dfc_b), .out = WSP(f16, h->o_yfc),
+                                  .lin_stream = ls}, st));
+    LO_TRY(lo_nchw_to_nhwc_f16(WSP(f16, h->o_yfc), WSP(f16, h->o_h0), B, 64, 512, st, h->o_h08 ? WSP(uint8_t, h->o_h08) : nullptr));
+  }
   const f16* cur = WSP(f16, h->o_h0);
   size_t cur8 = h->o_h08;
   for (int s = 0; s < 4; ++s) {
@@ -112,7 +119,8 @@
   }
   LO_TRY(lo_nhwc_to_nchw_f16(cur, WSP(f16, h->o_xflat), B, 64, 512, st));
   LO_TRY(vae_wait_level(h, st, 3));
-  LO_TRY(lo_conv_run(h->g_head, {.in = WSP(f16, h->o_xflat), .w = WSP(f16, h->o_wp_head), .slab = WSP(float, h->o_slab_head), .nsplit = h->head_split}, st));
+  LO_TRY(lo_conv_run(h->g_head, {.in = WSP(f16, h->o_xflat), .w = WSP(f16, h->o_wp_head), .slab = WSP(float, h->o_slab_head), .nsplit = h->head_split,
+                                 .lin_stream = h->lin_stream}, st));
   LO_REQUIRE(h->p_off[h->idx_fc_lv_b] == h->p_off[h->idx_fc_mu_b] + (size_t)L, "flat layout: head biases not adjacent");
   LO_TRY(lo_head_reduce(WSP(float, h->o_slab_head), PRM(h->idx_fc_mu_b), eps, seed, WSP(float, h->o_mu), WSP(float, h->o_lv),
                         WSP(f16, h->o_z), WSP(float, h->o_eps), WSP(float, h->o_klp), B, L, h->head_split, st, mu, logvar));
@@ -219,6 +227,7 @@
   float inv;
   bool side;
   f16 *Ga, *Gb, *Gc, *Gd;
+  bool dz_in_slab = false;
   VaeBackward(LoVae* h_, const float* P_, float* G_, void* ws_, float loss_scale_, void* stream)
       : h(h_), P(P_), G(G_), ws(ws_), loss_scale(loss_scale_), st(S(stream)), inv(1.0f / loss_scale_), side(vae_side_on(h_)),
         Ga(WSP(f16, h_->o_G[0])), Gb(WSP(f16, h_->o_G[1])), Gc(WSP(f16, h_->o_G[2])), Gd(WSP(f16, h_->o_G[3])) {}
@@ -348,7 +357,10 @@
   LO_TRY(lo_colsum_f16(Gfc, GRD(h->idx_dfc_b), B, 32768, inv, gs));
   if (!fac)
     LO_TRY(lo_wgrad_run(h->g_dfc, WSP(f16, h->o_z), Gfc, WSP(float, h->o_wslab_lin), GRD(h->idx_dfc_w), inv, gs));
-  LO_TRY(lo_conv_run(h->g_dfc_d, {.in = Gfc, .w = WSP(f16, h->o_wp_dfc_t), .slab = WSP(float, h->o_slab_dz), .nsplit = h->dfcd_split}, st));
+  LO_TRY(lo_conv_run(h->g_dfc_d, {.in = Gfc, .w = WSP(f16, h->o_wp_dfc_t), .slab = WSP(float, h->o_slab_dz), .nsplit = h->dfcd_split,
+                                  .lin_stream = h->lin_stream}, st));
+  dz_in_slab = !dz32 && (h->lin_stream >= 2 || (h->lin_stream == 1 && (long)B * L >= 64 * 512));
+  if (dz_in_slab) return LO_OK;
   return lo_splitk_reduce(WSP(float, h->o_slab_dz), nullptr, dz32, WSP(f16, h->o_dz), B, L, h->dfcd_split, st);
 }
 
@@ -358,9 +370,10 @@
   hipStream_t gs = beside ? h->side : st;
   {
     LoHandover ho(h, beside);
+    const LoLatentSlabSrc slab_src{WSP(float, h->o_slab_dz), h->dfcd_split, WSP(f16, h->o_dz)};
     LO_TRY(lo_latent_bwd(WSP(f16, h->o_dz), WSP(float, h->o_mu), WSP(float, h->o_lv), WSP(float, h->o_eps),
                          fused ? WSP(float, h->o_coefs) : nullptr, fused ? nullptr : gmu, fused ? nullptr : glv, loss_scale,
-                         WSP(f16, h->o_dml), B, L, st));
+                         WSP(f16, h->o_dml), B, L, st, dz_in_slab ? &slab_src : nullptr));
     LO_TRY(ho.finish(st));
     if (beside) LO_HIP(hipStreamWaitEvent(h->side, ho.ev, 0));
   }
@@ -373,9 +386,12 @@
   } else {
     LO_TRY(lo_wgrad_run(h->g_head, WSP(f16, h->o_xflat), WSP(f16, h->o_dml), WSP(float, h->o_wslab_lin), GRD(h->idx_fc_mu_w), inv, gs));
   }
-  LO_TRY(lo_conv_run(h->g_head_d, {.in = WSP(f16, h->o_dml), .w = WSP(f16, h->o_wp_head_t), .out = Gb}, st));
+  const int ls = h->lin_stream;
+  const bool direct = lo_conv_choose(h->g_head_d, {.nhwc = true, .lin_stream = ls}).kernel == LO_CK_LINEAR_STREAM;
+  if (!direct) LO_TRY(lo_conv_run(h->g_head_d, {.in = WSP(f16, h->o_dml), .w = WSP(f16, h->o_wp_head_t), .out = Gb, .lin_stream = ls}, st));
   LoHandover ho(h->ev_pre, beside && hand_to_side);
-  LO_TRY(lo_nchw_to_nhwc_f16(Gb, Ga, B, 64, 512, st));
+  if (direct) LO_TRY(lo_conv_run(h->g_head_d, {.in = WSP(f16, h->o_dml), .w = WSP(f16, h->o_wp_head_t), .out = Ga, .nhwc_hw = 64, .lin_stream = ls}, st));
+  else LO_TRY(lo_nchw_to_nhwc_f16(Gb, Ga, B, 64, 512, st));
   LO_TRY(ho.finish(st));
   if (ho.ev) LO_HIP(hipStreamWaitEvent(h->side, ho.ev, 0));
   return LO_OK;
```

Result: no change. 24920 sprites/s, median of 3 (+0.5%).
